# mudit1729/dinov2-od

Measured on AMD Instinct MI355X. Metric: images/sec forward, DINOv2 ViT-B/14 518x518 + 100-query head, higher is better.
Workload: dtype bf16; 1 GPU; ViT-B/14 518x518 bf16, 100 queries, batch 64 per GPU (BASELINE configs[2]'s batch of 64; it fits one GPU, so every GPU runs the whole configuration: weak scaling); global_batch=64, per_gpu_batch=64, image=518, queries=100, parallelism=dp1, hipgraph=True, n_ranks_seen=1, micro_batches=2

## Files before the change

dinov2_od_amd/csrc/dod_api.hip:

```cpp
#include "dod_internal.h"

#include <cstdarg>
#include <cstdio>
#include <atomic>
#include <cstdlib>

using namespace dod;

static std::string g_err;

static int vfail(const dod_handle* h, int code, const char* fmt, va_list ap, int launch_rc = 0) {
  char buf[512];
  const int n = vsnprintf(buf, sizeof buf, fmt, ap);
  if (launch_rc && n >= 0 && (size_t)n < sizeof buf) snprintf(buf + n, sizeof buf - n, " rejected (rc %d)", launch_rc);
  if (h) h->err = buf; else g_err = buf;
  return code;
}
int dod::fail(const dod_handle* h, int code, const char* fmt, ...) {
  va_list ap; va_start(ap, fmt); code = vfail(h, code, fmt, ap); va_end(ap);
  return code;
}
int dod::rejected(const dod_handle* h, int r, const char* fmt, ...) {
  if (!r) return DOD_OK;
  va_list ap; va_start(ap, fmt); const int code = vfail(h, r == 3 ? DOD_ERR_HIP : DOD_ERR_INVALID, fmt, ap, r); va_end(ap);
  return code;
}

static bool check_common(dod_handle* h, int B, int H, int W, int* rc) {
  if (!h) { *rc = fail(nullptr, DOD_ERR_INVALID, "null handle"); return false; }
  if (!h->finalized) { *rc = fail(h, DOD_ERR_STATE, "dod_finalize_weights has not been called"); return false; }
  if (B <= 0) { *rc = fail(h, DOD_ERR_INVALID, "batch must be positive (got %d)", B); return false; }
  if (H < h->cfg.patch || W < h->cfg.patch) { *rc = fail(h, DOD_ERR_INVALID, "image %dx%d smaller than one %dx%d patch", H, W, h->cfg.patch, h->cfg.patch); return false; }
  return true;
}

static std::atomic<int> g_options[DOD_OPT_COUNT] = {{-1}, {-1}, {-1}, {-1}, {-1}, {-1}, {-1}, {-1}, {-1}, {-1}, {-1}};
int dod_option(int which) { return which >= 0 && which < DOD_OPT_COUNT ? g_options[which].load() : -1; }
static const char* const k_option_names[DOD_OPT_COUNT] = {"tailsplit", "dec_fused_split", "mha_chunk_images", "no_fused_patch", "ln_fold", "deterministic", "f32_ksplit",
                                                       "attn_bwd_flash", "epi_regmath", "f32x3_tile", "attn_diet"};

static std::atomic<long> g_form_launches[FORM_COUNT];
static const char* const k_form_names[FORM_COUNT] = {"bf16_128_r2", "bf16_128_r3", "bf16_m16", "k64", "ppm", "x3_16w", "x3_pp", "h2", "fp8_rows", "fp8mx_256x128",
                                                     "fp8mx2_256x128", "fp8mx2_256x256", "f32", "patch_fused"};
void gemm_form_launched(int form) { if (form >= 0 && form < FORM_COUNT) ++g_form_launches[form]; }

extern "C" {

int dod_test_set_option(const char* name, int value) {
  if (!name) return fail(nullptr, DOD_ERR_INVALID, "null option name");
  for (int i = 0; i < DOD_OPT_COUNT; ++i)
    if (!strcmp(name, k_option_names[i])) { g_options[i].store(value); return DOD_OK; }
  return fail(nullptr, DOD_ERR_INVALID, "unknown test option '%s'", name);
}
long dod_test_counter(const char* name) {
  if (name && !strcmp(name, "tail_splits")) return gemm_tail_split_count();
  if (name && !strcmp(name, "rem_cuts")) return gemm_rem_cut_count();
  if (name && !strcmp(name, "f32_ksplits")) return gemm_f32_ksplit_count();
  if (name && !strcmp(name, "epi_regmath")) return gemm_epi_regmath_count();
  if (name && !strcmp(name, "attn_diet")) return attn_half_tile_count();
  if (name && !strcmp(name, "f32x3_launches")) return gemm_f32x3_count(0);
  if (name && !strcmp(name, "f32x3_wide_launches")) return gemm_f32x3_count(1);
  if (name && !strcmp(name, "optim_launches")) return optim_launch_count();
  if (name && !strcmp(name, "optim_chunk_elems")) return optim_constant(0);
  if (name && !strcmp(name, "optim_table_tensors")) return optim_constant(1);
  if (name && !strcmp(name, "optim_norm_table_tensors")) return optim_constant(2);
  if (name && !strncmp(name, "form_", 5))
    for (int i = 0; i < FORM_COUNT; ++i)
      if (!strcmp(name + 5, k_form_names[i])) return g_form_launches[i].load();
  return -1;
}

const char* dod_version(void) { return "dinodet 0.3 (gfx950)"; }
int dod_abi_version(void) { return DOD_ABI_VERSION; }

int dod_device_count(void) {
  int n = 0;
  return hipGetDeviceCount(&n) == hipSuccess ? n : -1;
}

const char* dod_last_error(const dod_handle* h) { return h ? h->err.c_str() : g_err.c_str(); }

int dod_create(const dod_config* cfg, dod_handle** out) {
  if (!cfg || !out) return fail(nullptr, DOD_ERR_INVALID, "null argument");
  const dod_config& c = *cfg;
  if (c.hidden <= 0 || c.layers <= 0 || c.heads <= 0 || c.hidden % c.heads) return fail(nullptr, DOD_ERR_INVALID, "bad backbone dims hidden=%d heads=%d layers=%d", c.hidden, c.heads, c.layers);
  if (c.hidden % 64) return fail(nullptr, DOD_ERR_INVALID, "hidden (%d) must be a multiple of 64", c.hidden);
  {
    const int fm = c.precision == DOD_PREC_FP32 ? 4 : 64;
    if (c.ffn_hidden <= 0 || c.ffn_hidden % fm) return fail(nullptr, DOD_ERR_INVALID, "ffn_hidden (%d) must be a multiple of %d in this precision", c.ffn_hidden, fm);
  }
  if (c.patch <= 0 || c.pos_grid <= 0) return fail(nullptr, DOD_ERR_INVALID, "bad patch/pos_grid");
  if (c.num_queries <= 0 || c.dec_hidden <= 0 || c.dec_heads <= 0 || c.dec_layers <= 0 || c.num_classes <= 0 || c.dim_feedforward <= 0) return fail(nullptr, DOD_ERR_INVALID, "bad decoder dims");
  if (c.dec_hidden % 64 || c.dim_feedforward % 4) return fail(nullptr, DOD_ERR_INVALID, "decoder hidden (%d) must be a multiple of 64, dim_feedforward (%d) of 4", c.dec_hidden, c.dim_feedforward);
  if (c.target_dim && c.target_dim != c.dec_hidden) return fail(nullptr, DOD_ERR_INVALID, "projection dim %d != decoder hidden %d", c.target_dim, c.dec_hidden);
  if (!c.target_dim && c.hidden != c.dec_hidden) return fail(nullptr, DOD_ERR_INVALID, "backbone width %d != decoder hidden %d and no projection", c.hidden, c.dec_hidden);
  if (c.use_deformable && (c.n_points <= 0 || c.n_points > 8)) return fail(nullptr, DOD_ERR_INVALID, "n_points must be 1..8");
  if (c.dec_layers > 64) return fail(nullptr, DOD_ERR_INVALID, "at most 64 decoder layers");
  if (c.precision != DOD_PREC_FP32 && c.precision != DOD_PREC_BF16 && c.precision != DOD_PREC_FP8 && c.precision != DOD_PREC_BF16X3 && c.precision != DOD_PREC_FP16X2) return fail(nullptr, DOD_ERR_INVALID, "unknown precision %d", c.precision);
  dod_handle* h = new (std::nothrow) dod_handle();
  if (!h) return fail(nullptr, DOD_ERR_STATE, "out of host memory");
  h->cfg = c;
  *out = h;
  return DOD_OK;
}

void dod_destroy(dod_handle* h) {
  if (!h) return;
  for (auto& r : h->prof) { (void)hipEventDestroy(r.a); (void)hipEventDestroy(r.b); }
  for (auto e : h->evpool) (void)hipEventDestroy(e);
  for (void* p : h->owned) (void)hipFree(p);
  delete h;
}

int dod_set_weight(dod_handle* h, const char* key, const void* dev_ptr, const int64_t* shape, int ndim, int dtype) {
  if (!h || !key || !dev_ptr || ndim < 0 || ndim > 8 || (ndim && !shape)) return fail(h, DOD_ERR_INVALID, "dod_set_weight: bad argument");
  if (dtype != DOD_F32 && dtype != DOD_BF16) return fail(h, DOD_ERR_INVALID, "dod_set_weight('%s'): dtype %d is neither DOD_F32 nor DOD_BF16", key, dtype);
  std::string k(key);
  if (k.rfind("module.", 0) == 0) k = k.substr(7);
  WRef r; r.raw = dev_ptr; r.dtype = dtype; r.ptr = dtype == DOD_F32 ? (const float*)dev_ptr : nullptr; r.shape.assign(shape, shape + ndim);
  h->w[k] = r;
  h->finalized = false;
  return DOD_OK;
}

int dod_reserve_gemm_scratch(size_t bytes) { return (gemm_tail_reserve(bytes) || gemm_f32_ksplit_reserve()) ? fail(nullptr, DOD_ERR_HIP, "scratch allocation of %zu bytes failed", bytes) : DOD_OK; }

int dod_finalize_weights(dod_handle* h, void* stream) {
  if (!h) return fail(nullptr, DOD_ERR_INVALID, "null handle");
  { static const size_t mb = [] { const char* v = getenv("DINODET_GEMM_SCRATCH_MB"); return v && atoi(v) > 0 ? (size_t)atoi(v) : (size_t)64; }();
    (void)gemm_tail_reserve(mb << 20);
    (void)gemm_f32_ksplit_reserve(); }
  int rc = finalize_impl(h, (hipStream_t)stream);
  if (rc || !h->has_dec) return rc;
  hipStream_t s = (hipStream_t)stream;
  const dod_config& g = h->cfg;
  const size_t Q = g.num_queries, Dd = g.dec_hidden;
  h->l0_tgt = h->l0_proj = nullptr;
  Carver sz(nullptr);
  const size_t bytes = carve_decoder(h, sz, 1, 1, nullptr, false) + 256;
  void* tmp = nullptr;
  float *t0 = nullptr, *p0 = nullptr;
  HIPCHK(h, hipMalloc(&tmp, bytes));
  if (hipMalloc((void**)&t0, Q * Dd * 4) != hipSuccess || (g.use_deformable && hipMalloc((void**)&p0, Q * (size_t)h->ncat * 4) != hipSuccess)) {
    (void)hipFree(tmp); if (t0) (void)hipFree(t0);
    return fail(h, DOD_ERR_HIP, "allocation of the decoder's layer-0 constants failed");
  }
  h->owned.push_back(t0); if (p0) h->owned.push_back(p0);
  Carver cv((void*)(((uintptr_t)tmp + 255) & ~(uintptr_t)255));
  DecWS dw;
  carve_decoder(h, cv, 1, 1, &dw, false);
  rc = decoder_impl(h, nullptr, 1, 1, dw, nullptr, s, true);
  if (!rc) {
    hipError_t e1 = hipMemcpyAsync(t0, dw.tgt, Q * Dd * 4, hipMemcpyDeviceToDevice, s);
    hipError_t e2 = p0 ? hipMemcpyAsync(p0, dw.proj, Q * (size_t)h->ncat * 4, hipMemcpyDeviceToDevice, s) : hipSuccess;
    hipError_t e3 = hipStreamSynchronize(s);
    if (e1 != hipSuccess || e2 != hipSuccess || e3 != hipSuccess) rc = fail(h, DOD_ERR_HIP, "decoder layer-0 constants: %s", hipGetErrorString(e3 != hipSuccess ? e3 : (e1 != hipSuccess ? e1 : e2)));
  } else (void)hipStreamSynchronize(s);
  (void)hipFree(tmp);
  if (rc) return rc;
  h->l0_tgt = t0; h->l0_proj = p0;
  return DOD_OK;
}

int dod_prepare(dod_handle* h, int H, int W, void* stream) {
  if (!h) return fail(nullptr, DOD_ERR_INVALID, "null handle");
  return prepare_impl(h, H, W, (hipStream_t)stream);
}

int dod_num_tokens(const dod_handle* h, int H, int W) { return h ? (H / h->cfg.patch) * (W / h->cfg.patch) + 1 : 0; }

size_t dod_workspace_bytes(const dod_handle* h, int B, int H, int W) {
  if (!h || B <= 0 || H < h->cfg.patch || W < h->cfg.patch) return 0;
  const int N = dod_num_tokens(h, H, W);
  Carver c(nullptr);
  carve_backbone(h, c, B, N, nullptr);
  carve_decoder(h, c, B, N, nullptr, false);
  return c.off + 256;
}

size_t dod_decoder_workspace_bytes(const dod_handle* h, int B, int N) {
  if (!h || B <= 0 || N <= 0) return 0;
  Carver c(nullptr);
  carve_decoder(h, c, B, N, nullptr, true);
  return c.off + 256;
}

int dod_set_tap(dod_handle* h, int stage, float* dst) {
  if (!h) return fail(nullptr, DOD_ERR_INVALID, "null handle");
  if (dst) h->taps[stage] = dst; else h->taps.erase(stage);
  return DOD_OK;
}

int dod_forward(dod_handle* h, const float* pixels, int B, int H, int W, float* det, void* workspace, size_t wsb, void* stream) {
  int rc;
  if (!check_common(h, B, H, W, &rc)) return rc;
  if (!pixels || !det || !workspace) return fail(h, DOD_ERR_INVALID, "null buffer");
  if (wsb < dod_workspace_bytes(h, B, H, W)) return fail(h, DOD_ERR_STATE, "workspace too small: %zu < %zu", wsb, dod_workspace_bytes(h, B, H, W));
  const int N = dod_num_tokens(h, H, W);
  Carver c(align_ws(workspace));
  BbWS bw; DecWS dw;
  carve_backbone(h, c, B, N, &bw);
  carve_decoder(h, c, B, N, &dw, false);
  CARVE_FITS(h, c, workspace, wsb)
  rc = backbone_impl(h, pixels, B, H, W, bw, nullptr, true, (hipStream_t)stream); if (rc) return rc;
  return decoder_impl(h, bw.mem, B, N, dw, det, (hipStream_t)stream);
}

int dod_forward_u8(dod_handle* h, const uint8_t* pixels_hwc, int B, int H, int W, float* det, void* workspace, size_t wsb, void* stream) {
  int rc;
  if (!check_common(h, B, H, W, &rc)) return rc;
  if (!pixels_hwc || !det || !workspace) return fail(h, DOD_ERR_INVALID, "null buffer");
  if (wsb < dod_workspace_bytes(h, B, H, W)) return fail(h, DOD_ERR_STATE, "workspace too small: %zu < %zu", wsb, dod_workspace_bytes(h, B, H, W));
  const int N = dod_num_tokens(h, H, W);
  Carver c(align_ws(workspace));
  BbWS bw; DecWS dw;
  carve_backbone(h, c, B, N, &bw);
  carve_decoder(h, c, B, N, &dw, false);
  CARVE_FITS(h, c, workspace, wsb)
  rc = backbone_impl(h, nullptr, B, H, W, bw, nullptr, true, (hipStream_t)stream, -1, nullptr, pixels_hwc); if (rc) return rc;
  return decoder_impl(h, bw.mem, B, N, dw, det, (hipStream_t)stream);
}

int dod_backbone_forward(dod_handle* h, const float* pixels, int B, int H, int W, float* features, void* workspace, size_t wsb, void* stream) {
  int rc;
  if (!check_common(h, B, H, W, &rc)) return rc;
  if (!pixels || !features || !workspace) return fail(h, DOD_ERR_INVALID, "null buffer");
  if (wsb < dod_workspace_bytes(h, B, H, W)) return fail(h, DOD_ERR_STATE, "workspace too small: %zu < %zu", wsb, dod_workspace_bytes(h, B, H, W));
  const int N = dod_num_tokens(h, H, W);
  Carver c(align_ws(workspace));
  BbWS bw;
  carve_backbone(h, c, B, N, &bw);
  CARVE_FITS(h, c, workspace, wsb)
  return backbone_impl(h, pixels, B, H, W, bw, features, false, (hipStream_t)stream);
}

int dod_backbone_prefix(dod_handle* h, const float* pixels, int B, int H, int W, int nblocks, float* x_out, void* workspace, size_t wsb, void* stream) {
  int rc;
  if (!check_common(h, B, H, W, &rc)) return rc;
  if (!pixels || !x_out || !workspace) return fail(h, DOD_ERR_INVALID, "null buffer");
  if (nblocks < 0 || nblocks > h->cfg.layers) return fail(h, DOD_ERR_INVALID, "nblocks %d outside 0..%d", nblocks, h->cfg.layers);
  if (wsb < dod_workspace_bytes(h, B, H, W)) return fail(h, DOD_ERR_STATE, "workspace too small: %zu < %zu", wsb, dod_workspace_bytes(h, B, H, W));
  const int N = dod_num_tokens(h, H, W);
  Carver c(align_ws(workspace));
  BbWS bw;
  carve_backbone(h, c, B, N, &bw);
  CARVE_FITS(h, c, workspace, wsb)
  return backbone_impl(h, pixels, B, H, W, bw, nullptr, false, (hipStream_t)stream, nblocks, x_out);
}

int dod_decoder_forward(dod_handle* h, const float* memory, int B, int N, float* det, void* workspace, size_t wsb, void* stream) {
  if (!h) return fail(nullptr, DOD_ERR_INVALID, "null handle");
  if (!h->finalized) return fail(h, DOD_ERR_STATE, "dod_finalize_weights has not been called");
  if (B <= 0 || N <= 0) return fail(h, DOD_ERR_INVALID, "bad B=%d N=%d", B, N);
  if (!memory || !det || !workspace) return fail(h, DOD_ERR_INVALID, "null buffer");
  if (wsb < dod_decoder_workspace_bytes(h, B, N)) return fail(h, DOD_ERR_STATE, "workspace too small");
  Carver c(align_ws(workspace));
  DecWS dw;
  carve_decoder(h, c, B, N, &dw, true);
  CARVE_FITS(h, c, workspace, wsb)
  hipStream_t s = (hipStream_t)stream;
  const void* mem_op = memory;
  if (is_bf16(h)) {
    KCHK(h, launch_cast_bf16(memory, (bf16_t*)dw.mem_op, (size_t)B * N * h->cfg.dec_hidden, s));
    mem_op = dw.mem_op;
  }
  return decoder_impl(h, mem_op, B, N, dw, det, s);
}

int dod_profile(dod_handle* h, int enable) {
  if (!h) return fail(nullptr, DOD_ERR_INVALID, "null handle");
  for (auto& r : h->prof) { h->evpool.push_back(r.a); h->evpool.push_back(r.b); }
  h->prof.clear();
  h->prof_on = enable != 0;
  return DOD_OK;
}

int dod_profile_read(dod_handle* h, int cls, double* ms, double* flops, int* launches) {
  if (!h || cls < 0 || cls >= PC_COUNT) return fail(h, DOD_ERR_INVALID, "bad profile class");
  double t = 0, f = 0; int n = 0;
  for (auto& r : h->prof) {
    if (r.cls != cls) continue;
    HIPCHK(h, hipEventSynchronize(r.b));
    float e = 0.f;
    HIPCHK(h, hipEventElapsedTime(&e, r.a, r.b));
    t += e; f += r.flops; ++n;
  }
  if (ms) *ms = t; if (flops) *flops = f; if (launches) *launches = n;
  return DOD_OK;
}

int dod_op_linear(int in_dtype, const void* A, int lda, const void* W, int ldw, int M, int N, int K, const float* bias,
                  const float* scale, const float* resid, int ldr, void* out, int out_dtype, int ldc, int act, void* stream) {
  if (!A || !W || !out) return fail(nullptr, DOD_ERR_INVALID, "null buffer");
  GemmEpi e = epi(bias, out_dtype == DOD_F32 ? (float*)out : nullptr, out_dtype == DOD_BF16 ? out : nullptr, ldc, act, scale, resid, ldr);
  if (act == DOD_ACT_SWIGLU_PAIRS) {
    if (in_dtype != DOD_BF16 || out_dtype != DOD_BF16 || scale || resid || (N & 7)) return fail(nullptr, DOD_ERR_INVALID, "DOD_ACT_SWIGLU_PAIRS: bf16 in / out, N %% 8 == 0, no scale / residual");
    e.act = ACT_NONE; e.glu = 1;
  }
  int r = in_dtype == DOD_BF16 ? launch_gemm_bf16((const bf16_t*)A, lda, (const bf16_t*)W, ldw, M, N, K, e, (hipStream_t)stream)
                               : launch_gemm_f32((const float*)A, lda, (const float*)W, ldw, M, N, K, e, (hipStream_t)stream);
  return rejected(nullptr, r, "dod_op_linear M=%d N=%d K=%d", M, N, K);
}
int dod_op_gemm_f32x(const float* A, int lda, int a_kmajor, long long a_sb, long long a_sh, const float* W, int ldw, int w_kmajor, long long w_sb,
                     long long w_sh, float* C, int ldc, long long c_sb, long long c_sh, int M, int N, int K, int batch, int hb, float alpha,
                     int accumulate, int ksplit, void* stream) {
  if (!A || !W || !C) return fail(nullptr, DOD_ERR_INVALID, "null buffer");
  GemmF32X g; memset(&g, 0, sizeof g);
  g.A = A; g.lda = lda; g.a_kmajor = a_kmajor; g.a_sb = a_sb; g.a_sh = a_sh;
  g.W = W; g.ldw = ldw; g.w_kmajor = w_kmajor; g.w_sb = w_sb; g.w_sh = w_sh;
  g.C = C; g.ldc = ldc; g.c_sb = c_sb; g.c_sh = c_sh;
  g.M = M; g.N = N; g.K = K; g.batch = batch; g.hb = hb; g.alpha = alpha; g.accumulate = accumulate; g.ksplit = ksplit;
  return rejected(nullptr, launch_gemm_f32x(g, (hipStream_t)stream), "dod_op_gemm_f32x M=%d N=%d K=%d batch=%d", M, N, K, batch);
}
int dod_op_gemm_f32x3(const float* A, int lda, int a_kmajor, long long a_sb, long long a_sh, const float* W, int ldw, int w_kmajor, long long w_sb,
                      long long w_sh, float* C, int ldc, long long c_sb, long long c_sh, int M, int N, int K, int batch, int hb, float alpha,
                      int accumulate, int ksplit, void* stream) {
  if (!A || !W || !C) return fail(nullptr, DOD_ERR_INVALID, "null buffer");
  GemmF32X g; memset(&g, 0, sizeof g);
  g.A = A; g.lda = lda; g.a_kmajor = a_kmajor; g.a_sb = a_sb; g.a_sh = a_sh;
  g.W = W; g.ldw = ldw; g.w_kmajor = w_kmajor; g.w_sb = w_sb; g.w_sh = w_sh;
  g.C = C; g.ldc = ldc; g.c_sb = c_sb; g.c_sh = c_sh;
  g.M = M; g.N = N; g.K = K; g.batch = batch; g.hb = hb; g.alpha = alpha; g.accumulate = accumulate; g.ksplit = ksplit;
  return rejected(nullptr, launch_gemm_f32x3(g, (hipStream_t)stream), "dod_op_gemm_f32x3 M=%d N=%d K=%d batch=%d", M, N, K, batch);
}
int dod_op_linear_f32x3(const float* X, int ldx, const float* W, const float* bias, const float* scale, const float* resid, int ldr, int M, int N, int K,
                        float* Y, int ldy, int act, void* stream) {
  if (!X || !W || !Y) return fail(nullptr, DOD_ERR_INVALID, "null buffer");
  if (act < DOD_ACT_NONE || act > DOD_ACT_SIGMOID) return fail(nullptr, DOD_ERR_INVALID, "dod_op_linear_f32x3: activation %d", act);
  GemmF32X g; memset(&g, 0, sizeof g);
  g.A = X; g.lda = ldx; g.W = W; g.ldw = K; g.C = Y; g.ldc = ldy; g.M = M; g.N = N; g.K = K; g.batch = 1; g.hb = 1; g.alpha = 1.0f; g.ksplit = 1;
  g.bias = bias; g.scale = scale; g.resid = resid; g.ldr = ldr; g.act = act;
  return rejected(nullptr, launch_gemm_f32x3(g, (hipStream_t)stream), "dod_op_linear_f32x3 M=%d N=%d K=%d", M, N, K);
}
int dod_op_linear_fp8(const void* A, int lda, const float* a_scale, const void* W, int ldw, const float* w_scale, int M, int N, int K,
                      const float* bias, const float* scale, const float* resid, int ldr, void* out, int out_dtype, int ldc, int act,
                      void* stream) {
  if (!A || !W || !out || !a_scale || !w_scale) return fail(nullptr, DOD_ERR_INVALID, "null buffer");
  GemmEpi e = epi(bias, out_dtype == DOD_F32 ? (float*)out : nullptr, out_dtype == DOD_BF16 ? out : nullptr, ldc, act, scale, resid, ldr);
  e.a_scale = a_scale; e.w_scale = w_scale;
  return rejected(nullptr, launch_gemm_fp8((const unsigned char*)A, lda, (const unsigned char*)W, ldw, M, N, K, e, (hipStream_t)stream), "dod_op_linear_fp8 M=%d N=%d K=%d", M, N, K);
}
int dod_op_linear_fp8_mx(const void* A, int lda, const void* a_block_scales, const void* W, int ldw, const float* w_scale, int M, int N, int K,
                         const float* bias, const float* scale, const float* resid, int ldr, void* out, int out_dtype, int ldc, int act,
                         void* stream) {
  if (!A || !W || !out || !a_block_scales || !w_scale) return fail(nullptr, DOD_ERR_INVALID, "null buffer");
  GemmEpi e = epi(bias, out_dtype == DOD_F32 ? (float*)out : nullptr, out_dtype == DOD_BF16 ? out : nullptr, ldc, act, scale, resid, ldr);
  e.a_bs = (const unsigned char*)a_block_scales; e.w_scale = w_scale;
  return rejected(nullptr, launch_gemm_fp8((const unsigned char*)A, lda, (const unsigned char*)W, ldw, M, N, K, e, (hipStream_t)stream), "dod_op_linear_fp8_mx M=%d N=%d K=%d", M, N, K);
}
int dod_op_linear_fp8_glu_mx(const void* A, int lda, const float* a_scale, const void* W, int ldw, const float* w_scale, int M, int N, int K,
                             const float* bias, void* out_q, int ldq, void* out_block_scales, void* stream) {
  if (!A || !W || !a_scale || !w_scale || !out_q || !out_block_scales) return fail(nullptr, DOD_ERR_INVALID, "null buffer");
  GemmEpi e = epi(bias, nullptr, out_q, ldq);
  e.a_scale = a_scale; e.w_scale = w_scale; e.glu = 1; e.out_bs = (unsigned char*)out_block_scales;
  return rejected(nullptr, launch_gemm_fp8((const unsigned char*)A, lda, (const unsigned char*)W, ldw, M, N, K, e, (hipStream_t)stream), "dod_op_linear_fp8_glu_mx M=%d N=%d K=%d", M, N, K);
}
int dod_op_linear_fp8_mx2(const void* A, int lda, const void* a_block_scales, const void* W, int ldw, const void* w_block_scales, int M, int N, int K,
                          const float* bias, const float* scale, const float* resid, int ldr, void* out, int out_dtype, int ldc, int act,
                          void* glu_out_block_scales, void* stream) {
  if (!A || !W || !out || !a_block_scales || !w_block_scales) return fail(nullptr, DOD_ERR_INVALID, "null buffer");
  GemmEpi e = epi(bias, out_dtype == DOD_F32 ? (float*)out : nullptr, out_dtype == DOD_BF16 ? out : nullptr, ldc, act, scale, resid, ldr);
  e.a_bs = (const unsigned char*)a_block_scales; e.w_bs = (const unsigned char*)w_block_scales;
  if (glu_out_block_scales) { e.out_f32 = nullptr; e.out_bf16 = (bf16_t*)out; e.glu = 1; e.out_bs = (unsigned char*)glu_out_block_scales; }
  return rejected(nullptr, launch_gemm_fp8((const unsigned char*)A, lda, (const unsigned char*)W, ldw, M, N, K, e, (hipStream_t)stream), "dod_op_linear_fp8_mx2 M=%d N=%d K=%d", M, N, K);
}
int dod_op_quant_mx_fp8(const void* x, int in_dtype, int ld, int rows, int cols, void* q, int ldq, void* block_scales, void* stream) {
  if (!x || !q || !block_scales) return fail(nullptr, DOD_ERR_INVALID, "null buffer");
  return rejected(nullptr, launch_quant_mx_fp8(x, in_dtype == DOD_BF16, ld, rows, cols, (unsigned char*)q, ldq, (unsigned char*)block_scales, (hipStream_t)stream), "dod_op_quant_mx_fp8 rows=%d cols=%d", rows, cols);
}
int dod_op_split_pair(const float* x, int ld, int rows, int cols, void* out, void* stream) {
  if (!x || !out) return fail(nullptr, DOD_ERR_INVALID, "null buffer");
  return launch_split2(x, ld, (bf16_t*)out, rows, cols, (hipStream_t)stream) ? fail(nullptr, DOD_ERR_HIP, "launch failed") : DOD_OK;
}
int dod_op_linear_x3(const void* A2, const void* W2, int M, int N, int K, const float* bias, const float* scale, const float* resid, int ldr,
                     void* out, int out_layout, int ldc, int act, void* stream) {
  if (!A2 || !W2 || !out) return fail(nullptr, DOD_ERR_INVALID, "null buffer");
  GemmEpi e = epi(bias, out_layout == 0 ? (float*)out : nullptr, out_layout != 0 ? out : nullptr, ldc, act, scale, resid, ldr);
  if (out_layout == 2) e.out_split = -N;
  return rejected(nullptr, launch_gemm_x3((const bf16_t*)A2, 2 * K, (const bf16_t*)W2, 2 * K, M, N, K, e, (hipStream_t)stream), "dod_op_linear_x3 M=%d N=%d K=%d", M, N, K);
}
int dod_op_split_h2(const float* x, int ld, int rows, int cols, void* out, void* wexp, void* stream) {
  if (!x || !out) return fail(nullptr, DOD_ERR_INVALID, "null buffer");
  return rejected(nullptr, launch_split_h2(x, ld, out, rows, cols, (unsigned char*)wexp, (hipStream_t)stream), "dod_op_split_h2 rows=%d cols=%d", rows, cols);
}
int dod_op_linear_h2(const void* A, const void* W, const void* wexp, int M, int N, int K, const float* bias, const float* scale, const float* resid,
                     int ldr, void* out, int out_layout, int ldc, int act, void* stream) {
  if (!A || !W || !wexp || !out) return fail(nullptr, DOD_ERR_INVALID, "null buffer");
  GemmEpi e = epi(bias, out_layout == 0 ? (float*)out : nullptr, out_layout != 0 ? out : nullptr, ldc, act, scale, resid, ldr);
  if (out_layout == 2) e.out_split = -N;
  if (out_layout == 3) e.out_h2 = 1;
  e.h2_wexp = (const unsigned char*)wexp;
  return rejected(nullptr, launch_gemm_h2(A, 4 * K, W, 3 * K, M, N, K, e, (hipStream_t)stream), "dod_op_linear_h2 M=%d N=%d K=%d", M, N, K);
}
int dod_op_linear_ln(int family, const void* A, const void* W, const void* wexp, int M, int N, int K, const float* bias, const float* scale,
                     const float* resid, int ldr, void* out, int out_layout, int ldc, int act, const dod_ln_fold* ln, void* stream) {
  if (!A || !W || !out || !ln) return fail(nullptr, DOD_ERR_INVALID, "null buffer");
  if (family != DOD_PREC_BF16 && family != DOD_PREC_BF16X3 && family != DOD_PREC_FP16X2) return fail(nullptr, DOD_ERR_INVALID, "family must be a bf16 / bf16x3 / fp16x2 precision");
  if ((ln->stats == nullptr) != (ln->csum == nullptr)) return fail(nullptr, DOD_ERR_INVALID, "stats and csum go together");
  if (ln->stats && scale) return fail(nullptr, DOD_ERR_INVALID, "the folded consumer has no LayerScale");
  if (ln->part && !(resid && out_layout == 0)) return fail(nullptr, DOD_ERR_INVALID, "the folded producer is the fp32 residual epilogue");
  GemmEpi e = epi(bias, out_layout == 0 ? (float*)out : nullptr, out_layout != 0 ? out : nullptr, ldc, act, scale, resid, ldr);
  if (out_layout == 2) e.out_split = -N;
  if (out_layout == 3) e.out_h2 = 1;
  e.ln_stats = (const float2*)ln->stats; e.ln_c = ln->csum;
  if (ln->part_in) {
    if (!ln->stats || ln->stats_out == ln->stats) return fail(nullptr, DOD_ERR_INVALID, "part_in needs stats (the shift) and a DIFFERENT stats_out buffer");
    e.ln_part_in = (const float2*)ln->part_in; e.ln_npart = (K + 127) / 128; e.ln_stats_out = (float2*)ln->stats_out; e.ln_eps = ln->eps;
  }
  if (ln->part) {
    e.ln_part = (float2*)ln->part; e.ln_npart = (N + 127) / 128; e.ln_op = ln->op_out; e.ln_shift = (const float2*)ln->shift;
    e.ln_op_kind = family == DOD_PREC_FP16X2 ? LNOP_H2 : (family == DOD_PREC_BF16X3 ? LNOP_PAIR : LNOP_BF16);
    e.ln_op_ld = family == DOD_PREC_BF16 ? N : 2 * N;
  }
  int r;
  if (family == DOD_PREC_FP16X2) {
    if (!wexp) return fail(nullptr, DOD_ERR_INVALID, "null buffer");
    e.h2_wexp = (const unsigned char*)wexp;
    r = launch_gemm_h2(A, 4 * K, W, 3 * K, M, N, K, e, (hipStream_t)stream);
  } else if (family == DOD_PREC_BF16X3) r = launch_gemm_x3((const bf16_t*)A, 2 * K, (const bf16_t*)W, 2 * K, M, N, K, e, (hipStream_t)stream);
  else r = launch_gemm_bf16((const bf16_t*)A, K, (const bf16_t*)W, K, M, N, K, e, (hipStream_t)stream);
  return rejected(nullptr, r, "dod_op_linear_ln M=%d N=%d K=%d", M, N, K);
}
int dod_op_rowstats(const float* x, int rows, int D, float eps, void* op_out, int family, void* stats, void* stream) {
  if (!x || !op_out || !stats) return fail(nullptr, DOD_ERR_INVALID, "null buffer");
  const int kind = family == DOD_PREC_FP16X2 ? LNOP_H2 : (family == DOD_PREC_BF16X3 ? LNOP_PAIR : (family == DOD_PREC_BF16 ? LNOP_BF16 : 0));
  return rejected(nullptr, launch_rowstats(x, rows, D, eps, op_out, kind, (float2*)stats, (hipStream_t)stream), "dod_op_rowstats rows=%d D=%d", rows, D);
}
int dod_op_ln_finalize(const void* part, int rows, int D, float eps, void* stats, void* stream) {
  if (!part || !stats) return fail(nullptr, DOD_ERR_INVALID, "null buffer");
  return rejected(nullptr, launch_ln_finalize((const float2*)part, (D + 127) / 128, rows, D, eps, (float2*)stats, (hipStream_t)stream), "dod_op_ln_finalize rows=%d D=%d", rows, D);
}
int dod_op_attention_x3(const void* qkv2, void* ctx2, int B, int N, int heads, float scale, void* stream) {
  if (!qkv2 || !ctx2) return fail(nullptr, DOD_ERR_INVALID, "null buffer");
  return rejected(nullptr, launch_attn_x3((const bf16_t*)qkv2, (bf16_t*)ctx2, B, N, heads, scale, (hipStream_t)stream), "dod_op_attention_x3");
}
static bool attn_grid_fits(int B, int N, int heads) {
  return (((long long)B * heads + 7) / 8 * 8) * (((long long)N + 127) / 128 + 1) <= 0x7fffffffLL;
}
int dod_op_attention_x3_h2(const void* qkv2, void* ctx_h2, int B, int N, int heads, float scale, void* stream) {
  if (!qkv2 || !ctx_h2) return fail(nullptr, DOD_ERR_INVALID, "null buffer");
  if (B <= 0 || N <= 0 || heads <= 0) return fail(nullptr, DOD_ERR_INVALID, "dod_op_attention_x3_h2: B=%d N=%d heads=%d must be positive", B, N, heads);
  if (!attn_grid_fits(B, N, heads)) return fail(nullptr, DOD_ERR_INVALID, "dod_op_attention_x3_h2: B=%d N=%d heads=%d is more workgroups than one launch holds", B, N, heads);
  return rejected(nullptr, launch_attn_x3((const bf16_t*)qkv2, (bf16_t*)ctx_h2, B, N, heads, scale, (hipStream_t)stream, 1), "dod_op_attention_x3_h2");
}
int dod_op_quant_rows_fp8(const void* x, int in_dtype, int ld, int rows, int cols, void* q, int ldq, float* scale, void* stream) {
  if (!x || !q || !scale) return fail(nullptr, DOD_ERR_INVALID, "null buffer");
  return rejected(nullptr, launch_quant_rows_fp8(x, in_dtype == DOD_BF16, ld, rows, cols, (unsigned char*)q, ldq, scale, (hipStream_t)stream), "dod_op_quant_rows_fp8 rows=%d cols=%d", rows, cols);
}
int dod_op_layernorm(const float* x, const float* add, const float* gamma, const float* beta, float eps, int rows, int D, void* out, int out_dtype, void* stream) {
  if (!x || !gamma || !beta || !out) return fail(nullptr, DOD_ERR_INVALID, "null buffer");
  return rejected(nullptr, launch_layernorm(x, add, gamma, beta, eps, rows, D, ln_out(out_dtype == DOD_F32 ? (float*)out : nullptr, out_dtype == DOD_BF16 ? (bf16_t*)out : nullptr), (hipStream_t)stream), "dod_op_layernorm rows=%d D=%d", rows, D);
}
int dod_op_attention_bf16(const void* qkv, void* ctx, int B, int N, int heads, float scale, void* stream) {
  if (!qkv || !ctx) return fail(nullptr, DOD_ERR_INVALID, "null buffer");
  return rejected(nullptr, launch_attn_bf16((const bf16_t*)qkv, (bf16_t*)ctx, B, N, heads, scale, (hipStream_t)stream), "dod_op_attention_bf16");
}
int dod_op_attention_bf16_mx(const void* qkv, void* ctx_q8, void* ctx_bs, int B, int N, int heads, float scale, void* stream) {
  if (!qkv || !ctx_q8 || !ctx_bs) return fail(nullptr, DOD_ERR_INVALID, "null buffer");
  if (B <= 0 || N <= 0 || heads <= 0) return fail(nullptr, DOD_ERR_INVALID, "dod_op_attention_bf16_mx: B=%d N=%d heads=%d must be positive", B, N, heads);
  if (!attn_grid_fits(B, N, heads)) return fail(nullptr, DOD_ERR_INVALID, "dod_op_attention_bf16_mx: B=%d N=%d heads=%d is more workgroups than one launch holds", B, N, heads);
  return rejected(nullptr, launch_attn_bf16((const bf16_t*)qkv, (bf16_t*)ctx_q8, B, N, heads, scale, (hipStream_t)stream, (unsigned char*)ctx_bs), "dod_op_attention_bf16_mx");
}
int dod_op_attention_f32(const float* q, const float* k, const float* v, float* o, int ldq, int ldk, int ldv, int ldo, int Lq, int Lk,
                         int B, int heads, int dh, float scale, void* stream) {
  if (!q || !k || !v || !o) return fail(nullptr, DOD_ERR_INVALID, "null buffer");
  AttnF32 a; a.q = q; a.k = k; a.v = v; a.o = o; a.ldq = ldq; a.ldk = ldk; a.ldv = ldv; a.ldo = ldo; a.Lq = Lq; a.Lk = Lk; a.B = B; a.heads = heads; a.dh = dh; a.scale = scale;
  return rejected(nullptr, launch_attn_f32(a, (hipStream_t)stream), "dod_op_attention_f32 (dh=%d)", dh);
}
int dod_op_deform_sample(const float* proj, int ldp, const float* values, int B, int Q, int N, int Hd, int P, int dh, int hh, int ww, float* out, void* stream) {
  if (!proj || !values || !out) return fail(nullptr, DOD_ERR_INVALID, "null buffer");
  if (hh * ww != N) return fail(nullptr, DOD_ERR_INVALID, "Cannot reshape input of size %d into a %dx%d feature map", N, hh, ww);
  return rejected(nullptr, launch_deform_sample(proj, ldp, values, B, Q, N, Hd, P, dh, hh, ww, out, (hipStream_t)stream), "dod_op_deform_sample");
}
int dod_op_pos_resize(const float* pos_in, int G, int gh, int gw, int D, float* pos_out, void* stream) {
  if (!pos_in || !pos_out) return fail(nullptr, DOD_ERR_INVALID, "null buffer");
  return launch_pos_resize(pos_in, G, gh, gw, D, pos_out, (hipStream_t)stream) ? fail(nullptr, DOD_ERR_HIP, "launch failed") : DOD_OK;
}
int dod_op_im2col(const float* img, int B, int H, int W, int patch, int Kp, void* out, int out_dtype, void* stream) {
  if (!img || !out) return fail(nullptr, DOD_ERR_INVALID, "null buffer");
  int r = launch_im2col(img, B, H, W, patch, Kp, out_dtype == DOD_F32 ? (float*)out : nullptr, out_dtype == DOD_BF16 ? (bf16_t*)out : nullptr, (hipStream_t)stream);
  return r ? fail(nullptr, DOD_ERR_INVALID, "dod_op_im2col rejected") : DOD_OK;
}

}
```

dinov2_od_amd/csrc/dod_common.h:

```cpp
#pragma once
#include <hip/hip_runtime.h>
#include <stdint.h>
#include <stdlib.h>

typedef __attribute__((ext_vector_type(8))) __bf16 bf16x8;
typedef __attribute__((ext_vector_type(4))) __bf16 bf16x4;
typedef __attribute__((ext_vector_type(2))) __bf16 bf16x2;
typedef __attribute__((ext_vector_type(16))) float f32x16;
typedef __attribute__((ext_vector_type(4))) float f32x4;
typedef __attribute__((ext_vector_type(2))) float f32x2;
typedef unsigned short bf16_t;

#define DOD_WAVE 64

enum { DOD_OPT_TAILSPLIT = 0,
       DOD_OPT_DEC_FUSED_SPLIT,
       DOD_OPT_MHA_CHUNK_IMAGES,
       DOD_OPT_NO_FUSED_PATCH,
       DOD_OPT_LN_FOLD,
       DOD_OPT_DETERMINISTIC,
       DOD_OPT_F32_KSPLIT,
       DOD_OPT_ATTN_BWD_FLASH,
       DOD_OPT_EPI_REGMATH,
       DOD_OPT_F32X3_TILE,
       DOD_OPT_ATTN_DIET,
       DOD_OPT_COUNT };
int dod_option(int which);
long gemm_tail_split_count();
long optim_launch_count();
long optim_constant(int which);
long gemm_rem_cut_count();
long attn_half_tile_count();
long gemm_epi_regmath_count();
enum { FORM_BF16_128_R2 = 0, FORM_BF16_128_R3, FORM_BF16_M16, FORM_K64, FORM_PPM, FORM_X3_16W, FORM_X3_PP, FORM_H2, FORM_FP8_ROWS, FORM_FP8MX_256X128,
       FORM_FP8MX2_256X128, FORM_FP8MX2_256X256, FORM_F32, FORM_PATCH_FUSED, FORM_COUNT };
void gemm_form_launched(int form);

#ifdef DINODET_TUNING
#define DOD_TUNE_ENV(name) getenv(name)
#else
#define DOD_TUNE_ENV(name) (static_cast<const char*>(nullptr))
#endif

__device__ __forceinline__ bf16_t f2bf(float f) {
  __bf16 b = (__bf16)f;
  return __builtin_bit_cast(bf16_t, b);
}
__device__ __forceinline__ float bf2f(bf16_t h) {
  return __builtin_bit_cast(float, ((uint32_t)h) << 16);
}
__device__ __forceinline__ uint32_t pack2bf(float lo, float hi) {
  f32x2 v = {lo, hi};
  bf16x2 h = __builtin_convertvector(v, bf16x2);
  return __builtin_bit_cast(uint32_t, h);
}
__device__ __forceinline__ float wave_sum(float v) {
#pragma unroll
  for (int o = 32; o > 0; o >>= 1) v += __shfl_xor(v, o, 64);
  return v;
}
__device__ __forceinline__ float wave_max(float v) {
#pragma unroll
  for (int o = 32; o > 0; o >>= 1) v = fmaxf(v, __shfl_xor(v, o, 64));
  return v;
}
__device__ __forceinline__ unsigned pack4_fp8(float a, float b, float c, float d) {
  int w = __builtin_amdgcn_cvt_pk_fp8_f32(a, b, 0, false);
  w = __builtin_amdgcn_cvt_pk_fp8_f32(c, d, w, true);
  return (unsigned)w;
}
__device__ __forceinline__ unsigned mx_ebyte(float amax) {
  const unsigned b = __float_as_uint(amax * (1.0f / 448.0f));
  unsigned eb = ((b >> 23) & 0xffu) + ((b & 0x7fffffu) ? 1u : 0u);
  eb = eb < 1u ? 1u : (eb > 253u ? 253u : eb);
  return eb;
}
__device__ __forceinline__ float mx_inv_scale(unsigned eb) { return __uint_as_float((254u - eb) << 23); }
__device__ __forceinline__ size_t mx_scale_off(int K, int bi) { return (size_t)(bi & 1) * (K >> 6) + (bi >> 1); }
typedef __attribute__((ext_vector_type(2))) _Float16 f16x2;
typedef __attribute__((ext_vector_type(8))) _Float16 f16x8;
__device__ __forceinline__ float clampf_(float v, float lim) { return __builtin_fminf(__builtin_fmaxf(v, -lim), lim); }
__device__ __forceinline__ void h2_quad(float4 v, float shi, uint2& f16, unsigned& hi8, unsigned& lo8) {
  v.x = clampf_(v.x, 65504.f); v.y = clampf_(v.y, 65504.f); v.z = clampf_(v.z, 65504.f); v.w = clampf_(v.w, 65504.f);
  const f16x2 p0 = {(_Float16)v.x, (_Float16)v.y}, p1 = {(_Float16)v.z, (_Float16)v.w};
  f16.x = __builtin_bit_cast(unsigned, p0); f16.y = __builtin_bit_cast(unsigned, p1);
  const float hx = (float)p0.x, hy = (float)p0.y, hz = (float)p1.x, hw = (float)p1.y;
  const float slo = shi * 2048.0f;
  hi8 = pack4_fp8(clampf_(hx * shi, 448.f), clampf_(hy * shi, 448.f), clampf_(hz * shi, 448.f), clampf_(hw * shi, 448.f));
  lo8 = pack4_fp8(clampf_((v.x - hx) * slo, 448.f), clampf_((v.y - hy) * slo, 448.f), clampf_((v.z - hz) * slo, 448.f), clampf_((v.w - hw) * slo, 448.f));
}
__device__ __forceinline__ size_t h2_off8(int K, int c) { return (size_t)2 * K + (size_t)(c >> 4) * 32 + (c & 15); }

__device__ __forceinline__ float gelu_erf(float x) { return 0.5f * x * (1.0f + erff(x * 0.70710678118654752440f)); }
typedef float f32x2_t __attribute__((ext_vector_type(2)));
__device__ __forceinline__ f32x2_t gelu_fast2(f32x2_t x) {
  f32x2_t ax; ax.x = __builtin_fabsf(x.x); ax.y = __builtin_fabsf(x.y);
  const f32x2_t z = ax * 0.8493218002880191f;
  const f32x2_t d = __builtin_elementwise_fma(z, (f32x2_t)(0.2727374808792225f), (f32x2_t)(1.0f));
  f32x2_t t; t.x = __builtin_amdgcn_rcpf(d.x); t.y = __builtin_amdgcn_rcpf(d.y);
  f32x2_t p = __builtin_elementwise_fma(t, (f32x2_t)(0.5f * 1.061405429f), (f32x2_t)(0.5f * -1.453152027f));
  p = __builtin_elementwise_fma(p, t, (f32x2_t)(0.5f * 1.421413741f));
  p = __builtin_elementwise_fma(p, t, (f32x2_t)(0.5f * -0.284496736f));
  p = __builtin_elementwise_fma(p, t, (f32x2_t)(0.5f * 0.254829592f));
  const f32x2_t nz2 = -z * z;
  f32x2_t e; e.x = __builtin_amdgcn_exp2f(nz2.x); e.y = __builtin_amdgcn_exp2f(nz2.y);
  const f32x2_t q = ax * (t * p);
  const f32x2_t r = __builtin_elementwise_fma(ax, (f32x2_t)(0.5f), x * 0.5f);
  return __builtin_elementwise_fma(-q, e, r);
}
__device__ __forceinline__ void gelu_fast4(float4& v) {
  f32x2_t a = {v.x, v.y}, b = {v.z, v.w};
  a = gelu_fast2(a); b = gelu_fast2(b);
  v.x = a.x; v.y = a.y; v.z = b.x; v.w = b.y;
}
__device__ __forceinline__ float sigmoidf_(float x) { return 1.0f / (1.0f + expf(-x)); }

enum { ACT_NONE = 0, ACT_RELU = 1, ACT_GELU = 2, ACT_SIGMOID = 3 };

struct GemmEpi {
  const float* bias;
  const float* scale;
  const float* resid;
  int ldr;
  float* out_f32;
  bf16_t* out_bf16;
  int ldc;
  int act;
  const float* pos;
  int rows_per_img;
  int out_rows_per_img;
  int out_split;
  const float* a_scale;
  const float* w_scale;
  unsigned char* out_bs;
  const unsigned char* a_bs;
  const unsigned char* w_bs;
  int out_h2;
  const unsigned char* h2_wexp;
  int ksplit;
  int kslice_len;
  long long kslice_stride;
  int glu;
  void* ln_op;
  int ln_op_kind;
  int ln_op_ld;
  float2* ln_part;
  int ln_npart;
  const float2* ln_shift;
  const float2* ln_stats;
  const float* ln_c;
  const float2* ln_part_in;
  float2* ln_stats_out;
  float ln_eps;
};
enum { LNOP_BF16 = 1, LNOP_PAIR = 2, LNOP_H2 = 3 };
inline bool gemm_epi_rows_ok(const GemmEpi& e) {
  return e.rows_per_img == 0 && !e.pos && e.ksplit <= 1 && !e.a_scale && !e.a_bs && !e.out_bs;
}
inline GemmEpi gemm_epi_rows(const GemmEpi& e, int m0) {
  GemmEpi r = e;
  const size_t m = (size_t)m0;
  if (r.resid) r.resid += m * r.ldr;
  if (r.out_f32) r.out_f32 += m * r.ldc;
  if (r.out_bf16) r.out_bf16 += m * r.ldc;
  if (r.ln_op) r.ln_op = reinterpret_cast<char*>(r.ln_op) + m * (size_t)r.ln_op_ld * 2;
  if (r.ln_part) r.ln_part += m * r.ln_npart;
  if (r.ln_shift) r.ln_shift += m;
  if (r.ln_stats) r.ln_stats += m;
  if (r.ln_part_in) r.ln_part_in += m * r.ln_npart;
  if (r.ln_stats_out) r.ln_stats_out += m;
  return r;
}

int launch_gemm_bf16(const bf16_t* A, int lda, const bf16_t* W, int ldw, int M, int N, int K,
                     const GemmEpi& e, hipStream_t s);
int launch_gemm_f32(const float* A, int lda, const float* W, int ldw, int M, int N, int K,
                    const GemmEpi& e, hipStream_t s, bool allow_ksplit = false);
int gemm_f32_ksplit_reserve();
long gemm_f32_ksplit_count();
struct GemmF32X {
  const float* A; const float* W; float* C; const float* bias;
  const float* scale;
  const float* resid;
  int ldr;
  int lda, ldw, ldc, M, N, K;
  long long a_sb, a_sh, w_sb, w_sh, c_sb, c_sh;
  int batch, hb;
  int a_kmajor, w_kmajor;
  float alpha;
  int accumulate;
  int act;
  int ksplit;
};
int launch_gemm_f32x(const GemmF32X& g, hipStream_t s);
int launch_gemm_f32x3(const GemmF32X& g, hipStream_t s);
long gemm_f32x3_count(int wide);
int launch_quant_mx_fp8(const void* x, int in_bf16, int ld, int rows, int cols, unsigned char* q, int ldq, unsigned char* bs, hipStream_t s);
int launch_gemm_fp8(const unsigned char* A, int lda, const unsigned char* W, int ldw, int M, int N, int K,
                    const GemmEpi& e, hipStream_t s);
int launch_attn_x3(const bf16_t* qkv2, bf16_t* ctx3, int B, int N, int heads, float scale, hipStream_t s, int ctx_h2 = 0);
int launch_swiglu_fp8(const bf16_t* in, int rows, int Fh, unsigned char* q, float* scale, hipStream_t s);
int launch_quant_rows_fp8(const void* x, int in_bf16, int ld, int rows, int cols, unsigned char* q, int ldq, float* scale,
                          hipStream_t s);

struct LnOut {
  float* f32 = nullptr;
  bf16_t* bf16 = nullptr;
  unsigned char* fp8 = nullptr;
  float* scale = nullptr;
  bf16_t* split = nullptr;
  bf16_t* a3 = nullptr;
  unsigned char* bs = nullptr;
};
inline LnOut ln_out(float* f32, bf16_t* bf16 = nullptr, bf16_t* a3 = nullptr) { LnOut o; o.f32 = f32; o.bf16 = bf16; o.a3 = a3; return o; }
int launch_layernorm(const float* x, const float* add, const float* gamma, const float* beta, float eps, int rows, int D, const LnOut& out,
                     hipStream_t s, int split_h2 = 0);
int launch_rowstats(const float* x, int rows, int D, float eps, void* op, int op_kind, float2* stats, hipStream_t s);
int launch_ln_finalize(const float2* part, int npart, int rows, int D, float eps, float2* stats, hipStream_t s);
int launch_ln_fold(const float* W, int rows, int cols, const float* gamma, const float* beta, const float* bias_in, float* Wout, float* bias_out, hipStream_t s);
int launch_rowsum(const float* W, int rows, int cols, int round_bf16, float* c, hipStream_t s);

int launch_attn_bf16(const bf16_t* qkv, bf16_t* ctx, int B, int N, int heads, float scale, hipStream_t s, unsigned char* ctx_bs = nullptr);

struct AttnF32 {
  const float *q, *k, *v; float* o;
  int ldq, ldk, ldv, ldo;
  int Lq, Lk;
  int B, heads, dh;
  float scale;
  bf16_t* o3 = nullptr;
  float* lse = nullptr;
};
int launch_attn_f32(const AttnF32& a, hipStream_t s);
struct AttnF32Bwd {
  const float *q, *k, *v, *o, *d_o, *lse;
  float *dq, *dk, *dv, *delta;
  int ldq, ldk, ldv, ldo, lddq, lddk, lddv;
  int Lq, Lk, B, heads, dh;
  float scale;
};
int launch_attn_f32_bwd(const AttnF32Bwd& a, hipStream_t s);

int launch_im2col(const float* img, int B, int H, int W, int patch, int Kp, float* out_f32, bf16_t* out_bf16, hipStream_t s);
int launch_patch_pack(const float* W, int D, int p, bf16_t* out, int x3, hipStream_t s);
int launch_patch_embed(const void* img, int u8, int B, int H, int W, int p, const bf16_t* Wp, int x3, const float* bias, const float* pos,
                       float* out, int D, hipStream_t s);
int launch_cls_row(const float* cls, const float* pos, float* x, int B, int N, int D, hipStream_t s);
int launch_pos_resize(const float* pos_in, int G, int gh, int gw, int D, float* pos_out, hipStream_t s);
int launch_interleave_halves(const float* src, float* dst, int F, int cols, hipStream_t s);
int launch_swiglu(const float* in_f32, const bf16_t* in_bf16, int rows, int Fh, float* out_f32, bf16_t* out_bf16, hipStream_t s);
int launch_cast_bf16(const float* in, bf16_t* out, size_t n, hipStream_t s);
int launch_copy2d(const float* src, int ld_src, float* dst, int ld_dst, int rows, int cols, int cols_pad, hipStream_t s);
int launch_lora_merge(const float* W, const float* A, const float* Bm, float alpha, int out_f, int in_f, int r, float* dst, hipStream_t s);
int launch_split3(const float* in, int ld_in, bf16_t* out, int rows, int K, int mode, hipStream_t s);
int launch_split2(const float* in, int ld_in, bf16_t* out, int rows, int K, hipStream_t s);
int launch_split_h2(const float* in, int ld_in, void* out, int rows, int K, unsigned char* wexp, hipStream_t s);
int launch_gemm_h2(const void* A, int lda, const void* W, int ldw, int M, int N, int K, const GemmEpi& e, hipStream_t s);
int gemm_tail_split(int kind, const void* A, int lda, const void* W, int ldw, int M, int N, int K, const GemmEpi& e, hipStream_t s);
int gemm_tail_reserve(size_t bytes);
int launch_gemm_bf16_k64(const bf16_t* A, int lda, const bf16_t* W, int ldw, int M, int N, int K, const GemmEpi& e, hipStream_t s);
int gemm_tile_mode();
int launch_gemm_bf16_ppm(const bf16_t* A, int lda, const bf16_t* W, int ldw, int M, int N, int K, const GemmEpi& e, hipStream_t s);
int launch_gemm_x3_pp(const bf16_t* A2, int lda, const bf16_t* W2, int ldw, int M, int N, int K, const GemmEpi& e, hipStream_t s);
int launch_gemm_x3(const bf16_t* A2, int lda, const bf16_t* W2, int ldw, int M, int N, int K, const GemmEpi& e, hipStream_t s);
int launch_bcast_rows(const float* src, float* dst, int B, int rows, int D, hipStream_t s);

int launch_deform_sample(const float* proj, int ldp, const float* values, int B, int Q, int N, int Hd, int P, int dh,
                         int h, int w, float* out, hipStream_t s, int proj_shared = 0, bf16_t* out3 = nullptr);
```

dinov2_od_amd/csrc/gemm_bf16.hip:

```cpp
#include "dod_common.h"
#include "gemm_epi.h"
#include <atomic>
#include <cstdlib>

#define BM 128
#define BN 128
#define BK 64
#define STAGE_BYTES (2 * BM * BK * 2)

__device__ __forceinline__ int swz128(int row, int chunk) { return chunk ^ ((row >> 1) & 7); }

template <int LN, int SLOTS>
__global__ __launch_bounds__(256) void gemm_bf16_kernel(const bf16_t* __restrict__ A, int lda,
                                                        const bf16_t* __restrict__ W, int ldw,
                                                        int M, int N, int K, GemmEpi e) {
  extern __shared__ __attribute__((aligned(16))) char smem[];
  const int tid = threadIdx.x, lane = tid & 63, wid = tid >> 6;
  const int wm = wid >> 1, wn = wid & 1;
  const int tiles_m = (M + BM - 1) / BM, tiles_n = (N + BN - 1) / BN;
  const int nwg = tiles_m * tiles_n;
  int bid = blockIdx.x;
  {
    const int q = nwg >> 3, r = nwg & 7, xcd = bid & 7;
    bid = (xcd < r ? xcd * (q + 1) : r * (q + 1) + (xcd - r) * q) + (bid >> 3);
  }
  int tm, tn;
  {
    const int GM = 8;
    const int per_group = GM * tiles_n;
    const int grp = bid / per_group, first_m = grp * GM;
    const int gsz = (tiles_m - first_m) < GM ? (tiles_m - first_m) : GM;
    const int in_g = bid - grp * per_group;
    tm = first_m + in_g % gsz;
    tn = in_g / gsz;
  }
  const int m0 = tm * BM, n0 = tn * BN;

  typedef __attribute__((address_space(1))) const void* gptr_t;
  typedef __attribute__((address_space(3))) void* lptr_t;
  const bf16_t* gA0; const bf16_t* gA1; const bf16_t* gA2; const bf16_t* gA3;
  const bf16_t* gW0; const bf16_t* gW1; const bf16_t* gW2; const bf16_t* gW3;
  {
    auto src = [&](const bf16_t* base, int ld, int r0, int piece, int lim) {
      const int rl = piece * 8 + (lane >> 3);
      int r = r0 + rl; r = r < lim ? r : lim - 1;
      const int c = (lane & 7) ^ ((rl >> 1) & 7);
      return base + (size_t)r * ld + c * 8;
    };
    const int p0 = wid * 4;
    gA0 = src(A, lda, m0, p0, M); gA1 = src(A, lda, m0, p0 + 1, M); gA2 = src(A, lda, m0, p0 + 2, M); gA3 = src(A, lda, m0, p0 + 3, M);
    gW0 = src(W, ldw, n0, p0, N); gW1 = src(W, ldw, n0, p0 + 1, N); gW2 = src(W, ldw, n0, p0 + 2, N); gW3 = src(W, ldw, n0, p0 + 3, N);
  }
  const int wbase = __builtin_amdgcn_readfirstlane(wid) * 4096;
#define STAGE(stage, k0)                                                                                   \
  {                                                                                                        \
    char* sA_ = smem + (stage) * STAGE_BYTES + wbase;                                                      \
    char* sW_ = sA_ + BM * BK * 2;                                                                         \
    __builtin_amdgcn_global_load_lds((gptr_t)(gA0 + (k0)), (lptr_t)(sA_), 16, 0, 0);                       \
    __builtin_amdgcn_global_load_lds((gptr_t)(gA1 + (k0)), (lptr_t)(sA_ + 1024), 16, 0, 0);                \
    __builtin_amdgcn_global_load_lds((gptr_t)(gA2 + (k0)), (lptr_t)(sA_ + 2048), 16, 0, 0);                \
    __builtin_amdgcn_global_load_lds((gptr_t)(gA3 + (k0)), (lptr_t)(sA_ + 3072), 16, 0, 0);                \
    __builtin_amdgcn_global_load_lds((gptr_t)(gW0 + (k0)), (lptr_t)(sW_), 16, 0, 0);                       \
    __builtin_amdgcn_global_load_lds((gptr_t)(gW1 + (k0)), (lptr_t)(sW_ + 1024), 16, 0, 0);                \
    __builtin_amdgcn_global_load_lds((gptr_t)(gW2 + (k0)), (lptr_t)(sW_ + 2048), 16, 0, 0);                \
    __builtin_amdgcn_global_load_lds((gptr_t)(gW3 + (k0)), (lptr_t)(sW_ + 3072), 16, 0, 0);                \
  }

  f32x16 acc[2][2];
#pragma unroll
  for (int i = 0; i < 2; ++i)
#pragma unroll
    for (int j = 0; j < 2; ++j)
#pragma unroll
      for (int r = 0; r < 16; ++r) acc[i][j][r] = 0.f;

  const int nk = K / BK;
  STAGE(0, 0)
  if (SLOTS > 2 && nk > 1) STAGE(1, BK)
  const int lr = lane & 31, lh = lane >> 5;
  int slot = 0;
  for (int kt = 0; kt < nk; ++kt) {
    if (SLOTS > 2 && kt + 1 < nk) asm volatile("s_waitcnt vmcnt(8)" ::: "memory");
    else asm volatile("s_waitcnt vmcnt(0)" ::: "memory");
    __builtin_amdgcn_s_barrier();
    asm volatile("" ::: "memory");
    if (kt + SLOTS - 1 < nk) {
      const int ns = slot + SLOTS - 1 >= SLOTS ? slot - 1 : slot + SLOTS - 1;
      STAGE(ns, (kt + SLOTS - 1) * BK)
    }
    const char* sA = smem + slot * STAGE_BYTES;
    const char* sW = sA + BM * BK * 2;
#pragma unroll
    for (int kk = 0; kk < 4; ++kk) {
      bf16x8 af[2], wf[2];
#pragma unroll
      for (int i = 0; i < 2; ++i) {
        const int rowa = wm * 64 + i * 32 + lr;
        af[i] = *reinterpret_cast<const bf16x8*>(sA + rowa * 128 + swz128(rowa, kk * 2 + lh) * 16);
        const int roww = wn * 64 + i * 32 + lr;
        wf[i] = *reinterpret_cast<const bf16x8*>(sW + roww * 128 + swz128(roww, kk * 2 + lh) * 16);
      }
#pragma unroll
      for (int i = 0; i < 2; ++i)
#pragma unroll
        for (int j = 0; j < 2; ++j)
          acc[i][j] = __builtin_amdgcn_mfma_f32_32x32x16_bf16(wf[j], af[i], acc[i][j], 0, 0, 0);
    }
    slot = slot + 1 == SLOTS ? 0 : slot + 1;
  }
  __syncthreads();

  constexpr int PITCH = BN * 4 + 16;
#pragma unroll
  for (int i = 0; i < 2; ++i)
#pragma unroll
    for (int j = 0; j < 2; ++j)
      stage_acc(smem, PITCH, wm * 64 + i * 32 + lr, wn * 64 + j * 32, acc[i][j], lh);
  const ColParams cp = load_col_params<BN, LN>(e, n0, N, tid);
  auto rowmap = [&](int row_l) { return m0 + row_l; };
  stage_row_stats<BM, BN, LN>(smem, PITCH, e, M, tid, rowmap, K, n0);
  __syncthreads();
  drain_tile<BM, BN, 256, LN>(smem, PITCH, e, cp, M, N, n0, tid, rowmap);
}

#define B4K 32
#define B5M 256
#define B5N 128
#define B5_STAGE ((B5M + B5N) * B4K * 2)
#define B5_SLOTS 3

#define STAGE5(slot_, k0)                                                                                  \
  {                                                                                                        \
    char* sA_ = smem + (slot_) * B5_STAGE + wu * 2048;                                                     \
    char* sW_ = smem + (slot_) * B5_STAGE + B5M * B4K * 2 + wu * 1024;                                     \
    __builtin_amdgcn_global_load_lds((gptr_t)(gA0 + (k0)), (lptr_t)(sA_), 16, 0, 0);                       \
    __builtin_amdgcn_global_load_lds((gptr_t)(gA1 + (k0)), (lptr_t)(sA_ + 1024), 16, 0, 0);                \
    __builtin_amdgcn_global_load_lds((gptr_t)(gW0 + (k0)), (lptr_t)(sW_), 16, 0, 0);                       \
  }

__device__ __forceinline__ int swz64m16(int row, int chunk) { return chunk ^ (((row >> 3) & 1) << 1); }

#ifdef DINODET_TUNING
__device__ unsigned long long* g_gemm_stamps = nullptr;
#endif

template <int LN>
__global__ __launch_bounds__(512, 4) void gemm_bf16_256x128_m16_kernel(const bf16_t* __restrict__ A, int lda,
                                                                       const bf16_t* __restrict__ W, int ldw,
                                                                       int M, int N, int K, GemmEpi e, int GM) {
  extern __shared__ __attribute__((aligned(16))) char smem[];
  const int tid = threadIdx.x, lane = tid & 63, wid = tid >> 6;
  const int wm = wid >> 1, wn = wid & 1;
  const int tiles_m = (M + B5M - 1) / B5M, tiles_n = (N + B5N - 1) / B5N;
  const int nwg = tiles_m * tiles_n;
#ifdef DINODET_TUNING
  unsigned long long* stamps = g_gemm_stamps;
  unsigned long long t_start = 0, t_loop = 0;
  if (stamps) t_start = __builtin_amdgcn_s_memrealtime();
#endif
  int tm, tn;
  tile_map(blockIdx.x, tiles_m, tiles_n, GM, &tm, &tn);
  const int m0 = tm * B5M, n0 = tn * B5N;
  typedef __attribute__((address_space(1))) const void* gptr_t;
  typedef __attribute__((address_space(3))) void* lptr_t;
  const bf16_t* gA0; const bf16_t* gA1; const bf16_t* gW0;
  {
    auto src = [&](const bf16_t* base, int ld, int r0, int piece, int lim) {
      const int rl = piece * 16 + (lane >> 2);
      int r = r0 + rl; r = r < lim ? r : lim - 1;
      const int c = swz64m16(rl, lane & 3);
      return base + (size_t)r * ld + c * 8;
    };
    gA0 = src(A, lda, m0, wid * 2, M); gA1 = src(A, lda, m0, wid * 2 + 1, M);
    gW0 = src(W, ldw, n0, wid, N);
  }
  const int wu = __builtin_amdgcn_readfirstlane(wid);
  f32x4 acc[4][4];
#pragma unroll
  for (int i = 0; i < 4; ++i)
#pragma unroll
    for (int j = 0; j < 4; ++j) acc[i][j] = f32x4{0.f, 0.f, 0.f, 0.f};
  const int nk = K / B4K;
  const int l15 = lane & 15, l4 = lane >> 4;
  STAGE5(0, 0)
  if (nk > 1) STAGE5(1, B4K)
  int offA[4], offW[4];
#pragma unroll
  for (int i = 0; i < 4; ++i) { const int row = wm * 64 + i * 16 + l15; offA[i] = row * 64 + swz64m16(row, l4) * 16; }
#pragma unroll
  for (int j = 0; j < 4; ++j) { const int row = wn * 64 + j * 16 + l15; offW[j] = B5M * B4K * 2 + row * 64 + swz64m16(row, l4) * 16; }
  int slot = 0;
  for (int kt = 0; kt < nk; ++kt) {
    if (kt + 1 < nk) asm volatile("s_waitcnt vmcnt(3)" ::: "memory");
    else asm volatile("s_waitcnt vmcnt(0)" ::: "memory");
    __builtin_amdgcn_s_barrier();
    asm volatile("" ::: "memory");
    if (kt + 2 < nk) {
      const int ns = slot >= 1 ? slot - 1 : 2;
      STAGE5(ns, (kt + 2) * B4K)
    }
    const char* st = smem + slot * B5_STAGE;
    bf16x8 af[4], wf[4];
#pragma unroll
    for (int i = 0; i < 4; ++i) af[i] = *reinterpret_cast<const bf16x8*>(st + offA[i]);
#pragma unroll
    for (int j = 0; j < 4; ++j) wf[j] = *reinterpret_cast<const bf16x8*>(st + offW[j]);
#pragma unroll
    for (int i = 0; i < 4; ++i)
#pragma unroll
      for (int j = 0; j < 4; ++j)
        acc[i][j] = __builtin_amdgcn_mfma_f32_16x16x32_bf16(wf[j], af[i], acc[i][j], 0, 0, 0);
    slot = slot == 2 ? 0 : slot + 1;
  }
#ifdef DINODET_TUNING
  if (stamps) t_loop = __builtin_amdgcn_s_memrealtime();
#endif
  constexpr int PITCH = B5N * 4 + 16;
  const ColParams cp = load_col_params<B5N, LN>(e, n0, N, tid);
#pragma unroll
  for (int pass = 0; pass < 2; ++pass) {
    __builtin_amdgcn_s_barrier();
    asm volatile("" ::: "memory");
#pragma unroll
    for (int ii = 0; ii < 2; ++ii)
#pragma unroll
      for (int j = 0; j < 4; ++j) {
        const int row_l = wm * 32 + ii * 16 + l15;
        const int col = wn * 64 + j * 16 + 4 * l4;
        const f32x4 a = acc[pass * 2 + ii][j];
        *reinterpret_cast<float4*>(smem + row_l * PITCH + col * 4) = make_float4(a[0], a[1], a[2], a[3]);
      }
    auto rowmap = [&](int row_l) { return m0 + (row_l >> 5) * 64 + pass * 32 + (row_l & 31); };
    stage_row_stats<128, B5N, LN>(smem, PITCH, e, M, tid, rowmap, K, n0);
    __syncthreads();
    drain_tile<128, B5N, 512, LN>(smem, PITCH, e, cp, M, N, n0, tid, rowmap);
  }
#ifdef DINODET_TUNING
  if (stamps && tid == 0) {
    asm volatile("s_waitcnt vmcnt(0)" ::: "memory");
    unsigned long long* o = stamps + (size_t)blockIdx.x * 4;
    o[0] = t_start; o[1] = t_loop; o[2] = __builtin_amdgcn_s_memrealtime(); o[3] = blockIdx.x;
  }
#endif
}

static constexpr int LDS128 = (BM * (BN * 4 + 16)) > 2 * STAGE_BYTES ? (BM * (BN * 4 + 16)) : 2 * STAGE_BYTES;
static constexpr int LDS128R = 3 * STAGE_BYTES;
static constexpr int LDS5 = (128 * (B5N * 4 + 16)) > B5_SLOTS * B5_STAGE ? (128 * (B5N * 4 + 16)) : B5_SLOTS * B5_STAGE;

static std::atomic<long> g_rem_cuts{0};
long gemm_rem_cut_count() { return g_rem_cuts.load(); }

int launch_gemm_bf16(const bf16_t* A, int lda, const bf16_t* W, int ldw, int M, int N, int K,
                     const GemmEpi& e, hipStream_t s) {
  if (M <= 0 || N <= 0 || K <= 0) return 1;
  if (K % BK != 0 || N % 4 != 0 || lda % 8 != 0 || ldw % 8 != 0 || e.ldc % 4 != 0) return 2;
  if (e.resid && e.ldr % 4 != 0) return 2;
  if (!e.out_f32 && !e.out_bf16) return 2;
  static bool attr_set[16] = {};
  int dev = 0;
  (void)hipGetDevice(&dev);
  if (dev >= 0 && dev < 16 && !attr_set[dev]) {
#define ATTR_(LN_) (void)hipFuncSetAttribute(reinterpret_cast<const void*>(gemm_bf16_kernel<LN_, 2>), hipFuncAttributeMaxDynamicSharedMemorySize, LDS128); \
                   (void)hipFuncSetAttribute(reinterpret_cast<const void*>(gemm_bf16_kernel<LN_, 3>), hipFuncAttributeMaxDynamicSharedMemorySize, LDS128R); \
                   (void)hipFuncSetAttribute(reinterpret_cast<const void*>(gemm_bf16_256x128_m16_kernel<LN_>), hipFuncAttributeMaxDynamicSharedMemorySize, LDS5);
    ATTR_(LN_NONE) ATTR_(LN_CONS) ATTR_(LN_PROD)
#undef ATTR_
    attr_set[dev] = true;
  }
  const char* force = DOD_TUNE_ENV("DINODET_GEMM_TILE");
  if (!force && M >= 2048 && N >= 512 && e.act != ACT_GELU && e.act != ACT_SIGMOID && e.rows_per_img == 0 && K % 64 == 0) {
    const int t = gemm_tail_split(0, A, lda, W, ldw, M, N, K, e, s);
    if (t >= 0) return t;
  }
  if (force && force[0] == 'q' && K % 64 == 0) return launch_gemm_bf16_ppm(A, lda, W, ldw, M, N, K, e, s);
  if (force && force[0] == 'x') return launch_gemm_bf16_k64(A, lda, W, ldw, M, N, K, e, s);
  const int gm5 = (N >= 3072 ? 8 : (N >= 2048 ? 4 : 2)) | (gemm_tile_mode() & 0x300);
  const int tiles5 = ((M + B5M - 1) / B5M) * ((N + B5N - 1) / B5N);
#define GO_M16(LN_) hipLaunchKernelGGL(gemm_bf16_256x128_m16_kernel<LN_>, dim3(tiles5), dim3(512), LDS5, s, A, lda, W, ldw, M, N, K, e, gm5);
  if (!force && M >= 4096 && N >= 512 && K % 64 == 0 && e.act != ACT_SIGMOID && e.rows_per_img == 0) {
    static int cus[16] = {};
    if (dev >= 0 && dev < 16 && !cus[dev]) { int c = 0; (void)hipDeviceGetAttribute(&c, hipDeviceAttributeMultiprocessorCount, dev); cus[dev] = c > 0 ? c : 256; }
    const int cu = (dev >= 0 && dev < 16) ? cus[dev] : 256;
    const long tm = (M + 255) / 256, t_big = tm * ((N + 255) / 256), t_small = tm * ((N + 127) / 128);
    const double c_big = (double)((t_big + cu - 1) / cu) * (e.act == ACT_GELU ? 1.08 : 1.0);
    const double c_small = (double)((t_small + cu - 1) / cu) * (K >= 2048 ? 0.62 : 0.55);
    if (N >= 1536 && K < 2048) {
      const long rounds = t_big / cu, rem = t_big % cu;
      static const int rem_div = [] { const char* v = DOD_TUNE_ENV("DINODET_GEMM_REMCUT"); return v ? atoi(v) : 6; }();
      if (rounds >= 1 && rounds <= 2 && rem * 16 >= cu && rem_div > 0 && rem * rem_div <= cu && gemm_epi_rows_ok(e)) {
        const int tn = (N + 255) / 256;
        const int Mmain = (int)((rounds * cu) / tn) * 256, R = M - Mmain;
        if (Mmain >= 2048 && R > 0 && R < 2048) {
          const int rc = launch_gemm_bf16_k64(A, lda, W, ldw, Mmain, N, K, e, s);
          if (rc) return rc;
          ++g_rem_cuts;
          return launch_gemm_bf16(A + (size_t)Mmain * lda, lda, W, ldw, R, N, K, gemm_epi_rows(e, Mmain), s);
        }
      }
      return launch_gemm_bf16_k64(A, lda, W, ldw, M, N, K, e, s);
    }
    static const double m16_bias = [] { const char* v = DOD_TUNE_ENV("DINODET_GEMM_M16_BIAS"); return v ? atof(v) : 1.02; }();
    if (c_big <= c_small * m16_bias) {
      if (K >= 2048) return launch_gemm_bf16_ppm(A, lda, W, ldw, M, N, K, e, s);
      return launch_gemm_bf16_k64(A, lda, W, ldw, M, N, K, e, s);
    }
    LN_DISPATCH(e, GO_M16)
    gemm_form_launched(FORM_BF16_M16);
    return hipGetLastError() == hipSuccess ? 0 : 3;
  }
  const bool few = (long)tiles5 * 2 <= 256 + 64;
  const bool m16 = force ? (force[0] == '8') : (M >= 1024 && N >= 128 && !few);
  if (m16) {
    LN_DISPATCH(e, GO_M16)
    gemm_form_launched(FORM_BF16_M16);
  } else {
    const int tiles = ((M + BM - 1) / BM) * ((N + BN - 1) / BN);
    static const int ring = [] { const char* v = DOD_TUNE_ENV("DINODET_GEMM_RING"); return v ? atoi(v) : 1; }();
    int cu128 = 256;
    { static int cus[16] = {}; if (dev >= 0 && dev < 16) { if (!cus[dev]) { int c = 0; (void)hipDeviceGetAttribute(&c, hipDeviceAttributeMultiprocessorCount, dev); cus[dev] = c > 0 ? c : 256; } cu128 = cus[dev]; } }
#define GO_128(LN_) hipLaunchKernelGGL((gemm_bf16_kernel<LN_, 2>), dim3(tiles), dim3(256), LDS128, s, A, lda, W, ldw, M, N, K, e);
#define GO_128R(LN_) hipLaunchKernelGGL((gemm_bf16_kernel<LN_, 3>), dim3(tiles), dim3(256), LDS128R, s, A, lda, W, ldw, M, N, K, e);
    if (ring && tiles <= cu128 && K >= 3 * BK) { LN_DISPATCH(e, GO_128R) gemm_form_launched(FORM_BF16_128_R3); }
    else { LN_DISPATCH(e, GO_128) gemm_form_launched(FORM_BF16_128_R2); }
#undef GO_128
#undef GO_128R
  }
  return hipGetLastError() == hipSuccess ? 0 : 3;
}
#undef GO_M16

#ifdef DINODET_TUNING
extern "C" int dod_debug_gemm_stamps(void* dev_buf) {
  unsigned long long* p = (unsigned long long*)dev_buf;
  return hipMemcpyToSymbol(HIP_SYMBOL(g_gemm_stamps), &p, sizeof(p)) == hipSuccess ? 0 : 4;
}

template <int SHAPE>
__global__ __launch_bounds__(256, 2) void mfma_peak_kernel(int iters, unsigned long long* out) {
  bf16x8 a, b;
#pragma unroll
  for (int i = 0; i < 8; ++i) { a[i] = (bf16_t)(0x3c00 + threadIdx.x + i); b[i] = (bf16_t)(0x3c10 + threadIdx.x * 3 + i); }
  if (iters < 0) {
    iters = -iters;
#pragma unroll
    for (int i = 0; i < 8; ++i) {
      const unsigned r1 = (threadIdx.x * 8u + i + 1u) * 2654435761u, r2 = (threadIdx.x * 8u + i + 7u) * 40503u * 2246822519u;
      a[i] = (bf16_t)(0x3f00u | ((r1 >> 9) & 0xffu) | (((r1 >> 20) & 1u) << 15));
      b[i] = (bf16_t)(0x3f00u | ((r2 >> 9) & 0xffu) | (((r2 >> 20) & 1u) << 15));
    }
  }
  const unsigned long long c0 = __builtin_amdgcn_s_memtime(), r0 = __builtin_amdgcn_s_memrealtime();
  float chk = 0.f;
  if (SHAPE == 16) {
    f32x4 acc[8];
#pragma unroll
    for (int i = 0; i < 8; ++i) acc[i] = f32x4{0.f, 0.f, 0.f, 0.f};
    for (int it = 0; it < iters; ++it) {
#pragma unroll
      for (int i = 0; i < 8; ++i) acc[i] = __builtin_amdgcn_mfma_f32_16x16x32_bf16(a, b, acc[i], 0, 0, 0);
    }
#pragma unroll
    for (int i = 0; i < 8; ++i) chk += acc[i][0];
  } else if (SHAPE == 1) {
    f32x16 acc1;
#pragma unroll
    for (int r = 0; r < 16; ++r) acc1[r] = 0.f;
    const float fa = bf2f(a[0]) * (1.0f + 0.37f * bf2f(a[1])), fb = bf2f(b[0]) * (1.0f + 0.41f * bf2f(b[1]));
    for (int it = 0; it < iters; ++it) {
#pragma unroll
      for (int i = 0; i < 4; ++i) acc1 = __builtin_amdgcn_mfma_f32_32x32x2f32(fa, fb, acc1, 0, 0, 0);
    }
    chk += acc1[0];
  } else if (SHAPE == 2) {
    f32x16 acc[4];
#pragma unroll
    for (int i = 0; i < 4; ++i)
#pragma unroll
      for (int r = 0; r < 16; ++r) acc[i][r] = 0.f;
    const float fa = bf2f(a[0]) * (1.0f + 0.37f * bf2f(a[1])), fb = bf2f(b[0]) * (1.0f + 0.41f * bf2f(b[1]));
    for (int it = 0; it < iters; ++it) {
#pragma unroll
      for (int i = 0; i < 4; ++i) acc[i] = __builtin_amdgcn_mfma_f32_32x32x2f32(fa, fb, acc[i], 0, 0, 0);
    }
#pragma unroll
    for (int i = 0; i < 4; ++i) chk += acc[i][0];
  } else {
    f32x16 acc[4];
#pragma unroll
    for (int i = 0; i < 4; ++i)
#pragma unroll
      for (int r = 0; r < 16; ++r) acc[i][r] = 0.f;
    for (int it = 0; it < iters; ++it) {
#pragma unroll
      for (int i = 0; i < 4; ++i) acc[i] = __builtin_amdgcn_mfma_f32_32x32x16_bf16(a, b, acc[i], 0, 0, 0);
    }
#pragma unroll
    for (int i = 0; i < 4; ++i) chk += acc[i][0];
  }
  const unsigned long long c1 = __builtin_amdgcn_s_memtime(), r1 = __builtin_amdgcn_s_memrealtime();
  if (threadIdx.x == 0) {
    out[(size_t)blockIdx.x * 4 + 0] = c1 - c0;
    out[(size_t)blockIdx.x * 4 + 1] = r1 - r0;
    out[(size_t)blockIdx.x * 4 + 2] = (unsigned long long)__float_as_uint(chk);
  }
}
extern "C" int dod_debug_mfma_peak(int shape, int iters, int blocks, void* dev_out, void* stream) {
  if (!dev_out || iters == 0 || blocks <= 0 || (shape != 16 && shape != 32 && shape != 2 && shape != 1)) return 1;
  if (shape == 1) hipLaunchKernelGGL(mfma_peak_kernel<1>, dim3(blocks), dim3(256), 0, (hipStream_t)stream, iters, (unsigned long long*)dev_out);
  else if (shape == 2) hipLaunchKernelGGL(mfma_peak_kernel<2>, dim3(blocks), dim3(256), 0, (hipStream_t)stream, iters, (unsigned long long*)dev_out);
  else if (shape == 16) hipLaunchKernelGGL(mfma_peak_kernel<16>, dim3(blocks), dim3(256), 0, (hipStream_t)stream, iters, (unsigned long long*)dev_out);
  else hipLaunchKernelGGL(mfma_peak_kernel<32>, dim3(blocks), dim3(256), 0, (hipStream_t)stream, iters, (unsigned long long*)dev_out);
  return hipGetLastError() == hipSuccess ? 0 : 4;
}

template <int NV, int mode>
__global__ __launch_bounds__(256, 2) void mfma_valu_probe_kernel(int iters, unsigned long long* out) {
  bf16x8 a, b;
#pragma unroll
  for (int i = 0; i < 8; ++i) { a[i] = (bf16_t)(0x3c00 + threadIdx.x + i); b[i] = (bf16_t)(0x3c10 + threadIdx.x * 3 + i); }
  f32x16 acc[4];
#pragma unroll
  for (int i = 0; i < 4; ++i)
#pragma unroll
    for (int r = 0; r < 16; ++r) acc[i][r] = 0.f;
  float v[NV];
#pragma unroll
  for (int i = 0; i < NV; ++i) v[i] = 1.0f + 0.001f * (threadIdx.x + i);
  const float m = 0.999f, c = 0.001f;
  const unsigned long long c0 = __builtin_amdgcn_s_memtime();
  for (int it = 0; it < iters; ++it) {
#pragma unroll
    for (int q = 0; q < 4; ++q) {
      if (mode & 1) asm volatile("v_mfma_f32_32x32x16_bf16 %0, %1, %2, %0" : "+v"(acc[q]) : "v"(a), "v"(b));
      if (mode & 2) {
#pragma unroll
        for (int i = 0; i < NV / 4; ++i) asm volatile("v_fma_f32 %0, %0, %1, %2" : "+v"(v[q * (NV / 4) + i]) : "v"(m), "v"(c));
      }
    }
  }
  const unsigned long long c1 = __builtin_amdgcn_s_memtime();
  float chk = 0.f;
#pragma unroll
  for (int i = 0; i < 4; ++i) chk += acc[i][0];
#pragma unroll
  for (int i = 0; i < NV; ++i) chk += v[i];
  if (threadIdx.x == 0) { out[(size_t)blockIdx.x * 4] = c1 - c0; out[(size_t)blockIdx.x * 4 + 2] = (unsigned long long)__float_as_uint(chk); }
}
template <int NV>
static int probe_launch(int mode, int iters, int blocks, void* dev_out, void* stream) {
  unsigned long long* o = (unsigned long long*)dev_out;
  if (mode == 1) hipLaunchKernelGGL((mfma_valu_probe_kernel<NV, 1>), dim3(blocks), dim3(256), 0, (hipStream_t)stream, iters, o);
  else if (mode == 2) hipLaunchKernelGGL((mfma_valu_probe_kernel<NV, 2>), dim3(blocks), dim3(256), 0, (hipStream_t)stream, iters, o);
  else if (mode == 3) hipLaunchKernelGGL((mfma_valu_probe_kernel<NV, 3>), dim3(blocks), dim3(256), 0, (hipStream_t)stream, iters, o);
  else return 1;
  return hipGetLastError() == hipSuccess ? 0 : 4;
}
extern "C" int dod_debug_mfma_valu_probe(int nvalu, int mode, int iters, int blocks, void* dev_out, void* stream) {
  if (!dev_out || iters <= 0 || blocks <= 0) return 1;
  if (nvalu == 16) return probe_launch<16>(mode, iters, blocks, dev_out, stream);
  if (nvalu == 28) return probe_launch<28>(mode, iters, blocks, dev_out, stream);
  if (nvalu == 56) return probe_launch<56>(mode, iters, blocks, dev_out, stream);
  return 1;
}
#endif
```

dinov2_od_amd/csrc/gemm_epi.h:

```cpp
#pragma once
#include "dod_common.h"

__device__ __forceinline__ int swz64(int row, int chunk) { return chunk ^ ((row >> 2) & 3); }

#ifdef DINODET_TUNING
__device__ __forceinline__ void stagger_start(int b, int mode) {
  const int sd = (mode >> 16) & 0xfff;
  if (sd == 0 || b >= 256) return;
  const int k = (b >> 3) % (((mode >> 12) & 0xf) + 1);
  if (k == 0) return;
  const unsigned long long until = __builtin_amdgcn_s_memrealtime() + (unsigned long long)k * sd * 16;
  while (__builtin_amdgcn_s_memrealtime() < until) __builtin_amdgcn_s_sleep(16);
}

#endif

__device__ __forceinline__ void tile_map(int b, int tiles_m, int tiles_n, int mode, int* tm_out, int* tn_out) {
#ifdef DINODET_TUNING
  stagger_start(b, mode);
#endif
  const int GM = mode & 0xff;
  const int nwg = tiles_m * tiles_n;
  int tm, tn;
#ifdef DINODET_TUNING
  if (mode & 0x400) {
    const int xcd = b & 7, idx = b >> 3, hn = tiles_n >> 1;
    tm = (idx / hn) * 4 + (xcd >> 1);
    tn = (xcd & 1) * hn + idx % hn;
    if (tm >= tiles_m) tm = -1;
  } else
#endif
  if (mode & 0x200) {
    const int per_group = GM * tiles_n;
    const int nfull = tiles_m / (8 * GM);
    const int body = nfull * 8 * per_group;
    if (b < body) {
      const int xcd = b & 7, idx = b >> 3;
      const int chunk = idx / per_group, in_g = idx - chunk * per_group;
      tm = (chunk * 8 + xcd) * GM + in_g % GM;
      tn = in_g / GM;
    } else {
      const int t = b - body, R = tiles_m - nfull * 8 * GM;
      tm = nfull * 8 * GM + t % R;
      tn = t / R;
    }
  } else {
    int bid = b;
    {
      const int q = nwg >> 3, r = nwg & 7, xcd = bid & 7;
      bid = (xcd < r ? xcd * (q + 1) : r * (q + 1) + (xcd - r) * q) + (bid >> 3);
    }
    const int per_group = GM * tiles_n;
    const int grp = bid / per_group, first_m = grp * GM;
    const int gsz = (tiles_m - first_m) < GM ? (tiles_m - first_m) : GM;
    const int in_g = bid - grp * per_group;
    tm = first_m + in_g % gsz;
    tn = in_g / gsz;
  }
  if ((mode & 0x100) && tm >= 0) tm = tiles_m - 1 - tm;
  *tm_out = tm; *tn_out = tn;
}

__device__ __forceinline__ float silu_mul(float a, float b) { return a / (1.0f + expf(-a)) * b; }

__device__ __forceinline__ void stage_acc(char* sm, int pitch, int row_l, int col_l, const f32x16& a, int lh) {
#pragma unroll
  for (int g = 0; g < 4; ++g) {
    const int nl = col_l + 8 * g + 4 * lh;
    *reinterpret_cast<float4*>(sm + row_l * pitch + nl * 4) = make_float4(a[4 * g], a[4 * g + 1], a[4 * g + 2], a[4 * g + 3]);
  }
}

enum { LN_NONE = 0, LN_CONS = 1, LN_PROD = 2 };
template <int ROWS, int COLS, int LN, typename RowMap>
__device__ __forceinline__ void stage_row_stats(char* sm, int pitch, const GemmEpi& e, int M, int tid, RowMap rowmap, int D = 0, int n0 = 0) {
  if (LN == LN_NONE) return;
  if (tid < ROWS) {
    const float2* src = LN == LN_CONS ? e.ln_stats : e.ln_shift;
    const int m = rowmap(tid);
    float2 st = make_float2(0.f, 0.f);
    if (src && m < M) {
      st = src[m];
      if (LN == LN_CONS && e.ln_part_in) {
        const float2* p = e.ln_part_in + (size_t)m * e.ln_npart;
        float S = 0.f, Q = 0.f;
        for (int g = 0; g < e.ln_npart; ++g) { const float2 pg = p[g]; S += pg.x; Q += pg.y; }
        const float dm = S / (float)D;
        st = make_float2(st.x + dm, 1.0f / sqrtf(fmaxf(Q / (float)D - dm * dm, 0.f) + e.ln_eps));
        if (n0 == 0 && e.ln_stats_out) e.ln_stats_out[m] = st;
      }
    }
    *reinterpret_cast<float2*>(sm + tid * pitch + COLS * 4) = st;
  }
}

struct ColParams { float4 bias, scale, wscale; };
__host__ __device__ __forceinline__ int ln_mode_of(const GemmEpi& e) { return e.ln_part ? LN_PROD : (e.ln_stats ? LN_CONS : LN_NONE); }
#define LN_DISPATCH(e_, GO_)                                          \
  switch (ln_mode_of(e_)) {                                           \
    case LN_PROD: { GO_(LN_PROD) } break;                             \
    case LN_CONS: { GO_(LN_CONS) } break;                             \
    default: { GO_(LN_NONE) } break;                                  \
  }

template <int COLS, int LN = LN_NONE>
__device__ __forceinline__ ColParams load_col_params(const GemmEpi& e, int n0, int N, int tid) {
  ColParams c;
  const int n = n0 + 4 * (tid % (COLS / 4));
  const bool ok = n < N;
  c.bias = (e.bias && ok) ? *reinterpret_cast<const float4*>(e.bias + n) : make_float4(0.f, 0.f, 0.f, 0.f);
  const float* sc = LN == LN_CONS ? e.ln_c : e.scale;
  c.scale = (sc && ok) ? *reinterpret_cast<const float4*>(sc + n) : make_float4(1.f, 1.f, 1.f, 1.f);
  c.wscale = (e.w_scale && ok) ? *reinterpret_cast<const float4*>(e.w_scale + n) : make_float4(1.f, 1.f, 1.f, 1.f);
  return c;
}

template <int CTRL, int ROW_MASK>
__device__ __forceinline__ float dpp_pick(float v) {
  return __builtin_bit_cast(float, __builtin_amdgcn_update_dpp(0, __builtin_bit_cast(int, v), CTRL, ROW_MASK, 0xf, true));
}
__device__ __forceinline__ float half32_sum_hi(float v) {
  v += dpp_pick<0xB1, 0xf>(v);
  v += dpp_pick<0x4E, 0xf>(v);
  v += dpp_pick<0x141, 0xf>(v);
  v += dpp_pick<0x140, 0xf>(v);
  v += dpp_pick<0x142, 0xa>(v);
  return v;
}
__device__ __forceinline__ void ln_store_op(const GemmEpi& e, size_t m, int n, int N, const float4& v) {
  if (e.ln_op_kind == LNOP_H2) {
    uint2 f16; unsigned hi8, lo8;
    h2_quad(v, 1.0f, f16, hi8, lo8);
    char* row = reinterpret_cast<char*>(e.ln_op) + m * (size_t)e.ln_op_ld * 2;
    *reinterpret_cast<uint2*>(row + 2 * n) = f16;
    char* p8 = row + h2_off8(N, n);
    *reinterpret_cast<unsigned*>(p8) = hi8;
    *reinterpret_cast<unsigned*>(p8 + 16) = lo8;
    return;
  }
  uint2 hi;
  hi.x = pack2bf(v.x, v.y);
  hi.y = pack2bf(v.z, v.w);
  bf16_t* o = reinterpret_cast<bf16_t*>(e.ln_op) + m * (size_t)e.ln_op_ld + n;
  *reinterpret_cast<uint2*>(o) = hi;
  if (e.ln_op_kind == LNOP_PAIR) {
    uint2 lo;
    lo.x = pack2bf(v.x - __uint_as_float(hi.x << 16), v.y - __uint_as_float(hi.x & 0xffff0000u));
    lo.y = pack2bf(v.z - __uint_as_float(hi.y << 16), v.w - __uint_as_float(hi.y & 0xffff0000u));
    *reinterpret_cast<uint2*>(o + (e.ln_op_ld >> 1)) = lo;
  }
}

template <int RB, int STEP, int ITER, int C4, bool LNF, typename RowMap>
__device__ __forceinline__ void drain_resid(const char* sm, int pitch, const GemmEpi& e, const ColParams& cp, int M, int N, int n, int c4, int tid, RowMap rowmap) {
  const int rb = tid / C4;
  const bool nv = !LNF || n < N;
  const int wj = (c4 & 31) - 16;
  const bool writer = LNF && wj >= 0 && wj < RB && (n & ~127) < N;
#pragma unroll 1
  for (int it = 0; it < ITER; it += RB) {
    float4 r[RB];
    int mm[RB];
    float kk[RB];
#pragma unroll
    for (int j = 0; j < RB; ++j) {
      mm[j] = rowmap(rb + (it + j) * STEP);
      r[j] = make_float4(0.f, 0.f, 0.f, 0.f);
      if (mm[j] < M && nv) r[j] = *reinterpret_cast<const float4*>(e.resid + (size_t)mm[j] * e.ldr + n);
      if (LNF) kk[j] = reinterpret_cast<const float2*>(sm + (rb + (it + j) * STEP) * pitch + C4 * 16)->x;
    }
    float2 mine = make_float2(0.f, 0.f);
#pragma unroll
    for (int j = 0; j < RB; ++j) {
      if (!LNF && mm[j] >= M) continue;
      const bool ok = nv && mm[j] < M;
      float4 v = *reinterpret_cast<const float4*>(sm + (rb + (it + j) * STEP) * pitch + c4 * 16);
      v.x += cp.bias.x; v.y += cp.bias.y; v.z += cp.bias.z; v.w += cp.bias.w;
      if (e.act == ACT_GELU) { gelu_fast4(v); }
      else if (e.act == ACT_RELU) { v.x = fmaxf(v.x, 0.f); v.y = fmaxf(v.y, 0.f); v.z = fmaxf(v.z, 0.f); v.w = fmaxf(v.w, 0.f); }
      v.x = fmaf(v.x, cp.scale.x, r[j].x); v.y = fmaf(v.y, cp.scale.y, r[j].y);
      v.z = fmaf(v.z, cp.scale.z, r[j].z); v.w = fmaf(v.w, cp.scale.w, r[j].w);
      if (ok) *reinterpret_cast<float4*>(e.out_f32 + (size_t)mm[j] * e.ldc + n) = v;
      if (LNF) {
        if (ok && e.ln_op) ln_store_op(e, (size_t)mm[j], n, N, v);
        const float a = v.x - kk[j], b = v.y - kk[j], c = v.z - kk[j], d = v.w - kk[j];
        const float sum = half32_sum_hi(nv ? (a + b) + (c + d) : 0.f);
        const float sq = half32_sum_hi(nv ? (a * a + b * b) + (c * c + d * d) : 0.f);
        if (wj == j) mine = make_float2(sum, sq);
      }
    }
    if (LNF && writer) {
      int mw = mm[0];
#pragma unroll
      for (int j = 1; j < RB; ++j) mw = wj == j ? mm[j] : mw;
      if (mw < M) e.ln_part[(size_t)mw * e.ln_npart + (n >> 7)] = mine;
    }
  }
}

template <int ROWS, int COLS, int NT, int LN = LN_NONE, typename RowMap>
__device__ __forceinline__ void drain_tile(const char* sm, int pitch, const GemmEpi& e, const ColParams& cp, int M, int N,
                                           int n0, int tid, RowMap rowmap) {
  constexpr int C4 = COLS / 4;
  static_assert(NT % C4 == 0, "a thread must keep its column group");
  static_assert(C4 % 32 == 0, "a 128-column statistics group is 32 lanes of one wave");
  const int c4 = tid % C4;
  const int n = n0 + 4 * c4;
  if (n >= N && LN != LN_PROD) return;
  if (e.resid && e.out_f32 && e.rows_per_img == 0 && !e.a_scale && (!e.a_bs || e.w_bs)) {
    constexpr int STEP = NT / C4, ITER = ROWS / STEP;
    static_assert(ROWS % STEP == 0, "whole passes over the tile rows");
    constexpr int RBD = ITER % 4 == 0 ? 4 : (ITER % 2 == 0 ? 2 : 1);
    drain_resid<RBD, STEP, ITER, C4, LN == LN_PROD>(sm, pitch, e, cp, M, N, n, c4, tid, rowmap);
    return;
  }
  if (n >= N) return;
#pragma unroll
  for (int row_l = tid / C4; row_l < ROWS; row_l += NT / C4) {
    const int m = rowmap(row_l);
    if (m >= M) continue;
    float4 v = *reinterpret_cast<const float4*>(sm + row_l * pitch + c4 * 16);
    if (e.a_scale || e.a_bs) {
      const float sa = e.a_scale ? e.a_scale[m] : 1.0f;
      v.x *= sa * cp.wscale.x; v.y *= sa * cp.wscale.y; v.z *= sa * cp.wscale.z; v.w *= sa * cp.wscale.w;
    }
    if (LN == LN_CONS) {
      const float2 st = *reinterpret_cast<const float2*>(sm + row_l * pitch + C4 * 16);
      v.x = fmaf(-st.x, cp.scale.x, v.x) * st.y; v.y = fmaf(-st.x, cp.scale.y, v.y) * st.y;
      v.z = fmaf(-st.x, cp.scale.z, v.z) * st.y; v.w = fmaf(-st.x, cp.scale.w, v.w) * st.y;
    }
    v.x += cp.bias.x; v.y += cp.bias.y; v.z += cp.bias.z; v.w += cp.bias.w;
    if (e.act == ACT_GELU) { gelu_fast4(v); }
    else if (e.act == ACT_RELU) { v.x = fmaxf(v.x, 0.f); v.y = fmaxf(v.y, 0.f); v.z = fmaxf(v.z, 0.f); v.w = fmaxf(v.w, 0.f); }
    if (LN != LN_CONS) { v.x *= cp.scale.x; v.y *= cp.scale.y; v.z *= cp.scale.z; v.w *= cp.scale.w; }
    size_t orow = (size_t)m;
    if (e.rows_per_img > 0) {
      const int b = m / e.rows_per_img, p = m - b * e.rows_per_img;
      orow = (size_t)b * e.out_rows_per_img + 1 + p;
      const float4 p4 = *reinterpret_cast<const float4*>(e.pos + (size_t)(1 + p) * N + n);
      v.x += p4.x; v.y += p4.y; v.z += p4.z; v.w += p4.w;
    }
    if (e.resid) {
      const float4 r4 = *reinterpret_cast<const float4*>(e.resid + orow * e.ldr + n);
      v.x += r4.x; v.y += r4.y; v.z += r4.z; v.w += r4.w;
    }
    if (e.out_f32) {
      *reinterpret_cast<float4*>(e.out_f32 + orow * e.ldc + n) = v;
    } else if (e.glu) {
      const float g0 = silu_mul(v.x, v.y), g1 = silu_mul(v.z, v.w);
      const unsigned hi = pack2bf(g0, g1);
      bf16_t* og = e.out_bf16 + orow * e.ldc + (n >> 1);
      *reinterpret_cast<unsigned*>(og) = hi;
      if (e.out_split < 0) *reinterpret_cast<unsigned*>(og - e.out_split) = pack2bf(g0 - __uint_as_float(hi << 16), g1 - __uint_as_float(hi & 0xffff0000u));
    } else if (e.out_h2) {
      uint2 f16; unsigned hi8, lo8;
      h2_quad(v, 1.0f, f16, hi8, lo8);
      char* row = reinterpret_cast<char*>(e.out_bf16) + orow * (size_t)e.ldc * 2;
      *reinterpret_cast<uint2*>(row + 2 * n) = f16;
      char* p8 = row + h2_off8(N, n);
      *reinterpret_cast<unsigned*>(p8) = hi8;
      *reinterpret_cast<unsigned*>(p8 + 16) = lo8;
    } else if (e.out_split > 0) {
      uint2 hi, lo;
      hi.x = pack2bf(v.x, v.y);
      hi.y = pack2bf(v.z, v.w);
      lo.x = pack2bf(v.x - __uint_as_float(hi.x << 16), v.y - __uint_as_float(hi.x & 0xffff0000u));
      lo.y = pack2bf(v.z - __uint_as_float(hi.y << 16), v.w - __uint_as_float(hi.y & 0xffff0000u));
      bf16_t* o = e.out_bf16 + orow * e.ldc + n;
      *reinterpret_cast<uint2*>(o) = hi;
      *reinterpret_cast<uint2*>(o + e.out_split) = hi;
      *reinterpret_cast<uint2*>(o + 2 * (size_t)e.out_split) = lo;
    } else if (e.out_split < 0) {
      uint2 hi, lo;
      hi.x = pack2bf(v.x, v.y);
      hi.y = pack2bf(v.z, v.w);
      lo.x = pack2bf(v.x - __uint_as_float(hi.x << 16), v.y - __uint_as_float(hi.x & 0xffff0000u));
      lo.y = pack2bf(v.z - __uint_as_float(hi.y << 16), v.w - __uint_as_float(hi.y & 0xffff0000u));
      bf16_t* o = e.out_bf16 + orow * e.ldc + n;
      *reinterpret_cast<uint2*>(o) = hi;
      *reinterpret_cast<uint2*>(o - e.out_split) = lo;
    } else {
      uint2 o;
      o.x = pack2bf(v.x, v.y);
      o.y = pack2bf(v.z, v.w);
      *reinterpret_cast<uint2*>(e.out_bf16 + orow * e.ldc + n) = o;
    }
  }
}


__host__ __device__ __forceinline__ bool drain8_ok(const GemmEpi& e, int N) {
  return e.out_bf16 && e.out_split <= 0 && !e.resid && e.rows_per_img == 0 && !e.a_scale && (!e.a_bs || e.w_bs) && !e.out_bs && (N & 7) == 0 && (e.ldc & 7) == 0 &&
         (e.out_split == 0 || ((-e.out_split) & 7) == 0);
}
template <int ROWS, int COLS, int NT, int LN = LN_NONE, typename RowMap>
__device__ __forceinline__ void drain_tile_bf16x8(const char* sm, int pitch, const GemmEpi& e, int M, int N, int n0, int tid, RowMap rowmap) {
  constexpr int C8 = COLS / 8;
  static_assert(NT % C8 == 0, "a thread must keep its column group");
  const int c8 = tid % C8;
  const int n = n0 + 8 * c8;
  if (n >= N) return;
  float4 b0 = make_float4(0.f, 0.f, 0.f, 0.f), b1 = b0, s0 = make_float4(1.f, 1.f, 1.f, 1.f), s1 = s0;
  if (e.bias) { b0 = *reinterpret_cast<const float4*>(e.bias + n); b1 = *reinterpret_cast<const float4*>(e.bias + n + 4); }
  constexpr bool ln = LN == LN_CONS;
  const float* sc = ln ? e.ln_c : e.scale;
  if (sc) { s0 = *reinterpret_cast<const float4*>(sc + n); s1 = *reinterpret_cast<const float4*>(sc + n + 4); }
#pragma unroll
  for (int row_l = tid / C8; row_l < ROWS; row_l += NT / C8) {
    const int m = rowmap(row_l);
    if (m >= M) continue;
    float4 v = *reinterpret_cast<const float4*>(sm + row_l * pitch + c8 * 32);
    float4 u = *reinterpret_cast<const float4*>(sm + row_l * pitch + c8 * 32 + 16);
    if (ln) {
      const float2 st = *reinterpret_cast<const float2*>(sm + row_l * pitch + COLS * 4);
      const f32x2_t t = (f32x2_t)(-st.x * st.y), rs = (f32x2_t)(st.y);
#define LN_PAIR_(va, vb, ca, cb, ba, bb)                                                                         \
      { const f32x2_t c_ = {ca, cb}, b_ = {ba, bb}, a_ = {va, vb};                                                \
        const f32x2_t o_ = __builtin_elementwise_fma(a_, rs, __builtin_elementwise_fma(t, c_, b_));               \
        va = o_.x; vb = o_.y; }
      LN_PAIR_(v.x, v.y, s0.x, s0.y, b0.x, b0.y) LN_PAIR_(v.z, v.w, s0.z, s0.w, b0.z, b0.w)
      LN_PAIR_(u.x, u.y, s1.x, s1.y, b1.x, b1.y) LN_PAIR_(u.z, u.w, s1.z, s1.w, b1.z, b1.w)
#undef LN_PAIR_
    } else {
      v.x += b0.x; v.y += b0.y; v.z += b0.z; v.w += b0.w;
      u.x += b1.x; u.y += b1.y; u.z += b1.z; u.w += b1.w;
    }
    if (e.act == ACT_GELU) {
      gelu_fast4(v); gelu_fast4(u);
    } else if (e.act == ACT_RELU) {
      v.x = fmaxf(v.x, 0.f); v.y = fmaxf(v.y, 0.f); v.z = fmaxf(v.z, 0.f); v.w = fmaxf(v.w, 0.f);
      u.x = fmaxf(u.x, 0.f); u.y = fmaxf(u.y, 0.f); u.z = fmaxf(u.z, 0.f); u.w = fmaxf(u.w, 0.f);
    }
    if (!ln) {
      v.x *= s0.x; v.y *= s0.y; v.z *= s0.z; v.w *= s0.w;
      u.x *= s1.x; u.y *= s1.y; u.z *= s1.z; u.w *= s1.w;
    }
    if (e.glu) {
      const float4 gq = make_float4(silu_mul(v.x, v.y), silu_mul(v.z, v.w), silu_mul(u.x, u.y), silu_mul(u.z, u.w));
      const int nh = n >> 1;
      if (e.out_h2) {
        uint2 f16; unsigned hi8, lo8;
        h2_quad(gq, 1.0f, f16, hi8, lo8);
        char* row = reinterpret_cast<char*>(e.out_bf16) + (size_t)m * e.ldc * 2;
        *reinterpret_cast<uint2*>(row + 2 * nh) = f16;
        char* p8 = row + h2_off8(N >> 1, nh);
        *reinterpret_cast<unsigned*>(p8) = hi8;
        *reinterpret_cast<unsigned*>(p8 + 16) = lo8;
        continue;
      }
      uint2 g;
      g.x = pack2bf(gq.x, gq.y);
      g.y = pack2bf(gq.z, gq.w);
      bf16_t* og = e.out_bf16 + (size_t)m * e.ldc + nh;
      *reinterpret_cast<uint2*>(og) = g;
      if (e.out_split < 0) {
        uint2 lo;
        lo.x = pack2bf(gq.x - __uint_as_float(g.x << 16), gq.y - __uint_as_float(g.x & 0xffff0000u));
        lo.y = pack2bf(gq.z - __uint_as_float(g.y << 16), gq.w - __uint_as_float(g.y & 0xffff0000u));
        *reinterpret_cast<uint2*>(og - e.out_split) = lo;
      }
      continue;
    }
    if (e.out_h2) {
      uint2 fa, fb; unsigned h0, l0, h1, l1;
      h2_quad(v, 1.0f, fa, h0, l0);
      h2_quad(u, 1.0f, fb, h1, l1);
      char* row = reinterpret_cast<char*>(e.out_bf16) + (size_t)m * e.ldc * 2;
      *reinterpret_cast<uint4*>(row + 2 * n) = make_uint4(fa.x, fa.y, fb.x, fb.y);
      char* p8 = row + h2_off8(N, n);
      *reinterpret_cast<uint2*>(p8) = make_uint2(h0, h1);
      *reinterpret_cast<uint2*>(p8 + 16) = make_uint2(l0, l1);
      continue;
    }
    uint4 hi;
    hi.x = pack2bf(v.x, v.y); hi.y = pack2bf(v.z, v.w); hi.z = pack2bf(u.x, u.y); hi.w = pack2bf(u.z, u.w);
    bf16_t* o = e.out_bf16 + (size_t)m * e.ldc + n;
    *reinterpret_cast<uint4*>(o) = hi;
    if (e.out_split < 0) {
      uint4 lo;
      lo.x = pack2bf(v.x - __uint_as_float(hi.x << 16), v.y - __uint_as_float(hi.x & 0xffff0000u));
      lo.y = pack2bf(v.z - __uint_as_float(hi.y << 16), v.w - __uint_as_float(hi.y & 0xffff0000u));
      lo.z = pack2bf(u.x - __uint_as_float(hi.z << 16), u.y - __uint_as_float(hi.z & 0xffff0000u));
      lo.w = pack2bf(u.z - __uint_as_float(hi.w << 16), u.w - __uint_as_float(hi.w & 0xffff0000u));
      *reinterpret_cast<uint4*>(o - e.out_split) = lo;
    }
  }
}

inline bool epi_regmath_ok(const GemmEpi& e, int N) {
  return drain8_ok(e, N) && e.out_split == 0 && !e.out_h2 && !e.glu && !e.ln_part && (!e.ln_part_in || (e.ln_npart >= 1 && e.ln_npart <= 8)) &&
         (e.act == ACT_NONE || e.act == ACT_RELU || e.act == ACT_GELU);
}
template <int LN>
__device__ __forceinline__ uint2 epi_quad_bf16(float4 v, const float4& c, const float4& b, float t1, float rs1, int act) {
  if (LN == LN_CONS) {
    const f32x2_t t = (f32x2_t)(t1), rs = (f32x2_t)(rs1);
#define LN_PAIR_(va, vb, ca, cb, ba, bb)                                                                         \
      { const f32x2_t c_ = {ca, cb}, b_ = {ba, bb}, a_ = {va, vb};                                                \
        const f32x2_t o_ = __builtin_elementwise_fma(a_, rs, __builtin_elementwise_fma(t, c_, b_));               \
        va = o_.x; vb = o_.y; }
    LN_PAIR_(v.x, v.y, c.x, c.y, b.x, b.y) LN_PAIR_(v.z, v.w, c.z, c.w, b.z, b.w)
#undef LN_PAIR_
  } else {
    v.x += b.x; v.y += b.y; v.z += b.z; v.w += b.w;
  }
  if (act == ACT_GELU) {
    gelu_fast4(v);
  } else if (act == ACT_RELU) {
    v.x = fmaxf(v.x, 0.f); v.y = fmaxf(v.y, 0.f); v.z = fmaxf(v.z, 0.f); v.w = fmaxf(v.w, 0.f);
  }
  if (LN != LN_CONS) { v.x *= c.x; v.y *= c.y; v.z *= c.z; v.w *= c.w; }
  return make_uint2(pack2bf(v.x, v.y), pack2bf(v.z, v.w));
}
__device__ __forceinline__ int epi_tile_w8(int row, int col) { return row * 512 + (((col >> 2) ^ (row & 15)) << 3); }
__device__ __forceinline__ uint4 epi_tile_r16(const char* sm, int row, int c8) {
  const uint4 q = *reinterpret_cast<const uint4*>(sm + row * 512 + ((c8 ^ ((row >> 1) & 7)) << 4));
  return (row & 1) ? make_uint4(q.z, q.w, q.x, q.y) : q;
}
```

dinov2_od_amd/csrc/gemm_pp.hip:

```cpp
#include <atomic>
#include <mutex>
#include "dod_common.h"
#include "gemm_epi.h"
#include <cstdlib>
#include <cstring>

#define PPM 256
#define PPN 256
#define PPK 64
#define PP_PLANE (256 * 64)
#define PP_TILE (4 * PP_PLANE)

__device__ __forceinline__ int pp_swz(int row, int chunk) { return chunk ^ (((row >> 3) & 1) << 1); }


#ifdef DINODET_TUNING
__device__ unsigned long long* g_pp_stamps = nullptr;
extern "C" int dod_debug_pp_stamps(void* dev_buf) {
  unsigned long long* p = (unsigned long long*)dev_buf;
  return hipMemcpyToSymbol(HIP_SYMBOL(g_pp_stamps), &p, sizeof(p)) == hipSuccess ? 0 : 3;
}
#define PP_STAMPS_DECL unsigned long long* const stamps = g_pp_stamps;
#else
#define PP_STAMPS_DECL unsigned long long* const stamps = nullptr;
#endif

template <bool X3, bool DC, int LN>
__global__ __launch_bounds__(512) void gemm_ppm_256x256_kernel(const bf16_t* __restrict__ A, int lda,
                                                               const bf16_t* __restrict__ W, int ldw, int M, int N,
                                                               int K, GemmEpi e_, int GM) {
  extern __shared__ __attribute__((aligned(16))) char smem[];
  const int tid = threadIdx.x, lane = tid & 63, wid = tid >> 6;
  const int wu = __builtin_amdgcn_readfirstlane(wid);
  const int grp_ = wu >> 2, wq = wu & 3;
  const int tiles_m = (M + PPM - 1) / PPM, tiles_n = (N + PPN - 1) / PPN;
  PP_STAMPS_DECL
  unsigned long long ts0 = 0, ts1 = 0, ts2 = 0, tr0 = 0;
  if (stamps) { ts0 = __builtin_amdgcn_s_memtime(); tr0 = __builtin_amdgcn_s_memrealtime(); }
  int tm, tn;
  tile_map(blockIdx.x, tiles_m, tiles_n, GM, &tm, &tn);
  if (tm < 0) return;
  const int m0 = tm * PPM, n0 = tn * PPN;
  const int Kl = e_.ksplit > 1 ? e_.kslice_len : K;
  const int kbase = e_.ksplit > 1 ? (int)blockIdx.y * Kl : 0;
  GemmEpi e = e_;
  if (e_.ksplit > 1) e.out_f32 = e_.out_f32 + (size_t)blockIdx.y * (size_t)e_.kslice_stride;
  typedef __attribute__((address_space(1))) const void* gptr_t;
  typedef __attribute__((address_space(3))) void* lptr_t;
  unsigned vA0, vA1, vW0, vW1;
  {
    const int rl = wid * 32 + (lane >> 2);
    const int c = pp_swz(rl, lane & 3);
    int ra0 = m0 + rl, ra1 = m0 + rl + 16; ra0 = ra0 < M ? ra0 : M - 1; ra1 = ra1 < M ? ra1 : M - 1;
    int rw0 = n0 + rl, rw1 = n0 + rl + 16; rw0 = rw0 < N ? rw0 : N - 1; rw1 = rw1 < N ? rw1 : N - 1;
    vA0 = (unsigned)(((size_t)ra0 * lda + c * 8) * 2); vA1 = (unsigned)(((size_t)ra1 * lda + c * 8) * 2);
    vW0 = (unsigned)(((size_t)rw0 * ldw + c * 8) * 2); vW1 = (unsigned)(((size_t)rw1 * ldw + c * 8) * 2);
  }
  const size_t bytesA = (size_t)M * lda * 2, bytesW = (size_t)N * ldw * 2;
  const __amdgpu_buffer_rsrc_t rA = __builtin_amdgcn_make_buffer_rsrc((void*)A, 0, (int)(bytesA > 0xfffffff0u ? 0xfffffff0u : bytesA), 0x00020000);
  const __amdgpu_buffer_rsrc_t rW = __builtin_amdgcn_make_buffer_rsrc((void*)W, 0, (int)(bytesW > 0xfffffff0u ? 0xfffffff0u : bytesW), 0x00020000);
  char* const sdst = smem + wu * 2048;
  constexpr int KT = X3 ? 32 : 64;
  const int pl1 = X3 ? K : 32;
#define PPM_STAGE_H(t, pl, hh)                                                                                 \
  {                                                                                                            \
    char* d_ = sdst + ((t) & 1) * PP_TILE + (pl) * PP_PLANE + (hh) * 1024;                                     \
    const int ko_ = (kbase + (t) * KT + (((pl) & 1) ? pl1 : 0)) * 2;                                                   \
    if ((pl) < 2) __builtin_amdgcn_raw_ptr_buffer_load_lds(rA, (lptr_t)(d_), 16, (hh) ? vA1 : vA0, ko_, 0, 0); \
    else __builtin_amdgcn_raw_ptr_buffer_load_lds(rW, (lptr_t)(d_), 16, (hh) ? vW1 : vW0, ko_, 0, 0);          \
  }
#define PPM_STAGE(t, pl) { PPM_STAGE_H(t, pl, 0) PPM_STAGE_H(t, pl, 1) }
  f32x4 acc[8][4];
#pragma unroll
  for (int i = 0; i < 8; ++i)
#pragma unroll
    for (int j = 0; j < 4; ++j) acc[i][j] = f32x4{0.f, 0.f, 0.f, 0.f};
  const int nk = Kl / KT;
  const int l15 = lane & 15, l4 = lane >> 4;
  int offA[8], offW[4];
#pragma unroll
  for (int i = 0; i < 8; ++i) { const int row = grp_ * 128 + i * 16 + l15; offA[i] = row * 64 + pp_swz(row, l4) * 16; }
#pragma unroll
  for (int j = 0; j < 4; ++j) { const int row = wq * 64 + j * 16 + l15; offW[j] = 2 * PP_PLANE + row * 64 + pp_swz(row, l4) * 16; }

  PPM_STAGE(0, 0) PPM_STAGE(0, 1) PPM_STAGE(0, 2) PPM_STAGE(0, 3)
  if (nk > 1) { PPM_STAGE(1, 2) PPM_STAGE(1, 3) }
  if (nk > 1) asm volatile("s_waitcnt vmcnt(4)" ::: "memory"); else asm volatile("s_waitcnt vmcnt(0)" ::: "memory");
  __builtin_amdgcn_s_barrier();
  if (grp_ == 1) __builtin_amdgcn_s_barrier();
  asm volatile("" ::: "memory");

  if (stamps) ts1 = __builtin_amdgcn_s_memtime();
  bf16x8 w0[4], w1[4], a0[2], a1[2];
#define PPM_PHASE(st, q, PF_ON, PF_T, PF_PL, VW)                                                               \
  {                                                                                                            \
    if ((q) == 0) {                                                                                            \
      _Pragma("unroll") for (int j = 0; j < 4; ++j) {                                                          \
        w0[j] = *reinterpret_cast<const bf16x8*>((st) + offW[j]);                                              \
        w1[j] = *reinterpret_cast<const bf16x8*>((st) + offW[j] + PP_PLANE);                                   \
      }                                                                                                        \
    }                                                                                                          \
    _Pragma("unroll") for (int ii = 0; ii < 2; ++ii) {                                                         \
      a0[ii] = *reinterpret_cast<const bf16x8*>((st) + offA[2 * (q) + ii]);                                    \
      a1[ii] = *reinterpret_cast<const bf16x8*>((st) + offA[2 * (q) + ii] + PP_PLANE);                         \
    }                                                                                                          \
    if (!DC && (PF_ON)) PPM_STAGE(PF_T, PF_PL)                                                                 \
    if ((VW) == 4) { if (DC) asm volatile("s_waitcnt vmcnt(2)" ::: "memory"); else asm volatile("s_waitcnt vmcnt(4)" ::: "memory"); } \
    else if ((VW) == 0) asm volatile("s_waitcnt vmcnt(0)" ::: "memory");                                       \
    asm volatile("s_waitcnt lgkmcnt(0)" ::: "memory");                                                         \
    __builtin_amdgcn_sched_barrier(0);                                                                         \
    __builtin_amdgcn_s_barrier();                                                                              \
    __builtin_amdgcn_sched_barrier(0);                                                                         \
    __builtin_amdgcn_s_setprio(1);                                                                             \
    _Pragma("unroll") for (int ii = 0; ii < 2; ++ii)                                                           \
      _Pragma("unroll") for (int j = 0; j < 4; ++j) {                                                          \
        if (DC && (PF_ON) && j == 1) {                                                                         \
          __builtin_amdgcn_sched_barrier(0);                                                                   \
          PPM_STAGE_H(PF_T, PF_PL, ii)                                                                         \
          __builtin_amdgcn_sched_barrier(0);                                                                   \
        }                                                                                                      \
        f32x4 c_ = acc[2 * (q) + ii][j];                                                                       \
        if (X3) {                                                                                              \
          c_ = __builtin_amdgcn_mfma_f32_16x16x32_bf16(w1[j], a0[ii], c_, 0, 0, 0);    \
          c_ = __builtin_amdgcn_mfma_f32_16x16x32_bf16(w0[j], a1[ii], c_, 0, 0, 0);                 \
          c_ = __builtin_amdgcn_mfma_f32_16x16x32_bf16(w0[j], a0[ii], c_, 0, 0, 0);                 \
        } else {                                                                                               \
          c_ = __builtin_amdgcn_mfma_f32_16x16x32_bf16(w0[j], a0[ii], c_, 0, 0, 0);               \
          c_ = __builtin_amdgcn_mfma_f32_16x16x32_bf16(w1[j], a1[ii], c_, 0, 0, 0);              \
        }                                                                                                      \
        acc[2 * (q) + ii][j] = c_;                                                                             \
      }                                                                                                        \
    __builtin_amdgcn_s_setprio(0);                                                                             \
    __builtin_amdgcn_sched_barrier(0);                                                                         \
    __builtin_amdgcn_s_barrier();                                                                              \
    __builtin_amdgcn_sched_barrier(0);                                                                         \
  }

  int u = 0;
  for (; u + 2 < nk; ++u) {
    const char* st = smem + (u & 1) * PP_TILE;
    PPM_PHASE(st, 0, true, u + 1, 0, -1)
    PPM_PHASE(st, 1, true, u + 1, 1, -1)
    PPM_PHASE(st, 2, true, u + 2, 2, -1)
    PPM_PHASE(st, 3, true, u + 2, 3, 4)
  }
  if (u + 1 < nk) {
    const char* st = smem + (u & 1) * PP_TILE;
    PPM_PHASE(st, 0, true, u + 1, 0, -1)
    PPM_PHASE(st, 1, true, u + 1, 1, -1)
    PPM_PHASE(st, 2, false, 0, 0, -1)
    PPM_PHASE(st, 3, false, 0, 0, 0)
    ++u;
  }
  {
    const char* st = smem + (u & 1) * PP_TILE;
    PPM_PHASE(st, 0, false, 0, 0, -1)
    PPM_PHASE(st, 1, false, 0, 0, -1)
    PPM_PHASE(st, 2, false, 0, 0, -1)
    PPM_PHASE(st, 3, false, 0, 0, -1)
  }
  if (grp_ == 0) __builtin_amdgcn_s_barrier();
  asm volatile("" ::: "memory");
  if (stamps) ts2 = __builtin_amdgcn_s_memtime();

  constexpr int PITCH = PPN * 4 + 16;
  const ColParams cp = load_col_params<PPN, LN>(e, n0, N, tid);
  const bool wide = drain8_ok(e, N);
#pragma unroll
  for (int pass = 0; pass < 2; ++pass) {
    if (pass) __syncthreads();
#pragma unroll
    for (int ii = 0; ii < 4; ++ii)
#pragma unroll
      for (int j = 0; j < 4; ++j) {
        const int row_l = grp_ * 64 + ii * 16 + l15;
        const int col = wq * 64 + j * 16 + 4 * l4;
        const f32x4 a = acc[pass * 4 + ii][j];
        *reinterpret_cast<float4*>(smem + row_l * PITCH + col * 4) = make_float4(a[0], a[1], a[2], a[3]);
      }
    auto rowmap = [&](int row_l) { return m0 + (row_l >> 6) * 128 + pass * 64 + (row_l & 63); };
    stage_row_stats<128, PPN, LN>(smem, PITCH, e, M, tid, rowmap, K, n0);
    __syncthreads();
    if (wide) drain_tile_bf16x8<128, PPN, 512, LN>(smem, PITCH, e, M, N, n0, tid, rowmap);
    else drain_tile<128, PPN, 512, LN>(smem, PITCH, e, cp, M, N, n0, tid, rowmap);
  }
  if (stamps && tid == 0) {
    asm volatile("s_waitcnt vmcnt(0)" ::: "memory");
    unsigned long long* o = stamps + (size_t)blockIdx.x * 8;
    o[0] = ts0; o[1] = ts1; o[2] = ts2; o[3] = __builtin_amdgcn_s_memtime(); o[4] = tr0; o[5] = __builtin_amdgcn_s_memrealtime(); o[6] = blockIdx.x; o[7] = 0;
  }
}


__device__ __forceinline__ int h2_swz(int row, int chunk) { return chunk ^ ((row >> 2) & 3); }
typedef __attribute__((ext_vector_type(8))) int i32x8_;
typedef __attribute__((ext_vector_type(4))) int i32x4_;
typedef __attribute__((ext_vector_type(2))) short s16x2_;
#define H2_ABUF (32 * 1024)
#define H2_A8 (16 * 1024)
#define H2_WBASE (3 * H2_ABUF)
#define H2_WBUF (24 * 1024)
#define H2_WL (16 * 1024)
#define H2_LDS (H2_WBASE + 2 * H2_WBUF)

__device__ __forceinline__ void h2_cvt8(const bf16x8& raw, float inv_scale, int& d0, int& d1) {
  const f16x8 v = __builtin_bit_cast(f16x8, raw);
  s16x2_ r0 = {0, 0}, r1 = {0, 0};
  r0 = __builtin_amdgcn_cvt_scalef32_pk_fp8_f16(r0, f16x2{v[0], v[1]}, inv_scale, false);
  r0 = __builtin_amdgcn_cvt_scalef32_pk_fp8_f16(r0, f16x2{v[2], v[3]}, inv_scale, true);
  r1 = __builtin_amdgcn_cvt_scalef32_pk_fp8_f16(r1, f16x2{v[4], v[5]}, inv_scale, false);
  r1 = __builtin_amdgcn_cvt_scalef32_pk_fp8_f16(r1, f16x2{v[6], v[7]}, inv_scale, true);
  d0 = __builtin_bit_cast(int, r0); d1 = __builtin_bit_cast(int, r1);
}

template <int LN>
__global__ __launch_bounds__(512) void gemm_h2_256x256_kernel(const char* __restrict__ A, int lda, const char* __restrict__ W, int ldw,
                                                              int M, int N, int K, GemmEpi e_, int GM) {
  extern __shared__ __attribute__((aligned(16))) char smem[];
  const int tid = threadIdx.x, lane = tid & 63, wid = tid >> 6;
  const int wu = __builtin_amdgcn_readfirstlane(wid);
  const int grp_ = wu >> 2, wq = wu & 3;
  const int tiles_m = (M + PPM - 1) / PPM, tiles_n = (N + PPN - 1) / PPN;
  PP_STAMPS_DECL
  unsigned long long ts0 = 0, ts1 = 0, ts2 = 0, tr0 = 0;
  if (stamps) { ts0 = __builtin_amdgcn_s_memtime(); tr0 = __builtin_amdgcn_s_memrealtime(); }
  int tm, tn;
  tile_map(blockIdx.x, tiles_m, tiles_n, GM, &tm, &tn);
  const int m0 = tm * PPM, n0 = tn * PPN;
  const int Kl = e_.ksplit > 1 ? e_.kslice_len : K;
  const int kb = e_.ksplit > 1 ? (int)blockIdx.y * (Kl / 32) : 0;
  GemmEpi e = e_;
  if (e_.ksplit > 1) e.out_f32 = e_.out_f32 + (size_t)blockIdx.y * (size_t)e_.kslice_stride;
  typedef __attribute__((address_space(3))) void* lptr_t;
  unsigned vA0, vA1, vW0, vW1, vWl;
  {
    const int rl = wid * 32 + (lane >> 2);
    const int c = h2_swz(rl, lane & 3);
    int ra0 = m0 + rl, ra1 = m0 + rl + 16; ra0 = ra0 < M ? ra0 : M - 1; ra1 = ra1 < M ? ra1 : M - 1;
    int rw0 = n0 + rl, rw1 = n0 + rl + 16; rw0 = rw0 < N ? rw0 : N - 1; rw1 = rw1 < N ? rw1 : N - 1;
    vA0 = (unsigned)((size_t)ra0 * lda + c * 16); vA1 = (unsigned)((size_t)ra1 * lda + c * 16);
    vW0 = (unsigned)((size_t)rw0 * ldw + c * 16); vW1 = (unsigned)((size_t)rw1 * ldw + c * 16);
    const int r2 = wid * 32 + (lane >> 1);
    int rwl = n0 + r2; rwl = rwl < N ? rwl : N - 1;
    vWl = (unsigned)((size_t)rwl * ldw + 2 * (size_t)K + (((lane & 1) ^ ((r2 >> 3) & 1)) * 16));
  }
  const size_t bytesA = (size_t)M * lda, bytesW = (size_t)N * ldw;
  const __amdgpu_buffer_rsrc_t rA = __builtin_amdgcn_make_buffer_rsrc((void*)A, 0, (int)(bytesA > 0xfffffff0u ? 0xfffffff0u : bytesA), 0x00020000);
  const __amdgpu_buffer_rsrc_t rW = __builtin_amdgcn_make_buffer_rsrc((void*)W, 0, (int)(bytesW > 0xfffffff0u ? 0xfffffff0u : bytesW), 0x00020000);
  const int K2 = 2 * K;
#define H2_STAGE_A(t, ab)                                                                                      \
  {                                                                                                            \
    char* b_ = smem + (ab) * H2_ABUF + wu * 2048;                                                              \
    __builtin_amdgcn_raw_ptr_buffer_load_lds(rA, (lptr_t)(b_), 16, vA0, (kb + (t)) * 64, 0, 0);                       \
    __builtin_amdgcn_raw_ptr_buffer_load_lds(rA, (lptr_t)(b_ + 1024), 16, vA1, (kb + (t)) * 64, 0, 0);                \
    __builtin_amdgcn_raw_ptr_buffer_load_lds(rA, (lptr_t)(b_ + H2_A8), 16, vA0, K2 + (kb + (t)) * 64, 0, 0);          \
    __builtin_amdgcn_raw_ptr_buffer_load_lds(rA, (lptr_t)(b_ + H2_A8 + 1024), 16, vA1, K2 + (kb + (t)) * 64, 0, 0);   \
  }
#define H2_STAGE_W(t)                                                                                          \
  {                                                                                                            \
    char* b_ = smem + H2_WBASE + ((t) & 1) * H2_WBUF;                                                          \
    __builtin_amdgcn_raw_ptr_buffer_load_lds(rW, (lptr_t)(b_ + wu * 2048), 16, vW0, (kb + (t)) * 64, 0, 0);           \
    __builtin_amdgcn_raw_ptr_buffer_load_lds(rW, (lptr_t)(b_ + wu * 2048 + 1024), 16, vW1, (kb + (t)) * 64, 0, 0);    \
    __builtin_amdgcn_raw_ptr_buffer_load_lds(rW, (lptr_t)(b_ + H2_WL + wu * 1024), 16, vWl, (kb + (t)) * 32, 0, 0);   \
  }
  f32x16 acc[4][2];
#pragma unroll
  for (int i = 0; i < 4; ++i)
#pragma unroll
    for (int j = 0; j < 2; ++j)
#pragma unroll
      for (int r = 0; r < 16; ++r) acc[i][j][r] = 0.f;
  const int nk = Kl / 32;
  const int lr = lane & 31, lg = lane >> 5;
  int offA[4], offW[2], offWl[2];
#pragma unroll
  for (int i = 0; i < 4; ++i) { const int row = grp_ * 128 + i * 32 + lr; offA[i] = row * 64 + h2_swz(row, 2 * lg) * 16; }
#pragma unroll
  for (int j = 0; j < 2; ++j) {
    const int row = wq * 64 + j * 32 + lr;
    offW[j] = row * 64 + h2_swz(row, 2 * lg) * 16;
    offWl[j] = H2_WL + row * 32 + ((lg ^ ((row >> 3) & 1)) * 16);
  }
  int sc_w; float cinv[2];
  {
    int na = n0 + wq * 64 + lr, nb = na + 32;
    na = na < N ? na : N - 1; nb = nb < N ? nb : N - 1;
    const int ba = (int)e.h2_wexp[na], bb = (int)e.h2_wexp[nb];
    cinv[0] = __uint_as_float((unsigned)ba << 23); cinv[1] = __uint_as_float((unsigned)bb << 23);
    sc_w = (ba - 11 < 0 ? 0 : ba - 11) | ((bb - 11 < 0 ? 0 : bb - 11) << 8);
  }
  const int sc_a = 127;

  H2_STAGE_A(0, 0) H2_STAGE_W(0)
  if (nk > 1) { H2_STAGE_A(1, 1) H2_STAGE_W(1) }
  if (nk > 1) asm volatile("s_waitcnt vmcnt(7)" ::: "memory"); else asm volatile("s_waitcnt vmcnt(0)" ::: "memory");
  __builtin_amdgcn_s_barrier();
  if (grp_ == 1) __builtin_amdgcn_s_barrier();
  asm volatile("" ::: "memory");
  if (stamps) ts1 = __builtin_amdgcn_s_memtime();

  bf16x8 w16[2][2], wl[2], a16[2][2], a8[2][2];
  i32x8_ w8v[2];
#define H2_PHASE(sa, sw, p, PF, PF_T, PF_AB, VW)                                                               \
  {                                                                                                            \
    if ((p) == 0) {                                                                                            \
      _Pragma("unroll") for (int j = 0; j < 2; ++j) {                                                          \
        w16[j][0] = *reinterpret_cast<const bf16x8*>((sw) + offW[j]);                                          \
        w16[j][1] = *reinterpret_cast<const bf16x8*>((sw) + (offW[j] ^ 16));                                   \
        wl[j] = *reinterpret_cast<const bf16x8*>((sw) + offWl[j]);                                             \
      }                                                                                                        \
    }                                                                                                          \
    _Pragma("unroll") for (int ii = 0; ii < 2; ++ii) {                                                         \
      a16[ii][0] = *reinterpret_cast<const bf16x8*>((sa) + offA[2 * (p) + ii]);                                \
      a16[ii][1] = *reinterpret_cast<const bf16x8*>((sa) + (offA[2 * (p) + ii] ^ 16));                         \
      a8[ii][0] = *reinterpret_cast<const bf16x8*>((sa) + offA[2 * (p) + ii] + H2_A8);                         \
      a8[ii][1] = *reinterpret_cast<const bf16x8*>((sa) + (offA[2 * (p) + ii] ^ 16) + H2_A8);                  \
    }                                                                                                          \
    if ((PF) == 1) H2_STAGE_A(PF_T, PF_AB)                                                                     \
    if ((PF) == 2) H2_STAGE_W(PF_T)                                                                            \
    if ((VW) == 7) asm volatile("s_waitcnt vmcnt(7)" ::: "memory");                                            \
    else if ((VW) == 0) asm volatile("s_waitcnt vmcnt(0)" ::: "memory");                                       \
    asm volatile("s_waitcnt lgkmcnt(0)" ::: "memory");                                                         \
    __builtin_amdgcn_sched_barrier(0);                                                                         \
    __builtin_amdgcn_s_barrier();                                                                              \
    __builtin_amdgcn_sched_barrier(0);                                                                         \
    __builtin_amdgcn_s_setprio(1);                                                                             \
    _Pragma("unroll") for (int ii = 0; ii < 2; ++ii)                                                           \
      _Pragma("unroll") for (int j = 0; j < 2; ++j) {                                                          \
        f32x16 c_ = acc[2 * (p) + ii][j];                                                                      \
        c_ = __builtin_amdgcn_mfma_f32_32x32x16_f16(__builtin_bit_cast(f16x8, w16[j][0]), __builtin_bit_cast(f16x8, a16[ii][0]), c_, 0, 0, 0); \
        c_ = __builtin_amdgcn_mfma_f32_32x32x16_f16(__builtin_bit_cast(f16x8, w16[j][1]), __builtin_bit_cast(f16x8, a16[ii][1]), c_, 0, 0, 0); \
        acc[2 * (p) + ii][j] = c_;                                                                             \
      }                                                                                                        \
    if ((p) == 0) {         \
      _Pragma("unroll") for (int j = 0; j < 2; ++j) {                                                          \
        int d0, d1, d2, d3;                                                                                    \
        h2_cvt8(w16[j][0], cinv[j], d0, d1);                                                                   \
        h2_cvt8(w16[j][1], cinv[j], d2, d3);                                                                   \
        const i32x4_ l_ = __builtin_bit_cast(i32x4_, wl[j]);                                                   \
        w8v[j] = i32x8_{l_[0], l_[1], l_[2], l_[3], d0, d1, d2, d3};                                           \
      }                                                                                                        \
    }                                                                                                          \
    _Pragma("unroll") for (int ii = 0; ii < 2; ++ii) {                                                         \
      const i32x8_ a8v = __builtin_shufflevector(__builtin_bit_cast(i32x4_, a8[ii][0]), __builtin_bit_cast(i32x4_, a8[ii][1]), 0, 1, 2, 3, 4, 5, 6, 7); \
      acc[2 * (p) + ii][0] = __builtin_amdgcn_mfma_scale_f32_32x32x64_f8f6f4(w8v[0], a8v, acc[2 * (p) + ii][0], 0, 0, 0, sc_w, 0, sc_a); \
      acc[2 * (p) + ii][1] = __builtin_amdgcn_mfma_scale_f32_32x32x64_f8f6f4(w8v[1], a8v, acc[2 * (p) + ii][1], 0, 0, 1, sc_w, 0, sc_a); \
    }                                                                                                          \
    __builtin_amdgcn_s_setprio(0);                                                                             \
    __builtin_amdgcn_sched_barrier(0);                                                                         \
    __builtin_amdgcn_s_barrier();                                                                              \
    __builtin_amdgcn_sched_barrier(0);                                                                         \
  }

  int u = 0, ua = 0;
  for (; u + 2 < nk; ++u) {
    const char* sa = smem + ua * H2_ABUF;
    const char* sw = smem + H2_WBASE + (u & 1) * H2_WBUF;
    const int ab2 = ua == 0 ? 2 : ua - 1;
    H2_PHASE(sa, sw, 0, 1, u + 2, ab2, -1)
    H2_PHASE(sa, sw, 1, 2, u + 2, 0, 7)
    ua = ua == 2 ? 0 : ua + 1;
  }
  if (u + 1 < nk) {
    const char* sa = smem + ua * H2_ABUF;
    const char* sw = smem + H2_WBASE + (u & 1) * H2_WBUF;
    H2_PHASE(sa, sw, 0, 0, 0, 0, -1)
    H2_PHASE(sa, sw, 1, 0, 0, 0, 0)
    ua = ua == 2 ? 0 : ua + 1;
    ++u;
  }
  {
    const char* sa = smem + ua * H2_ABUF;
    const char* sw = smem + H2_WBASE + (u & 1) * H2_WBUF;
    H2_PHASE(sa, sw, 0, 0, 0, 0, -1)
    H2_PHASE(sa, sw, 1, 0, 0, 0, -1)
  }
  if (grp_ == 0) __builtin_amdgcn_s_barrier();
  asm volatile("" ::: "memory");
  if (stamps) ts2 = __builtin_amdgcn_s_memtime();

  constexpr int PITCH = PPN * 4 + 16;
  const ColParams cp = load_col_params<PPN, LN>(e, n0, N, tid);
  const bool wide = drain8_ok(e, N);
#pragma unroll
  for (int pass = 0; pass < 2; ++pass) {
    if (pass) __syncthreads();
#pragma unroll
    for (int ii = 0; ii < 2; ++ii)
#pragma unroll
      for (int j = 0; j < 2; ++j) stage_acc(smem, PITCH, grp_ * 64 + ii * 32 + lr, wq * 64 + j * 32, acc[pass * 2 + ii][j], lg);
    auto rowmap = [&](int row_l) { return m0 + (row_l >> 6) * 128 + pass * 64 + (row_l & 63); };
    stage_row_stats<128, PPN, LN>(smem, PITCH, e, M, tid, rowmap, K, n0);
    __syncthreads();
    if (wide) drain_tile_bf16x8<128, PPN, 512, LN>(smem, PITCH, e, M, N, n0, tid, rowmap);
    else drain_tile<128, PPN, 512, LN>(smem, PITCH, e, cp, M, N, n0, tid, rowmap);
  }
  if (stamps && tid == 0) {
    asm volatile("s_waitcnt vmcnt(0)" ::: "memory");
    unsigned long long* o = stamps + (size_t)blockIdx.x * 8;
    o[0] = ts0; o[1] = ts1; o[2] = ts2; o[3] = __builtin_amdgcn_s_memtime(); o[4] = tr0; o[5] = __builtin_amdgcn_s_memrealtime(); o[6] = blockIdx.x; o[7] = 0;
  }
}


static constexpr int LDSPP = (128 * (PPN * 4 + 16)) > 2 * PP_TILE ? (128 * (PPN * 4 + 16)) : 2 * PP_TILE;

#ifdef DINODET_TUNING
static int wres_grid(int M, int N, int* gm) {
  const int tiles_m = (M + PPM - 1) / PPM, tiles_n = (N + PPN - 1) / PPN;
  const char* v = getenv("DINODET_GEMM_WRES");
  if (v && v[0] == '1' && tiles_n % 2 == 0 && tiles_m >= 32) { *gm = (*gm & ~0x300) | 0x400; return 8 * ((tiles_m + 3) / 4) * (tiles_n / 2); }
  return tiles_m * tiles_n;
}
#else
static int wres_grid(int M, int N, int*) { return ((M + PPM - 1) / PPM) * ((N + PPN - 1) / PPN); }
#endif

static void ppm_attr() {
  static bool attr_set[16] = {};
  int dev = 0;
  (void)hipGetDevice(&dev);
  if (dev >= 0 && dev < 16 && !attr_set[dev]) {
#define ATTR_(LN_) (void)hipFuncSetAttribute(reinterpret_cast<const void*>(gemm_ppm_256x256_kernel<false, false, LN_>), hipFuncAttributeMaxDynamicSharedMemorySize, LDSPP); \
                   (void)hipFuncSetAttribute(reinterpret_cast<const void*>(gemm_ppm_256x256_kernel<true, false, LN_>), hipFuncAttributeMaxDynamicSharedMemorySize, LDSPP);
    ATTR_(LN_NONE) ATTR_(LN_CONS) ATTR_(LN_PROD)
#undef ATTR_
    attr_set[dev] = true;
  }
}

int launch_gemm_bf16_ppm(const bf16_t* A, int lda, const bf16_t* W, int ldw, int M, int N, int K, const GemmEpi& e, hipStream_t s) {
  if (M <= 0 || N <= 0 || K <= 0 || K % PPK != 0) return 2;
  if (N % 4 != 0 || lda % 8 != 0 || ldw % 8 != 0 || e.ldc % 4 != 0) return 2;
  if (e.resid && e.ldr % 4 != 0) return 2;
  if (!e.out_f32 && !e.out_bf16) return 2;
  ppm_attr();
  int gm = gemm_tile_mode();
  const int tiles = wres_grid(M, N, &gm);
  gemm_form_launched(FORM_PPM);
#define GO_(LN_) hipLaunchKernelGGL((gemm_ppm_256x256_kernel<false, false, LN_>), dim3(tiles), dim3(512), LDSPP, s, A, lda, W, ldw, M, N, K, e, gm);
  LN_DISPATCH(e, GO_)
#undef GO_
  return hipGetLastError() == hipSuccess ? 0 : 3;
}

int launch_gemm_x3_pp(const bf16_t* A2, int lda, const bf16_t* W2, int ldw, int M, int N, int K, const GemmEpi& e, hipStream_t s) {
  if (M <= 0 || N <= 0 || K <= 0) return 1;
  if (K % 32 != 0 || N % 4 != 0 || lda % 8 != 0 || ldw % 8 != 0 || lda < 2 * K || ldw < 2 * K) return 2;
  if (e.out_f32 && e.ldc % 4 != 0) return 2;
  if (e.resid && e.ldr % 4 != 0) return 2;
  if (!e.out_f32 && !e.out_bf16) return 2;
  ppm_attr();
  int gm = gemm_tile_mode();
  const int tiles = wres_grid(M, N, &gm);
  gemm_form_launched(FORM_X3_PP);
#define GO_(LN_) hipLaunchKernelGGL((gemm_ppm_256x256_kernel<true, false, LN_>), dim3(tiles), dim3(512), LDSPP, s, A2, lda, W2, ldw, M, N, K, e, gm);
  LN_DISPATCH(e, GO_)
#undef GO_
  return hipGetLastError() == hipSuccess ? 0 : 3;
}

static constexpr int LDSH2 = (128 * (PPN * 4 + 16)) > H2_LDS ? (128 * (PPN * 4 + 16)) : H2_LDS;
static void h2_attr() {
  static bool attr_set[16] = {};
  int dev = 0;
  (void)hipGetDevice(&dev);
  if (dev >= 0 && dev < 16 && !attr_set[dev]) {
    (void)hipFuncSetAttribute(reinterpret_cast<const void*>(gemm_h2_256x256_kernel<LN_NONE>), hipFuncAttributeMaxDynamicSharedMemorySize, LDSH2);
    (void)hipFuncSetAttribute(reinterpret_cast<const void*>(gemm_h2_256x256_kernel<LN_CONS>), hipFuncAttributeMaxDynamicSharedMemorySize, LDSH2);
    (void)hipFuncSetAttribute(reinterpret_cast<const void*>(gemm_h2_256x256_kernel<LN_PROD>), hipFuncAttributeMaxDynamicSharedMemorySize, LDSH2);
    attr_set[dev] = true;
  }
}
int launch_gemm_h2(const void* A, int lda, const void* W, int ldw, int M, int N, int K, const GemmEpi& e, hipStream_t s) {
  if (M <= 0 || N <= 0 || K <= 0) return 1;
  if (K % 32 != 0 || N % 4 != 0 || lda % 16 != 0 || ldw % 16 != 0 || lda < 4 * K || ldw < 3 * K || !e.h2_wexp) return 2;
  if (e.out_f32 && e.ldc % 4 != 0) return 2;
  if (e.resid && e.ldr % 4 != 0) return 2;
  if (!e.out_f32 && !e.out_bf16) return 2;
  { const int No = e.glu ? N / 2 : N;
    if (e.out_h2 && (No % 32 != 0 || e.ldc < 2 * No || e.ldc % 8 != 0 || e.out_split != 0)) return 2;
    if (e.glu && e.out_h2 && (N % 8 != 0)) return 2; }
  { const int t = gemm_tail_split(2, A, lda, W, ldw, M, N, K, e, s); if (t >= 0) return t; }
  h2_attr();
  const int gm = gemm_tile_mode();
  const int tiles = ((M + PPM - 1) / PPM) * ((N + PPN - 1) / PPN);
  gemm_form_launched(FORM_H2);
#define GO_(LN_) hipLaunchKernelGGL(gemm_h2_256x256_kernel<LN_>, dim3(tiles), dim3(512), LDSH2, s, (const char*)A, lda, (const char*)W, ldw, M, N, K, e, gm);
  LN_DISPATCH(e, GO_)
#undef GO_
  return hipGetLastError() == hipSuccess ? 0 : 3;
}

#define KSR_ROWS 16
template <int LN>
__global__ __launch_bounds__(512) void gemm_ksplit_reduce_kernel(const float* __restrict__ part, long long slice_stride, int S, int R, int N,
                                                                 GemmEpi e, int m_base, int M, int K) {
  __shared__ __attribute__((aligned(16))) char smem[KSR_ROWS * (PPN * 4 + 16)];
  constexpr int PITCH = PPN * 4 + 16;
  const int tid = threadIdx.x;
  const int r0 = blockIdx.x * KSR_ROWS, n0 = blockIdx.y * PPN;
  const int c4 = tid & 63;
#pragma unroll
  for (int rl = tid >> 6; rl < KSR_ROWS; rl += 8) {
    const int r = r0 + rl, n = n0 + 4 * c4;
    float4 acc = make_float4(0.f, 0.f, 0.f, 0.f);
    if (r < R && n < N) {
      const float* p = part + (size_t)r * N + n;
      for (int sl = 0; sl < S; ++sl) {
        const float4 v = *reinterpret_cast<const float4*>(p + (size_t)sl * slice_stride);
        acc.x += v.x; acc.y += v.y; acc.z += v.z; acc.w += v.w;
      }
    }
    *reinterpret_cast<float4*>(smem + rl * PITCH + c4 * 16) = acc;
  }
  auto rowmap = [&](int row_l) { return m_base + r0 + row_l; };
  stage_row_stats<KSR_ROWS, PPN, LN>(smem, PITCH, e, M, tid, rowmap, K, n0);
  __syncthreads();
  const ColParams cp = load_col_params<PPN, LN>(e, n0, N, tid);
  if (drain8_ok(e, N)) drain_tile_bf16x8<KSR_ROWS, PPN, 512, LN>(smem, PITCH, e, M, N, n0, tid, rowmap);
  else drain_tile<KSR_ROWS, PPN, 512, LN>(smem, PITCH, e, cp, M, N, n0, tid, rowmap);
}

#define TAIL_SLOTS 4
#define TAIL_GENS 4
static std::mutex g_tail_mu;
static float* g_tail_scratch[16][TAIL_GENS] = {};
static int g_tail_gen[16] = {};
static size_t g_tail_bytes[16] = {};
static hipStream_t g_tail_owner[16][TAIL_SLOTS] = {};
static unsigned long long g_tail_used[16][TAIL_SLOTS] = {};
static unsigned long long g_tail_clock = 0;
int gemm_tail_reserve(size_t bytes) {
  int dev = 0;
  if (hipGetDevice(&dev) != hipSuccess || dev < 0 || dev >= 16) return 3;
  std::lock_guard<std::mutex> lk(g_tail_mu);
  if (g_tail_bytes[dev] >= bytes) return 0;
  if (g_tail_gen[dev] >= TAIL_GENS) return 3;
  float* blk = nullptr;
  if (hipMalloc((void**)&blk, bytes * TAIL_SLOTS) != hipSuccess) return 3;
  g_tail_scratch[dev][g_tail_gen[dev]++] = blk;
  for (int i = 0; i < TAIL_SLOTS; ++i) { g_tail_used[dev][i] = 0; g_tail_owner[dev][i] = nullptr; }
  g_tail_bytes[dev] = bytes;
  return 0;
}
static float* tail_slab(int dev, hipStream_t s) {
  std::lock_guard<std::mutex> lk(g_tail_mu);
  if (!g_tail_gen[dev]) return nullptr;
  int pick = -1;
  for (int i = 0; i < TAIL_SLOTS; ++i)
    if (g_tail_used[dev][i] && g_tail_owner[dev][i] == s) { pick = i; break; }
  if (pick < 0) {
    pick = 0;
    for (int i = 1; i < TAIL_SLOTS; ++i)
      if (g_tail_used[dev][i] < g_tail_used[dev][pick]) pick = i;
    g_tail_owner[dev][pick] = s;
  }
  g_tail_used[dev][pick] = ++g_tail_clock;
  return (float*)((char*)g_tail_scratch[dev][g_tail_gen[dev] - 1] + (size_t)pick * g_tail_bytes[dev]);
}

static int tail_mode() {
  const int m = dod_option(DOD_OPT_TAILSPLIT);
  if (m >= 0) return m;
  static const char* env = DOD_TUNE_ENV("DINODET_GEMM_TAILSPLIT");
  return env ? (env[0] == '0' ? 0 : (env[0] == '2' ? 2 : 1)) : 1;
}

static thread_local bool t_in_tail_split = false;
static std::atomic<long> g_tail_splits{0};
long gemm_tail_split_count() { return g_tail_splits.load(); }
int gemm_tail_split(int kind, const void* A, int lda, const void* W, int ldw, int M, int N, int K, const GemmEpi& e, hipStream_t s) {
  if (t_in_tail_split || e.ksplit > 1 || e.rows_per_img != 0 || e.a_scale || e.out_split > 0) return -1;
  const int mode = tail_mode();
  if (mode == 0) return -1;
  const int ktile = kind == 0 ? 64 : 32;
  if (N % 4 != 0 || K % ktile != 0) return -1;
  int dev = 0;
  if (hipGetDevice(&dev) != hipSuccess || dev < 0 || dev >= 16) return -1;
  static int cus[16] = {};
  if (!cus[dev]) { int c = 0; (void)hipDeviceGetAttribute(&c, hipDeviceAttributeMultiprocessorCount, dev); cus[dev] = c > 0 ? c : 256; }
  const int CU = cus[dev];
  const int tiles_n = (N + PPN - 1) / PPN, tiles_m = (M + PPM - 1) / PPM, tiles = tiles_m * tiles_n;
  const int nk = K / ktile;
  const bool force = mode == 2;
  int Mmain, R, tiles_r, S = 0;
  static const int k0frac = [] { const char* v = DOD_TUNE_ENV("DINODET_GEMM_KSPLIT0"); return v ? atoi(v) : 0; }();
  if (M >= 2048 && (kind >= 1 ? tiles * 2 <= CU + CU / 8 : tiles * 12 <= CU * k0frac)) {
    Mmain = 0; R = M; tiles_r = tiles;
    for (int c : {8, 6, 4, 3, 2})
      if (nk % c == 0 && nk / c >= 3 && tiles_r * c <= CU) { S = c; break; }
  } else {
    const int rounds = tiles / CU, rem = tiles % CU;
    const bool shallow = kind >= 1 && M >= 4096 && rounds >= 1 && rounds <= 2 && rem * 16 >= CU && rem * 6 <= CU;
    if (M < 8192 && !shallow) return -1;
    if (!force && !shallow && (K < 2048 || M < 65536)) return -1;
    if (rounds < 1 || rounds > 6 || rem == 0) return -1;
    const int m_main = (rounds * CU) / tiles_n;
    Mmain = m_main * PPM; R = M - Mmain;
    if (R <= 0) return -1;
    tiles_r = ((R + PPM - 1) / PPM) * tiles_n;
    for (int c : {8, 6, 4, 3, 2})
      if (nk % c == 0 && nk / c >= 3 && tiles_r * c <= CU) { S = c; break; }
    if (S >= 2 && (1.0 - 1.0 / S - 0.25) < 0.04 * (rounds + 1)) S = 0;
  }
  if (S < 2) return -1;
  const size_t slab = (size_t)R * N;
  if (g_tail_bytes[dev] < slab * S * 4) return -1;
  float* scratch = tail_slab(dev, s);
  if (!scratch) return -1;
  if (Mmain > 0) {
    t_in_tail_split = true;
    int rc;
    if (kind == 0) rc = launch_gemm_bf16((const bf16_t*)A, lda, (const bf16_t*)W, ldw, Mmain, N, K, e, s);
    else if (kind == 1) rc = launch_gemm_x3((const bf16_t*)A, lda, (const bf16_t*)W, ldw, Mmain, N, K, e, s);
    else rc = launch_gemm_h2(A, lda, W, ldw, Mmain, N, K, e, s);
    t_in_tail_split = false;
    if (rc) return rc;
  }
  GemmEpi es; memset(&es, 0, sizeof es);
  es.out_f32 = scratch; es.ldc = N; es.h2_wexp = e.h2_wexp;
  es.ksplit = S; es.kslice_len = K / S; es.kslice_stride = (long long)slab;
  const int gm = gemm_tile_mode() & 0xfff;
  gemm_form_launched(kind == 2 ? FORM_H2 : (kind == 1 ? FORM_X3_PP : FORM_PPM));
  if (kind == 2) {
    h2_attr();
    const char* Ar = (const char*)A + (size_t)Mmain * lda;
    hipLaunchKernelGGL(gemm_h2_256x256_kernel<LN_NONE>, dim3(tiles_r, S), dim3(512), LDSH2, s, Ar, lda, (const char*)W, ldw, R, N, K, es, gm);
  } else {
    ppm_attr();
    const bf16_t* Ar = (const bf16_t*)A + (size_t)Mmain * lda;
    if (kind == 1) hipLaunchKernelGGL((gemm_ppm_256x256_kernel<true, false, LN_NONE>), dim3(tiles_r, S), dim3(512), LDSPP, s, Ar, lda, (const bf16_t*)W, ldw, R, N, K, es, gm);
    else hipLaunchKernelGGL((gemm_ppm_256x256_kernel<false, false, LN_NONE>), dim3(tiles_r, S), dim3(512), LDSPP, s, Ar, lda, (const bf16_t*)W, ldw, R, N, K, es, gm);
  }
  if (hipGetLastError() != hipSuccess) return 3;
  ++g_tail_splits;
#define GO_(LN_) hipLaunchKernelGGL(gemm_ksplit_reduce_kernel<LN_>, dim3((R + KSR_ROWS - 1) / KSR_ROWS, tiles_n), dim3(512), 0, s, scratch, (long long)slab, S, R, N, e, Mmain, M, K);
  LN_DISPATCH(e, GO_)
#undef GO_
  return hipGetLastError() == hipSuccess ? 0 : 3;
}
```

dinov2_od_amd/csrc/gemm_x3.hip:

```cpp
#include "dod_common.h"
#include "gemm_epi.h"
#include <atomic>
#include <cstdio>
#include <cstdlib>

#define X3M 256
#define X3N 256
#define X3K 32
#define X3_PLANE (256 * X3K * 2)
#define X3_STAGE (4 * X3_PLANE)
#define X3_SLOTS 2

__device__ __forceinline__ int x3_swz(int row, int chunk) { return chunk ^ (((row >> 3) & 1) << 1); }

#define X3_PAR (X3_SLOTS * X3_STAGE)

template <int LN, int ACT>
__device__ __forceinline__ void x3_epi_regs(char* smem, const f32x4 (&acc)[4][4], const GemmEpi& e, int M, int N, int m0, int n0, int tid) {
  const int lane = tid & 63, wid = tid >> 6, wm = wid >> 2, wn = wid & 3, l15 = lane & 15, l4 = lane >> 4;
  const int c8 = tid & 31, nd = n0 + 8 * c8;
#define X3_LDS_SYNC asm volatile("s_waitcnt lgkmcnt(0)" ::: "memory"); __builtin_amdgcn_s_barrier(); asm volatile("" ::: "memory");
#define X3_MATH(I0)                                                                                                    \
  {                                                                                                                    \
    float tt[2], rr[2];                                                                                                \
    _Pragma("unroll") for (int ii = 0; ii < 2; ++ii) {                                                                 \
      float2 st = make_float2(0.f, 0.f);                                                                               \
      if (LN == LN_CONS) st = *reinterpret_cast<const float2*>(smem + X3_PAR + (wm * 64 + ((I0) + ii) * 16 + l15) * 8); \
      tt[ii] = -st.x * st.y; rr[ii] = st.y;                                                                            \
    }                                                                                                                  \
    _Pragma("unroll") for (int j = 0; j < 4; ++j) {                                                                    \
      const int col = wn * 64 + j * 16 + 4 * l4;                                                                       \
      const float4 b4 = *reinterpret_cast<const float4*>(smem + X3_PAR + 2048 + col * 4);                              \
      const float4 c4 = *reinterpret_cast<const float4*>(smem + X3_PAR + 3072 + col * 4);                              \
      _Pragma("unroll") for (int ii = 0; ii < 2; ++ii) {                                                               \
        const f32x4 a = acc[(I0) + ii][j];                                                                             \
        const uint2 o = epi_quad_bf16<LN>(make_float4(a[0], a[1], a[2], a[3]), c4, b4, tt[ii], rr[ii], ACT);           \
        *reinterpret_cast<uint2*>(smem + epi_tile_w8(wm * 64 + ((I0) + ii) * 16 + l15, col)) = o;                      \
      }                                                                                                                \
    }                                                                                                                  \
  }
#define X3_COPY(P)                                     \
  {                                                                                                                    \
    uint4 q[4];                                                                                                        \
    _Pragma("unroll") for (int it = 0; it < 4; ++it) q[it] = epi_tile_r16(smem, it * 64 + (P) * 32 + (tid >> 5), c8);  \
    _Pragma("unroll") for (int it = 0; it < 4; ++it) {                                                                 \
      const int row = it * 64 + (P) * 32 + (tid >> 5);                                                                 \
      if (nd < N && m0 + row < M) *reinterpret_cast<uint4*>(e.out_bf16 + (size_t)(m0 + row) * e.ldc + nd) = q[it];     \
    }                                                                                                                  \
  }
  X3_LDS_SYNC
  X3_MATH(0)
  X3_LDS_SYNC
  if (LN == LN_CONS && n0 == 0 && tid < 256 && m0 + tid < M && e.ln_part_in && e.ln_stats_out)
    e.ln_stats_out[m0 + tid] = *reinterpret_cast<const float2*>(smem + X3_PAR + tid * 8);
  X3_COPY(0)
  X3_MATH(2)
  X3_LDS_SYNC
  X3_COPY(1)
#undef X3_MATH
#undef X3_COPY
#undef X3_LDS_SYNC
}

template <bool PLAIN, int LN, bool REGM = false>
__global__ __launch_bounds__(1024) void gemm_x3_256x256_kernel(const bf16_t* __restrict__ A2, int lda,
                                                               const bf16_t* __restrict__ W2, int ldw, int M, int N,
                                                               int K, GemmEpi e, int GM) {
  extern __shared__ __attribute__((aligned(16))) char smem[];
  const int tid = threadIdx.x, lane = tid & 63, wid = tid >> 6;
  const int wm = wid >> 2, wn = wid & 3;
  const int tiles_m = (M + X3M - 1) / X3M, tiles_n = (N + X3N - 1) / X3N;
  int tm, tn;
  tile_map(blockIdx.x, tiles_m, tiles_n, GM, &tm, &tn);
  const int m0 = tm * X3M, n0 = tn * X3N;
  typedef __attribute__((address_space(1))) const void* gptr_t;
  typedef __attribute__((address_space(3))) void* lptr_t;
  unsigned vA, vW;
  {
    const int rl = wid * 16 + (lane >> 2);
    const int c = x3_swz(rl, lane & 3);
    int ra = m0 + rl; ra = ra < M ? ra : M - 1;
    int rw = n0 + rl; rw = rw < N ? rw : N - 1;
    vA = (unsigned)(((size_t)ra * lda + c * 8) * 2);
    vW = (unsigned)(((size_t)rw * ldw + c * 8) * 2);
  }
  const size_t bytesA = (size_t)M * lda * 2, bytesW = (size_t)N * ldw * 2;
  const __amdgpu_buffer_rsrc_t rA = __builtin_amdgcn_make_buffer_rsrc((void*)A2, 0, (int)(bytesA > 0xfffffff0u ? 0xfffffff0u : bytesA), 0x00020000);
  const __amdgpu_buffer_rsrc_t rW = __builtin_amdgcn_make_buffer_rsrc((void*)W2, 0, (int)(bytesW > 0xfffffff0u ? 0xfffffff0u : bytesW), 0x00020000);
  const int wu = __builtin_amdgcn_readfirstlane(wid);
  const int pl1b = (PLAIN ? 32 : K) * 2;
#define STAGE_X3(slot_, k0)                                                                                \
  {                                                                                                        \
    char* s_ = smem + (slot_) * X3_STAGE + wu * 1024;                                                      \
    const int kb_ = (k0) * 2;                                                                              \
    __builtin_amdgcn_raw_ptr_buffer_load_lds(rA, (lptr_t)(s_), 16, vA, kb_, 0, 0);                         \
    __builtin_amdgcn_raw_ptr_buffer_load_lds(rA, (lptr_t)(s_ + X3_PLANE), 16, vA, kb_ + pl1b, 0, 0);       \
    __builtin_amdgcn_raw_ptr_buffer_load_lds(rW, (lptr_t)(s_ + 2 * X3_PLANE), 16, vW, kb_, 0, 0);          \
    __builtin_amdgcn_raw_ptr_buffer_load_lds(rW, (lptr_t)(s_ + 3 * X3_PLANE), 16, vW, kb_ + pl1b, 0, 0);   \
  }
  f32x4 acc[4][4];
#pragma unroll
  for (int i = 0; i < 4; ++i)
#pragma unroll
    for (int j = 0; j < 4; ++j) acc[i][j] = f32x4{0.f, 0.f, 0.f, 0.f};
  constexpr int KSTEP = PLAIN ? 2 * X3K : X3K;
  const int nk = K / KSTEP;
  const int l15 = lane & 15, l4 = lane >> 4;
  unsigned long long st_r = 0, pg_r[8];
  float b_e = 0.f, c_e = 1.f;
  if constexpr (REGM) {
    if (tid < 256) {
      const int nc = n0 + tid < N ? n0 + tid : N - 1;
      const float* sc = LN == LN_CONS ? e.ln_c : e.scale;
      if (e.bias) b_e = e.bias[nc];
      if (sc) c_e = sc[nc];
      if (LN == LN_CONS) {
        const int mc = m0 + tid < M ? m0 + tid : M - 1;
        st_r = reinterpret_cast<const unsigned long long*>(e.ln_stats)[mc];
        const unsigned long long* p = reinterpret_cast<const unsigned long long*>(e.ln_part_in ? e.ln_part_in + (size_t)mc * e.ln_npart : e.ln_stats + mc);
        const int gl = e.ln_part_in ? e.ln_npart - 1 : 0;
#pragma unroll
        for (int g = 0; g < 8; ++g) pg_r[g] = p[g < gl ? g : gl];
      }
    }
  }
  STAGE_X3(0, 0)
  int offA[4], offW[4];
#pragma unroll
  for (int i = 0; i < 4; ++i) { const int row = wm * 64 + i * 16 + l15; offA[i] = row * 64 + x3_swz(row, l4) * 16; }
#pragma unroll
  for (int j = 0; j < 4; ++j) { const int row = wn * 64 + j * 16 + l15; offW[j] = 2 * X3_PLANE + row * 64 + x3_swz(row, l4) * 16; }
#define X3_KTILE(kt)                                                                                         \
  {                                                                                                          \
    if ((kt) + 1 < nk) STAGE_X3(((kt) + 1) & 1, ((kt) + 1) * KSTEP)                                          \
    const char* st = smem + ((kt) & 1) * X3_STAGE;                                                           \
    bf16x8 wh[4], wl[4];                                                                                     \
    _Pragma("unroll") for (int j = 0; j < 4; ++j) {                                                          \
      wh[j] = *reinterpret_cast<const bf16x8*>(st + offW[j]);                                                \
      wl[j] = *reinterpret_cast<const bf16x8*>(st + offW[j] + X3_PLANE);                                     \
    }                                                                                                        \
    _Pragma("unroll") for (int i = 0; i < 4; ++i) {                                                          \
      const bf16x8 ah = *reinterpret_cast<const bf16x8*>(st + offA[i]);                                      \
      const bf16x8 al = *reinterpret_cast<const bf16x8*>(st + offA[i] + X3_PLANE);                           \
      _Pragma("unroll") for (int j = 0; j < 4; ++j) {                                                        \
        if (PLAIN) {                                                                                         \
          acc[i][j] = __builtin_amdgcn_mfma_f32_16x16x32_bf16(wh[j], ah, acc[i][j], 0, 0, 0);     \
          acc[i][j] = __builtin_amdgcn_mfma_f32_16x16x32_bf16(wl[j], al, acc[i][j], 0, 0, 0);    \
        } else {                                                                                             \
          acc[i][j] = __builtin_amdgcn_mfma_f32_16x16x32_bf16(wl[j], ah, acc[i][j], 0, 0, 0);    \
          acc[i][j] = __builtin_amdgcn_mfma_f32_16x16x32_bf16(wh[j], al, acc[i][j], 0, 0, 0);                \
          acc[i][j] = __builtin_amdgcn_mfma_f32_16x16x32_bf16(wh[j], ah, acc[i][j], 0, 0, 0);                \
        }                                                                                                    \
      }                                                                                                      \
    }                                                                                                        \
  }
  int kt0 = 0;
  if constexpr (REGM) {
    asm volatile("s_waitcnt vmcnt(0)" ::: "memory");
    __builtin_amdgcn_s_barrier();
    asm volatile("" ::: "memory");
    if (tid < 256) {
      asm volatile("" : "+v"(b_e), "+v"(c_e), "+v"(st_r));
      if (LN == LN_CONS) {
#pragma unroll
        for (int g = 0; g < 8; ++g) asm volatile("" : "+v"(pg_r[g]));
      }
      float2 st_e = make_float2(__uint_as_float((unsigned)st_r), __uint_as_float((unsigned)(st_r >> 32)));
      if (n0 + tid >= N) { b_e = 0.f; c_e = 1.f; }
      if (LN == LN_CONS) {
        if (m0 + tid >= M) {
          st_e = make_float2(0.f, 0.f);
        } else if (e.ln_part_in) {
          float S = 0.f, Q = 0.f;
#pragma unroll
          for (int g = 0; g < 8; ++g)
            if (g < e.ln_npart) { S += __uint_as_float((unsigned)pg_r[g]); Q += __uint_as_float((unsigned)(pg_r[g] >> 32)); }
          const float dm = S / (float)K;
          st_e = make_float2(st_e.x + dm, 1.0f / sqrtf(fmaxf(Q / (float)K - dm * dm, 0.f) + e.ln_eps));
        }
        *reinterpret_cast<float2*>(smem + X3_PAR + tid * 8) = st_e;
      }
      *reinterpret_cast<float*>(smem + X3_PAR + 2048 + tid * 4) = b_e;
      *reinterpret_cast<float*>(smem + X3_PAR + 3072 + tid * 4) = c_e;
    }
    asm volatile("" ::: "memory");
    X3_KTILE(0)
    kt0 = 1;
  }
  for (int kt = kt0; kt < nk; ++kt) {
    asm volatile("s_waitcnt vmcnt(0)" ::: "memory");
    __builtin_amdgcn_s_barrier();
    asm volatile("" ::: "memory");
    X3_KTILE(kt)
  }
#undef X3_KTILE
  if constexpr (REGM) {
    if (e.act == ACT_GELU) x3_epi_regs<LN, ACT_GELU>(smem, acc, e, M, N, m0, n0, tid);
    else if (e.act == ACT_RELU) x3_epi_regs<LN, ACT_RELU>(smem, acc, e, M, N, m0, n0, tid);
    else x3_epi_regs<LN, ACT_NONE>(smem, acc, e, M, N, m0, n0, tid);
    return;
  }
  constexpr int PITCH = X3N * 4 + 16;
  const ColParams cp = load_col_params<X3N, LN>(e, n0, N, tid);
  const bool wide = drain8_ok(e, N);
#define X3_PASS(P)                                                                                                          \
  {                                                                                                                         \
    __builtin_amdgcn_s_barrier();                                                                                           \
    asm volatile("" ::: "memory");                                                                                          \
    _Pragma("unroll") for (int ii = 0; ii < 2; ++ii)                                                                        \
      _Pragma("unroll") for (int j = 0; j < 4; ++j) {                                                                       \
        const int row_l = wm * 32 + ii * 16 + l15;                                                                          \
        const int col = wn * 64 + j * 16 + 4 * l4;                                                                          \
        const f32x4 a = acc[(P) * 2 + ii][j];                                                                               \
        *reinterpret_cast<float4*>(smem + row_l * PITCH + col * 4) = make_float4(a[0], a[1], a[2], a[3]);                   \
      }                                                                                                                     \
    auto rowmap = [&](int row_l) { return m0 + (row_l >> 5) * 64 + (P) * 32 + (row_l & 31); };                              \
    stage_row_stats<128, X3N, LN>(smem, PITCH, e, M, tid, rowmap, K, n0);                                                          \
    __syncthreads();                                                                                                        \
    if (wide) drain_tile_bf16x8<128, X3N, 1024, LN>(smem, PITCH, e, M, N, n0, tid, rowmap);                                 \
    else drain_tile<128, X3N, 1024, LN>(smem, PITCH, e, cp, M, N, n0, tid, rowmap);                                         \
  }
  X3_PASS(0)
  X3_PASS(1)
#undef X3_PASS
}

int gemm_tile_mode() {
  const char* g = DOD_TUNE_ENV("DINODET_GEMM_GM");
  const char* o = DOD_TUNE_ENV("DINODET_GEMM_ORDER");
  int gm = g ? atoi(g) : 4;
  if (gm < 1 || gm > 64) gm = 4;
  const int ord = o ? atoi(o) : 2;
  int st = 0;
  if (const char* sg = DOD_TUNE_ENV("DINODET_GEMM_STAGGER")) {
    int G = 0; float us = 0.f;
    if (sscanf(sg, "%d,%f", &G, &us) == 2 && G >= 2 && G <= 16 && us > 0.f) {
      int step = (int)(us / 0.16f + 0.5f); step = step < 1 ? 1 : (step > 0xfff ? 0xfff : step);
      st = ((G - 1) << 12) | (step << 16);
    }
  }
  return gm | ((ord & 1) ? 0x100 : 0) | ((ord & 2) ? 0x200 : 0) | st;
}

static constexpr int LDSX3 = (128 * (X3N * 4 + 16)) > X3_SLOTS * X3_STAGE ? (128 * (X3N * 4 + 16)) : X3_SLOTS * X3_STAGE;
static constexpr int LDSX3E = X3_PAR + 4096;

static void x3_attr() {
  static bool attr_set[16] = {};
  int dev = 0;
  (void)hipGetDevice(&dev);
  if (dev >= 0 && dev < 16 && !attr_set[dev]) {
#define ATTR_(LN_) (void)hipFuncSetAttribute(reinterpret_cast<const void*>(gemm_x3_256x256_kernel<false, LN_>), hipFuncAttributeMaxDynamicSharedMemorySize, LDSX3); \
                   (void)hipFuncSetAttribute(reinterpret_cast<const void*>(gemm_x3_256x256_kernel<true, LN_>), hipFuncAttributeMaxDynamicSharedMemorySize, LDSX3);
    ATTR_(LN_NONE) ATTR_(LN_CONS) ATTR_(LN_PROD)
#undef ATTR_
#define ATTR_(LN_) (void)hipFuncSetAttribute(reinterpret_cast<const void*>(gemm_x3_256x256_kernel<true, LN_, true>), hipFuncAttributeMaxDynamicSharedMemorySize, LDSX3E);
    ATTR_(LN_NONE) ATTR_(LN_CONS)
#undef ATTR_
    attr_set[dev] = true;
  }
}

int launch_gemm_x3(const bf16_t* A2, int lda, const bf16_t* W2, int ldw, int M, int N, int K, const GemmEpi& e,
                   hipStream_t s) {
  if (M <= 0 || N <= 0 || K <= 0) return 1;
  if (K % X3K != 0 || N % 4 != 0 || lda % 8 != 0 || ldw % 8 != 0 || lda < 2 * K || ldw < 2 * K) return 2;
  if (e.out_f32 && e.ldc % 4 != 0) return 2;
  if (e.resid && e.ldr % 4 != 0) return 2;
  if (!e.out_f32 && !e.out_bf16) return 2;
  { const int t = gemm_tail_split(1, A2, lda, W2, ldw, M, N, K, e, s); if (t >= 0) return t; }
  {
    const char* v = DOD_TUNE_ENV("DINODET_X3_TILE");
    const bool pp = v ? v[0] == 'p' : (M >= 4096);
    if (pp) return launch_gemm_x3_pp(A2, lda, W2, ldw, M, N, K, e, s);
  }
  x3_attr();
  const int gm = gemm_tile_mode();
  const int tiles = ((M + X3M - 1) / X3M) * ((N + X3N - 1) / X3N);
#define GO_(LN_) hipLaunchKernelGGL((gemm_x3_256x256_kernel<false, LN_>), dim3(tiles), dim3(1024), LDSX3, s, A2, lda, W2, ldw, M, N, K, e, gm);
  LN_DISPATCH(e, GO_)
#undef GO_
  gemm_form_launched(FORM_X3_16W);
  return hipGetLastError() == hipSuccess ? 0 : 3;
}

static std::atomic<long> g_epi_regmath{0};
long gemm_epi_regmath_count() { return g_epi_regmath.load(); }

int launch_gemm_bf16_k64(const bf16_t* A, int lda, const bf16_t* W, int ldw, int M, int N, int K, const GemmEpi& e, hipStream_t s) {
  if (M <= 0 || N <= 0 || K <= 0 || K % 64 != 0) return 2;
  x3_attr();
  const int gm = gemm_tile_mode();
  const int tiles = ((M + X3M - 1) / X3M) * ((N + X3N - 1) / X3N);
  gemm_form_launched(FORM_K64);
  if (dod_option(DOD_OPT_EPI_REGMATH) != 0 && epi_regmath_ok(e, N)) {
#define GO_(LN_) hipLaunchKernelGGL((gemm_x3_256x256_kernel<true, LN_, true>), dim3(tiles), dim3(1024), LDSX3E, s, A, lda, W, ldw, M, N, K, e, gm);
    if (ln_mode_of(e) == LN_CONS) { GO_(LN_CONS) } else { GO_(LN_NONE) }
#undef GO_
    ++g_epi_regmath;
    return hipGetLastError() == hipSuccess ? 0 : 3;
  }
#define GO_(LN_) hipLaunchKernelGGL((gemm_x3_256x256_kernel<true, LN_>), dim3(tiles), dim3(1024), LDSX3, s, A, lda, W, ldw, M, N, K, e, gm);
  LN_DISPATCH(e, GO_)
#undef GO_
  return hipGetLastError() == hipSuccess ? 0 : 3;
}
```

Baseline: 2520 images/s.

## Prefetch epilogue params and residual rows early in residual-add GEMM kernels

After: 2528 images/s (median of 4 runs). About the same (+0.3%).

```diff
diff --git a/dinov2_od_amd/csrc/dod_api.hip b/dinov2_od_amd/csrc/dod_api.hip
--- a/dinov2_od_amd/csrc/dod_api.hip
+++ b/dinov2_od_amd/csrc/dod_api.hip
@@ -34,10 +34,10 @@
   return true;
 }
 
-static std::atomic<int> g_options[DOD_OPT_COUNT] = {{-1}, {-1}, {-1}, {-1}, {-1}, {-1}, {-1}, {-1}, {-1}, {-1}, {-1}};
+static std::atomic<int> g_options[DOD_OPT_COUNT] = {{-1}, {-1}, {-1}, {-1}, {-1}, {-1}, {-1}, {-1}, {-1}, {-1}, {-1}, {-1}};
 int dod_option(int which) { return which >= 0 && which < DOD_OPT_COUNT ? g_options[which].load() : -1; }
 static const char* const k_option_names[DOD_OPT_COUNT] = {"tailsplit", "dec_fused_split", "mha_chunk_images", "no_fused_patch", "ln_fold", "deterministic", "f32_ksplit",
-                                                       "attn_bwd_flash", "epi_regmath", "f32x3_tile", "attn_diet"};
+                                                       "attn_bwd_flash", "epi_regmath", "f32x3_tile", "attn_diet", "epi_prod_early"};
 
 static std::atomic<long> g_form_launches[FORM_COUNT];
 static const char* const k_form_names[FORM_COUNT] = {"bf16_128_r2", "bf16_128_r3", "bf16_m16", "k64", "ppm", "x3_16w", "x3_pp", "h2", "fp8_rows", "fp8mx_256x128",
@@ -58,6 +58,7 @@
   if (name && !strcmp(name, "f32_ksplits")) return gemm_f32_ksplit_count();
   if (name && !strcmp(name, "epi_regmath")) return gemm_epi_regmath_count();
   if (name && !strcmp(name, "attn_diet")) return attn_half_tile_count();
+  if (name && !strcmp(name, "epi_prod_early")) return gemm_epi_prod_early_count();
   if (name && !strcmp(name, "f32x3_launches")) return gemm_f32x3_count(0);
   if (name && !strcmp(name, "f32x3_wide_launches")) return gemm_f32x3_count(1);
   if (name && !strcmp(name, "optim_launches")) return optim_launch_count();
diff --git a/dinov2_od_amd/csrc/dod_common.h b/dinov2_od_amd/csrc/dod_common.h
--- a/dinov2_od_amd/csrc/dod_common.h
+++ b/dinov2_od_amd/csrc/dod_common.h
@@ -24,6 +24,7 @@
        DOD_OPT_EPI_REGMATH,
        DOD_OPT_F32X3_TILE,
        DOD_OPT_ATTN_DIET,
+       DOD_OPT_EPI_PROD_EARLY,
        DOD_OPT_COUNT };
 int dod_option(int which);
 long gemm_tail_split_count();
@@ -32,6 +33,8 @@
 long gemm_rem_cut_count();
 long attn_half_tile_count();
 long gemm_epi_regmath_count();
+long gemm_epi_prod_early_count();
+void gemm_epi_prod_early_launched();
 enum { FORM_BF16_128_R2 = 0, FORM_BF16_128_R3, FORM_BF16_M16, FORM_K64, FORM_PPM, FORM_X3_16W, FORM_X3_PP, FORM_H2, FORM_FP8_ROWS, FORM_FP8MX_256X128,
        FORM_FP8MX2_256X128, FORM_FP8MX2_256X256, FORM_F32, FORM_PATCH_FUSED, FORM_COUNT };
 void gemm_form_launched(int form);
diff --git a/dinov2_od_amd/csrc/gemm_bf16.hip b/dinov2_od_amd/csrc/gemm_bf16.hip
--- a/dinov2_od_amd/csrc/gemm_bf16.hip
+++ b/dinov2_od_amd/csrc/gemm_bf16.hip
@@ -144,7 +144,8 @@
 __device__ unsigned long long* g_gemm_stamps = nullptr;
 #endif
 
-template <int LN>
+#define B5_PARE (B5_SLOTS * B5_STAGE)
+template <int LN, bool EARLY = false>
 __global__ __launch_bounds__(512, 4) void gemm_bf16_256x128_m16_kernel(const bf16_t* __restrict__ A, int lda,
                                                                        const bf16_t* __restrict__ W, int ldw,
                                                                        int M, int N, int K, GemmEpi e, int GM) {
@@ -182,6 +183,8 @@
     for (int j = 0; j < 4; ++j) acc[i][j] = f32x4{0.f, 0.f, 0.f, 0.f};
   const int nk = K / B4K;
   const int l15 = lane & 15, l4 = lane >> 4;
+  ProdParams pp_e = {0ull, 0.f, 1.f};
+  if constexpr (EARLY) pp_e = prod_params_fetch<LN>(e, m0, n0, M, N, tid);
   STAGE5(0, 0)
   if (nk > 1) STAGE5(1, B4K)
   int offA[4], offW[4];
@@ -195,6 +198,9 @@
     else asm volatile("s_waitcnt vmcnt(0)" ::: "memory");
     __builtin_amdgcn_s_barrier();
     asm volatile("" ::: "memory");
+    if constexpr (EARLY) {
+      if (kt == 0) prod_params_park<LN>(smem + B5_PARE, pp_e, e, m0, n0, M, N, tid);
+    }
     if (kt + 2 < nk) {
       const int ns = slot >= 1 ? slot - 1 : 2;
       STAGE5(ns, (kt + 2) * B4K)
@@ -216,6 +222,28 @@
   if (stamps) t_loop = __builtin_amdgcn_s_memrealtime();
 #endif
   constexpr int PITCH = B5N * 4 + 16;
+  if constexpr (EARLY) {
+    auto rowmap0 = [&](int row_l) { return m0 + (row_l >> 5) * 64 + (row_l & 31); };
+    auto rowmap1 = [&](int row_l) { return m0 + (row_l >> 5) * 64 + 32 + (row_l & 31); };
+    ResidBatch<EarlyShape<128, B5N, 512>::RB> rbt;
+#define B5_STAGE_ACC(P)                                                                                          \
+    __builtin_amdgcn_s_barrier();                                                                                \
+    asm volatile("" ::: "memory");                                                                               \
+    _Pragma("unroll") for (int ii = 0; ii < 2; ++ii)                                                             \
+      _Pragma("unroll") for (int j = 0; j < 4; ++j) {                                                            \
+        const int row_l = wm * 32 + ii * 16 + l15;                                                               \
+        const int col = wn * 64 + j * 16 + 4 * l4;                                                               \
+        const f32x4 a = acc[(P) * 2 + ii][j];                                                                    \
+        *reinterpret_cast<float4*>(smem + row_l * PITCH + col * 4) = make_float4(a[0], a[1], a[2], a[3]);        \
+      }
+    B5_STAGE_ACC(0)
+    drain_early_begin<128, B5N, 512>(rbt, e, M, N, n0, tid, rowmap0);
+    const ColParams cpe = prod_col_params<B5N>(smem + B5_PARE, tid);
+    drain_tile_early<128, B5N, 512, LN, true>(smem, PITCH, smem + B5_PARE, e, cpe, M, N, m0, n0, tid, rowmap0, rowmap1, rbt);
+    B5_STAGE_ACC(1)
+    drain_tile_early<128, B5N, 512, LN, false>(smem, PITCH, smem + B5_PARE, e, cpe, M, N, m0, n0, tid, rowmap1, rowmap1, rbt);
+#undef B5_STAGE_ACC
+  } else {
   const ColParams cp = load_col_params<B5N, LN>(e, n0, N, tid);
 #pragma unroll
   for (int pass = 0; pass < 2; ++pass) {
@@ -235,6 +263,7 @@
     __syncthreads();
     drain_tile<128, B5N, 512, LN>(smem, PITCH, e, cp, M, N, n0, tid, rowmap);
   }
+  }
 #ifdef DINODET_TUNING
   if (stamps && tid == 0) {
     asm volatile("s_waitcnt vmcnt(0)" ::: "memory");
@@ -247,6 +276,8 @@
 static constexpr int LDS128 = (BM * (BN * 4 + 16)) > 2 * STAGE_BYTES ? (BM * (BN * 4 + 16)) : 2 * STAGE_BYTES;
 static constexpr int LDS128R = 3 * STAGE_BYTES;
 static constexpr int LDS5 = (128 * (B5N * 4 + 16)) > B5_SLOTS * B5_STAGE ? (128 * (B5N * 4 + 16)) : B5_SLOTS * B5_STAGE;
+static_assert(B5_PARE >= 128 * (B5N * 4 + 16), "the parked parameters lie behind the ring AND the staged fp32 tile");
+static constexpr int LDS5E = B5_PARE + EPI_PAR_BYTES;
 
 static std::atomic<long> g_rem_cuts{0};
 long gemm_rem_cut_count() { return g_rem_cuts.load(); }
@@ -266,6 +297,8 @@
                    (void)hipFuncSetAttribute(reinterpret_cast<const void*>(gemm_bf16_256x128_m16_kernel<LN_>), hipFuncAttributeMaxDynamicSharedMemorySize, LDS5);
     ATTR_(LN_NONE) ATTR_(LN_CONS) ATTR_(LN_PROD)
 #undef ATTR_
+    (void)hipFuncSetAttribute(reinterpret_cast<const void*>(gemm_bf16_256x128_m16_kernel<LN_NONE, true>), hipFuncAttributeMaxDynamicSharedMemorySize, LDS5E);
+    (void)hipFuncSetAttribute(reinterpret_cast<const void*>(gemm_bf16_256x128_m16_kernel<LN_PROD, true>), hipFuncAttributeMaxDynamicSharedMemorySize, LDS5E);
     attr_set[dev] = true;
   }
   const char* force = DOD_TUNE_ENV("DINODET_GEMM_TILE");
@@ -277,7 +310,12 @@
   if (force && force[0] == 'x') return launch_gemm_bf16_k64(A, lda, W, ldw, M, N, K, e, s);
   const int gm5 = (N >= 3072 ? 8 : (N >= 2048 ? 4 : 2)) | (gemm_tile_mode() & 0x300);
   const int tiles5 = ((M + B5M - 1) / B5M) * ((N + B5N - 1) / B5N);
-#define GO_M16(LN_) hipLaunchKernelGGL(gemm_bf16_256x128_m16_kernel<LN_>, dim3(tiles5), dim3(512), LDS5, s, A, lda, W, ldw, M, N, K, e, gm5);
+  const bool early5 = epi_prod_early_ok(e);
+#define GO_M16(LN_)                                                                                                                                      \
+  if (early5 && LN_ != LN_CONS) {                                                                                                                        \
+    hipLaunchKernelGGL((gemm_bf16_256x128_m16_kernel<LN_ == LN_PROD ? LN_PROD : LN_NONE, true>), dim3(tiles5), dim3(512), LDS5E, s, A, lda, W, ldw, M, N, K, e, gm5); \
+    gemm_epi_prod_early_launched();                                                                                                                      \
+  } else hipLaunchKernelGGL(gemm_bf16_256x128_m16_kernel<LN_>, dim3(tiles5), dim3(512), LDS5, s, A, lda, W, ldw, M, N, K, e, gm5);
   if (!force && M >= 4096 && N >= 512 && K % 64 == 0 && e.act != ACT_SIGMOID && e.rows_per_img == 0) {
     static int cus[16] = {};
     if (dev >= 0 && dev < 16 && !cus[dev]) { int c = 0; (void)hipDeviceGetAttribute(&c, hipDeviceAttributeMultiprocessorCount, dev); cus[dev] = c > 0 ? c : 256; }
diff --git a/dinov2_od_amd/csrc/gemm_epi.h b/dinov2_od_amd/csrc/gemm_epi.h
--- a/dinov2_od_amd/csrc/gemm_epi.h
+++ b/dinov2_od_amd/csrc/gemm_epi.h
@@ -288,6 +288,127 @@
   }
 }
 
+#define EPI_PAR_BYTES 4096
+#define EPI_LDS_SYNC asm volatile("s_waitcnt lgkmcnt(0)" ::: "memory"); __builtin_amdgcn_s_barrier(); asm volatile("" ::: "memory");
+
+inline bool epi_prod_early_ok(const GemmEpi& e) {
+  return dod_option(DOD_OPT_EPI_PROD_EARLY) != 0 && e.resid && e.out_f32 && !e.out_bf16 && e.rows_per_img == 0 && !e.a_scale && !e.a_bs && e.ksplit <= 1 &&
+         !e.ln_stats;
+}
+
+struct ProdParams { unsigned long long shift; float bias, scale; };
+template <int LN>
+__device__ __forceinline__ ProdParams prod_params_fetch(const GemmEpi& e, int m0, int n0, int M, int N, int tid) {
+  ProdParams p = {0ull, 0.f, 1.f};
+  if (tid < 256) {
+    const int nc = n0 + tid < N ? n0 + tid : N - 1;
+    const int mc = m0 + tid < M ? m0 + tid : M - 1;
+    p.bias = *(e.bias ? e.bias + nc : e.resid);
+    p.scale = *(e.scale ? e.scale + nc : e.resid);
+    if (LN == LN_PROD) p.shift = *reinterpret_cast<const unsigned long long*>(e.ln_shift ? reinterpret_cast<const float*>(e.ln_shift + mc) : e.resid);
+  }
+  return p;
+}
+template <int LN>
+__device__ __forceinline__ void prod_params_park(char* par, ProdParams p, const GemmEpi& e, int m0, int n0, int M, int N, int tid) {
+  if (tid < 256) {
+    asm volatile("" : "+v"(p.bias), "+v"(p.scale), "+v"(p.shift));
+    const bool nok = n0 + tid < N;
+    *reinterpret_cast<float*>(par + 2048 + tid * 4) = (e.bias && nok) ? p.bias : 0.f;
+    *reinterpret_cast<float*>(par + 3072 + tid * 4) = (e.scale && nok) ? p.scale : 1.f;
+    if (LN == LN_PROD) *reinterpret_cast<unsigned long long*>(par + tid * 8) = (e.ln_shift && m0 + tid < M) ? p.shift : 0ull;
+  }
+}
+template <int COLS>
+__device__ __forceinline__ ColParams prod_col_params(const char* par, int tid) {
+  ColParams c;
+  const int cl = 4 * (tid % (COLS / 4));
+  c.bias = *reinterpret_cast<const float4*>(par + 2048 + cl * 4);
+  c.scale = *reinterpret_cast<const float4*>(par + 3072 + cl * 4);
+  c.wscale = make_float4(1.f, 1.f, 1.f, 1.f);
+  return c;
+}
+
+template <int ROWS, int COLS, int NT>
+struct EarlyShape {
+  static constexpr int C4 = COLS / 4, STEP = NT / C4, ITER = ROWS / STEP, RB = ITER % 4 == 0 ? 4 : (ITER % 2 == 0 ? 2 : 1);
+  static_assert(NT % C4 == 0 && ROWS % STEP == 0 && C4 % 32 == 0, "drain_tile's conditions");
+};
+template <int RB> struct ResidBatch { float4 r[RB]; };
+
+template <int RB, int STEP, typename RowMap>
+__device__ __forceinline__ void resid_fetch(ResidBatch<RB>& b, const GemmEpi& e, int M, int nc, int rb, int it, RowMap rowmap) {
+#pragma unroll
+  for (int j = 0; j < RB; ++j) {
+    int m = rowmap(rb + (it + j) * STEP);
+    m = m < M ? m : M - 1;
+    b.r[j] = *reinterpret_cast<const float4*>(e.resid + (size_t)m * e.ldr + nc);
+  }
+}
+
+template <int ROWS, int COLS, int NT, int LN, bool NEXT, typename RowMap, typename RowMapN>
+__device__ __forceinline__ void drain_tile_early(char* sm, int pitch, const char* par, const GemmEpi& e, const ColParams& cp, int M, int N, int m0, int n0,
+                                                 int tid, RowMap rowmap, RowMapN rowmap_next, ResidBatch<EarlyShape<ROWS, COLS, NT>::RB>& cur) {
+  typedef EarlyShape<ROWS, COLS, NT> S;
+  constexpr int C4 = S::C4, STEP = S::STEP, ITER = S::ITER, RB = S::RB;
+  constexpr bool LNF = LN == LN_PROD;
+  if (LNF && tid < ROWS)
+    *reinterpret_cast<float2*>(sm + tid * pitch + COLS * 4) = *reinterpret_cast<const float2*>(par + (rowmap(tid) - m0) * 8);
+  EPI_LDS_SYNC
+  const int c4 = tid % C4, rb = tid / C4;
+  const int n = n0 + 4 * c4;
+  const bool nv = n < N;
+  const int nc = nv ? n : N - 4;
+  const int wj = (c4 & 31) - 16;
+  const bool writer = LNF && wj >= 0 && wj < RB && (n & ~127) < N;
+#pragma unroll
+  for (int it = 0; it < ITER; it += RB) {
+    ResidBatch<RB> nxt;
+    if (it + RB < ITER) resid_fetch<RB, STEP>(nxt, e, M, nc, rb, it + RB, rowmap);
+    else if (NEXT) resid_fetch<RB, STEP>(nxt, e, M, nc, rb, 0, rowmap_next);
+    int mm[RB];
+    float kk[RB];
+#pragma unroll
+    for (int j = 0; j < RB; ++j) {
+      mm[j] = rowmap(rb + (it + j) * STEP);
+      if (LNF) kk[j] = reinterpret_cast<const float2*>(sm + (rb + (it + j) * STEP) * pitch + C4 * 16)->x;
+    }
+    float2 mine = make_float2(0.f, 0.f);
+#pragma unroll
+    for (int j = 0; j < RB; ++j) {
+      const bool ok = nv && mm[j] < M;
+      const float4 r = ok ? cur.r[j] : make_float4(0.f, 0.f, 0.f, 0.f);
+      float4 v = *reinterpret_cast<const float4*>(sm + (rb + (it + j) * STEP) * pitch + c4 * 16);
+      v.x += cp.bias.x; v.y += cp.bias.y; v.z += cp.bias.z; v.w += cp.bias.w;
+      if (e.act == ACT_GELU) { gelu_fast4(v); }
+      else if (e.act == ACT_RELU) { v.x = fmaxf(v.x, 0.f); v.y = fmaxf(v.y, 0.f); v.z = fmaxf(v.z, 0.f); v.w = fmaxf(v.w, 0.f); }
+      v.x = fmaf(v.x, cp.scale.x, r.x); v.y = fmaf(v.y, cp.scale.y, r.y);
+      v.z = fmaf(v.z, cp.scale.z, r.z); v.w = fmaf(v.w, cp.scale.w, r.w);
+      if (ok) *reinterpret_cast<float4*>(e.out_f32 + (size_t)mm[j] * e.ldc + n) = v;
+      if (LNF) {
+        if (ok && e.ln_op) ln_store_op(e, (size_t)mm[j], n, N, v);
+        const float a = v.x - kk[j], b = v.y - kk[j], c = v.z - kk[j], d = v.w - kk[j];
+        const float sum = half32_sum_hi(nv ? (a + b) + (c + d) : 0.f);
+        const float sq = half32_sum_hi(nv ? (a * a + b * b) + (c * c + d * d) : 0.f);
+        if (wj == j) mine = make_float2(sum, sq);
+      }
+    }
+    if (LNF && writer) {
+      int mw = mm[0];
+#pragma unroll
+      for (int j = 1; j < RB; ++j) mw = wj == j ? mm[j] : mw;
+      if (mw < M) e.ln_part[(size_t)mw * e.ln_npart + (n >> 7)] = mine;
+    }
+    if (it + RB < ITER || NEXT) cur = nxt;
+  }
+}
+template <int ROWS, int COLS, int NT, typename RowMap>
+__device__ __forceinline__ void drain_early_begin(ResidBatch<EarlyShape<ROWS, COLS, NT>::RB>& cur, const GemmEpi& e, int M, int N, int n0, int tid, RowMap rowmap) {
+  typedef EarlyShape<ROWS, COLS, NT> S;
+  const int n = n0 + 4 * (tid % S::C4);
+  resid_fetch<S::RB, S::STEP>(cur, e, M, n < N ? n : N - 4, tid / S::C4, 0, rowmap);
+}
+
 
 __host__ __device__ __forceinline__ bool drain8_ok(const GemmEpi& e, int N) {
   return e.out_bf16 && e.out_split <= 0 && !e.resid && e.rows_per_img == 0 && !e.a_scale && (!e.a_bs || e.w_bs) && !e.out_bs && (N & 7) == 0 && (e.ldc & 7) == 0 &&
diff --git a/dinov2_od_amd/csrc/gemm_pp.hip b/dinov2_od_amd/csrc/gemm_pp.hip
--- a/dinov2_od_amd/csrc/gemm_pp.hip
+++ b/dinov2_od_amd/csrc/gemm_pp.hip
@@ -25,7 +25,8 @@
 #define PP_STAMPS_DECL unsigned long long* const stamps = nullptr;
 #endif
 
-template <bool X3, bool DC, int LN>
+#define PP_PARE (128 * (PPN * 4 + 16))
+template <bool X3, bool DC, int LN, bool EARLY = false>
 __global__ __launch_bounds__(512) void gemm_ppm_256x256_kernel(const bf16_t* __restrict__ A, int lda,
                                                                const bf16_t* __restrict__ W, int ldw, int M, int N,
                                                                int K, GemmEpi e_, int GM) {
@@ -83,9 +84,12 @@
 #pragma unroll
   for (int j = 0; j < 4; ++j) { const int row = wq * 64 + j * 16 + l15; offW[j] = 2 * PP_PLANE + row * 64 + pp_swz(row, l4) * 16; }
 
+  ProdParams pp_e = {0ull, 0.f, 1.f};
+  if constexpr (EARLY) pp_e = prod_params_fetch<LN>(e, m0, n0, M, N, tid);
   PPM_STAGE(0, 0) PPM_STAGE(0, 1) PPM_STAGE(0, 2) PPM_STAGE(0, 3)
   if (nk > 1) { PPM_STAGE(1, 2) PPM_STAGE(1, 3) }
   if (nk > 1) asm volatile("s_waitcnt vmcnt(4)" ::: "memory"); else asm volatile("s_waitcnt vmcnt(0)" ::: "memory");
+  if constexpr (EARLY) prod_params_park<LN>(smem + PP_PARE, pp_e, e, m0, n0, M, N, tid);
   __builtin_amdgcn_s_barrier();
   if (grp_ == 1) __builtin_amdgcn_s_barrier();
   asm volatile("" ::: "memory");
@@ -164,6 +168,28 @@
   if (stamps) ts2 = __builtin_amdgcn_s_memtime();
 
   constexpr int PITCH = PPN * 4 + 16;
+  if constexpr (EARLY) {
+    auto rowmap0 = [&](int row_l) { return m0 + (row_l >> 6) * 128 + (row_l & 63); };
+    auto rowmap1 = [&](int row_l) { return m0 + (row_l >> 6) * 128 + 64 + (row_l & 63); };
+    const ColParams cpe = prod_col_params<PPN>(smem + PP_PARE, tid);
+    ResidBatch<EarlyShape<128, PPN, 512>::RB> rbt;
+    drain_early_begin<128, PPN, 512>(rbt, e, M, N, n0, tid, rowmap0);
+#define PP_STAGE_ACC(P)                                                                                          \
+    _Pragma("unroll") for (int ii = 0; ii < 4; ++ii)                                                             \
+      _Pragma("unroll") for (int j = 0; j < 4; ++j) {                                                            \
+        const int row_l = grp_ * 64 + ii * 16 + l15;                                                             \
+        const int col = wq * 64 + j * 16 + 4 * l4;                                                               \
+        const f32x4 a = acc[(P) * 4 + ii][j];                                                                    \
+        *reinterpret_cast<float4*>(smem + row_l * PITCH + col * 4) = make_float4(a[0], a[1], a[2], a[3]);        \
+      }
+    PP_STAGE_ACC(0)
+    drain_tile_early<128, PPN, 512, LN, true>(smem, PITCH, smem + PP_PARE, e, cpe, M, N, m0, n0, tid, rowmap0, rowmap1, rbt);
+    __builtin_amdgcn_s_barrier();
+    asm volatile("" ::: "memory");
+    PP_STAGE_ACC(1)
+    drain_tile_early<128, PPN, 512, LN, false>(smem, PITCH, smem + PP_PARE, e, cpe, M, N, m0, n0, tid, rowmap1, rowmap1, rbt);
+#undef PP_STAGE_ACC
+  } else {
   const ColParams cp = load_col_params<PPN, LN>(e, n0, N, tid);
   const bool wide = drain8_ok(e, N);
 #pragma unroll
@@ -183,6 +209,7 @@
     __syncthreads();
     if (wide) drain_tile_bf16x8<128, PPN, 512, LN>(smem, PITCH, e, M, N, n0, tid, rowmap);
     else drain_tile<128, PPN, 512, LN>(smem, PITCH, e, cp, M, N, n0, tid, rowmap);
+  }
   }
   if (stamps && tid == 0) {
     asm volatile("s_waitcnt vmcnt(0)" ::: "memory");
@@ -404,6 +431,7 @@
 
 
 static constexpr int LDSPP = (128 * (PPN * 4 + 16)) > 2 * PP_TILE ? (128 * (PPN * 4 + 16)) : 2 * PP_TILE;
+static constexpr int LDSPPE = PP_PARE + EPI_PAR_BYTES;
 
 #ifdef DINODET_TUNING
 static int wres_grid(int M, int N, int* gm) {
@@ -425,6 +453,10 @@
                    (void)hipFuncSetAttribute(reinterpret_cast<const void*>(gemm_ppm_256x256_kernel<true, false, LN_>), hipFuncAttributeMaxDynamicSharedMemorySize, LDSPP);
     ATTR_(LN_NONE) ATTR_(LN_CONS) ATTR_(LN_PROD)
 #undef ATTR_
+#define ATTR_(LN_) (void)hipFuncSetAttribute(reinterpret_cast<const void*>(gemm_ppm_256x256_kernel<false, false, LN_, true>), hipFuncAttributeMaxDynamicSharedMemorySize, LDSPPE); \
+                   (void)hipFuncSetAttribute(reinterpret_cast<const void*>(gemm_ppm_256x256_kernel<true, false, LN_, true>), hipFuncAttributeMaxDynamicSharedMemorySize, LDSPPE);
+    ATTR_(LN_NONE) ATTR_(LN_PROD)
+#undef ATTR_
     attr_set[dev] = true;
   }
 }
@@ -438,6 +470,13 @@
   int gm = gemm_tile_mode();
   const int tiles = wres_grid(M, N, &gm);
   gemm_form_launched(FORM_PPM);
+  if (epi_prod_early_ok(e)) {
+#define GO_(LN_) hipLaunchKernelGGL((gemm_ppm_256x256_kernel<false, false, LN_, true>), dim3(tiles), dim3(512), LDSPPE, s, A, lda, W, ldw, M, N, K, e, gm);
+    if (ln_mode_of(e) == LN_PROD) { GO_(LN_PROD) } else { GO_(LN_NONE) }
+#undef GO_
+    gemm_epi_prod_early_launched();
+    return hipGetLastError() == hipSuccess ? 0 : 3;
+  }
 #define GO_(LN_) hipLaunchKernelGGL((gemm_ppm_256x256_kernel<false, false, LN_>), dim3(tiles), dim3(512), LDSPP, s, A, lda, W, ldw, M, N, K, e, gm);
   LN_DISPATCH(e, GO_)
 #undef GO_
@@ -454,6 +493,13 @@
   int gm = gemm_tile_mode();
   const int tiles = wres_grid(M, N, &gm);
   gemm_form_launched(FORM_X3_PP);
+  if (epi_prod_early_ok(e)) {
+#define GO_(LN_) hipLaunchKernelGGL((gemm_ppm_256x256_kernel<true, false, LN_, true>), dim3(tiles), dim3(512), LDSPPE, s, A2, lda, W2, ldw, M, N, K, e, gm);
+    if (ln_mode_of(e) == LN_PROD) { GO_(LN_PROD) } else { GO_(LN_NONE) }
+#undef GO_
+    gemm_epi_prod_early_launched();
+    return hipGetLastError() == hipSuccess ? 0 : 3;
+  }
 #define GO_(LN_) hipLaunchKernelGGL((gemm_ppm_256x256_kernel<true, false, LN_>), dim3(tiles), dim3(512), LDSPP, s, A2, lda, W2, ldw, M, N, K, e, gm);
   LN_DISPATCH(e, GO_)
 #undef GO_
diff --git a/dinov2_od_amd/csrc/gemm_x3.hip b/dinov2_od_amd/csrc/gemm_x3.hip
--- a/dinov2_od_amd/csrc/gemm_x3.hip
+++ b/dinov2_od_amd/csrc/gemm_x3.hip
@@ -14,6 +14,7 @@
 __device__ __forceinline__ int x3_swz(int row, int chunk) { return chunk ^ (((row >> 3) & 1) << 1); }
 
 #define X3_PAR (X3_SLOTS * X3_STAGE)
+#define X3_PARE (128 * (X3N * 4 + 16))
 
 template <int LN, int ACT>
 __device__ __forceinline__ void x3_epi_regs(char* smem, const f32x4 (&acc)[4][4], const GemmEpi& e, int M, int N, int m0, int n0, int tid) {
@@ -62,7 +63,7 @@
 #undef X3_LDS_SYNC
 }
 
-template <bool PLAIN, int LN, bool REGM = false>
+template <bool PLAIN, int LN, bool REGM = false, bool EARLY = false>
 __global__ __launch_bounds__(1024) void gemm_x3_256x256_kernel(const bf16_t* __restrict__ A2, int lda,
                                                                const bf16_t* __restrict__ W2, int ldw, int M, int N,
                                                                int K, GemmEpi e, int GM) {
@@ -124,6 +125,8 @@
       }
     }
   }
+  ProdParams pp_e = {0ull, 0.f, 1.f};
+  if constexpr (EARLY) pp_e = prod_params_fetch<LN>(e, m0, n0, M, N, tid);
   STAGE_X3(0, 0)
   int offA[4], offW[4];
 #pragma unroll
@@ -187,6 +190,15 @@
     X3_KTILE(0)
     kt0 = 1;
   }
+  if constexpr (EARLY) {
+    asm volatile("s_waitcnt vmcnt(0)" ::: "memory");
+    __builtin_amdgcn_s_barrier();
+    asm volatile("" ::: "memory");
+    prod_params_park<LN>(smem + X3_PARE, pp_e, e, m0, n0, M, N, tid);
+    asm volatile("" ::: "memory");
+    X3_KTILE(0)
+    kt0 = 1;
+  }
   for (int kt = kt0; kt < nk; ++kt) {
     asm volatile("s_waitcnt vmcnt(0)" ::: "memory");
     __builtin_amdgcn_s_barrier();
@@ -201,6 +213,29 @@
     return;
   }
   constexpr int PITCH = X3N * 4 + 16;
+  if constexpr (EARLY) {
+    auto rowmap0 = [&](int row_l) { return m0 + (row_l >> 5) * 64 + (row_l & 31); };
+    auto rowmap1 = [&](int row_l) { return m0 + (row_l >> 5) * 64 + 32 + (row_l & 31); };
+    ResidBatch<EarlyShape<128, X3N, 1024>::RB> rbt;
+    drain_early_begin<128, X3N, 1024>(rbt, e, M, N, n0, tid, rowmap0);
+#define X3_STAGE_ACC(P)                                                                                                     \
+    __builtin_amdgcn_s_barrier();                                                                                           \
+    asm volatile("" ::: "memory");                                                                                          \
+    _Pragma("unroll") for (int ii = 0; ii < 2; ++ii)                                                                        \
+      _Pragma("unroll") for (int j = 0; j < 4; ++j) {                                                                       \
+        const int row_l = wm * 32 + ii * 16 + l15;                                                                          \
+        const int col = wn * 64 + j * 16 + 4 * l4;                                                                          \
+        const f32x4 a = acc[(P) * 2 + ii][j];                                                                               \
+        *reinterpret_cast<float4*>(smem + row_l * PITCH + col * 4) = make_float4(a[0], a[1], a[2], a[3]);                   \
+      }
+    X3_STAGE_ACC(0)
+    const ColParams cpe = prod_col_params<X3N>(smem + X3_PARE, tid);
+    drain_tile_early<128, X3N, 1024, LN, true>(smem, PITCH, smem + X3_PARE, e, cpe, M, N, m0, n0, tid, rowmap0, rowmap1, rbt);
+    X3_STAGE_ACC(1)
+    drain_tile_early<128, X3N, 1024, LN, false>(smem, PITCH, smem + X3_PARE, e, cpe, M, N, m0, n0, tid, rowmap1, rowmap1, rbt);
+#undef X3_STAGE_ACC
+    return;
+  }
   const ColParams cp = load_col_params<X3N, LN>(e, n0, N, tid);
   const bool wide = drain8_ok(e, N);
 #define X3_PASS(P)                                                                                                          \
@@ -244,6 +279,7 @@
 
 static constexpr int LDSX3 = (128 * (X3N * 4 + 16)) > X3_SLOTS * X3_STAGE ? (128 * (X3N * 4 + 16)) : X3_SLOTS * X3_STAGE;
 static constexpr int LDSX3E = X3_PAR + 4096;
+static constexpr int LDSX3P = X3_PARE + EPI_PAR_BYTES;
 
 static void x3_attr() {
   static bool attr_set[16] = {};
@@ -257,6 +293,10 @@
 #define ATTR_(LN_) (void)hipFuncSetAttribute(reinterpret_cast<const void*>(gemm_x3_256x256_kernel<true, LN_, true>), hipFuncAttributeMaxDynamicSharedMemorySize, LDSX3E);
     ATTR_(LN_NONE) ATTR_(LN_CONS)
 #undef ATTR_
+#define ATTR_(LN_) (void)hipFuncSetAttribute(reinterpret_cast<const void*>(gemm_x3_256x256_kernel<false, LN_, false, true>), hipFuncAttributeMaxDynamicSharedMemorySize, LDSX3P); \
+                   (void)hipFuncSetAttribute(reinterpret_cast<const void*>(gemm_x3_256x256_kernel<true, LN_, false, true>), hipFuncAttributeMaxDynamicSharedMemorySize, LDSX3P);
+    ATTR_(LN_NONE) ATTR_(LN_PROD)
+#undef ATTR_
     attr_set[dev] = true;
   }
 }
@@ -277,15 +317,25 @@
   x3_attr();
   const int gm = gemm_tile_mode();
   const int tiles = ((M + X3M - 1) / X3M) * ((N + X3N - 1) / X3N);
+  gemm_form_launched(FORM_X3_16W);
+  if (epi_prod_early_ok(e)) {
+#define GO_(LN_) hipLaunchKernelGGL((gemm_x3_256x256_kernel<false, LN_, false, true>), dim3(tiles), dim3(1024), LDSX3P, s, A2, lda, W2, ldw, M, N, K, e, gm);
+    if (ln_mode_of(e) == LN_PROD) { GO_(LN_PROD) } else { GO_(LN_NONE) }
+#undef GO_
+    gemm_epi_prod_early_launched();
+    return hipGetLastError() == hipSuccess ? 0 : 3;
+  }
 #define GO_(LN_) hipLaunchKernelGGL((gemm_x3_256x256_kernel<false, LN_>), dim3(tiles), dim3(1024), LDSX3, s, A2, lda, W2, ldw, M, N, K, e, gm);
   LN_DISPATCH(e, GO_)
 #undef GO_
-  gemm_form_launched(FORM_X3_16W);
   return hipGetLastError() == hipSuccess ? 0 : 3;
 }
 
 static std::atomic<long> g_epi_regmath{0};
 long gemm_epi_regmath_count() { return g_epi_regmath.load(); }
+static std::atomic<long> g_epi_prod_early{0};
+long gemm_epi_prod_early_count() { return g_epi_prod_early.load(); }
+void gemm_epi_prod_early_launched() { ++g_epi_prod_early; }
 
 int launch_gemm_bf16_k64(const bf16_t* A, int lda, const bf16_t* W, int ldw, int M, int N, int K, const GemmEpi& e, hipStream_t s) {
   if (M <= 0 || N <= 0 || K <= 0 || K % 64 != 0) return 2;
@@ -300,6 +350,13 @@
     ++g_epi_regmath;
     return hipGetLastError() == hipSuccess ? 0 : 3;
   }
+  if (epi_prod_early_ok(e)) {
+#define GO_(LN_) hipLaunchKernelGGL((gemm_x3_256x256_kernel<true, LN_, false, true>), dim3(tiles), dim3(1024), LDSX3P, s, A, lda, W, ldw, M, N, K, e, gm);
+    if (ln_mode_of(e) == LN_PROD) { GO_(LN_PROD) } else { GO_(LN_NONE) }
+#undef GO_
+    gemm_epi_prod_early_launched();
+    return hipGetLastError() == hipSuccess ? 0 : 3;
+  }
 #define GO_(LN_) hipLaunchKernelGGL((gemm_x3_256x256_kernel<true, LN_>), dim3(tiles), dim3(1024), LDSX3, s, A, lda, W, ldw, M, N, K, e, gm);
   LN_DISPATCH(e, GO_)
 #undef GO_
```
